# cosdata/cosdata

Measured on AMD Instinct MI355X. Metric: QPS at recall@10≥0.95, 1024-dim dense cosine, 1/2/4/8 MI355X, higher is better.
Workload: dtype u8

## Files before the change

### cosdata_amd/_lib.py

```python
from __future__ import annotations

import ctypes as C
import os
import subprocess

_PKG = os.path.dirname(os.path.abspath(__file__))
SO_PATH = os.path.join(_PKG, "libcosdata_hip.so")
CSRC = os.path.join(_PKG, "csrc")

OK, ERR_STORAGE_MISMATCH, ERR_CALCULATION, ERR_INVALID, ERR_UNIMPLEMENTED, ERR_HIP, ERR_NOT_READY, ERR_NO_DEVICE = range(8)
STATUS_NAMES = {
    0: "OK", 1: "StorageMismatch", 2: "CalculationError", 3: "Invalid", 4: "Unimplemented", 5: "HipError",
    6: "NotReady", 7: "NoDevice",
}
ABI_VERSION = 1


class CosdataError(RuntimeError):

    def __init__(self, status: int, message: str):
        super().__init__(f"[{STATUS_NAMES.get(status, status)}] {message}")
        self.status = status


class CosParams(C.Structure):
    _fields_ = [
        ("struct_size", C.c_uint32), ("abi_version", C.c_uint32), ("dim", C.c_uint32), ("metric", C.c_uint32),
        ("storage", C.c_uint32), ("resolution", C.c_uint32), ("range_lo", C.c_float), ("range_hi", C.c_float),
        ("num_layers", C.c_uint32), ("neighbors_count", C.c_uint32), ("level0_neighbors_count", C.c_uint32),
        ("ef_construction", C.c_uint32), ("ef_search", C.c_uint32), ("shortlist_size", C.c_uint32),
        ("visited_mode", C.c_uint32), ("device", C.c_int32), ("id_base", C.c_uint32), ("reserved", C.c_uint32),
        ("seed", C.c_uint64),
    ]


class CosSearchStats(C.Structure):
    _fields_ = [
        ("evals", C.c_uint64), ("expansions", C.c_uint64), ("adj_bytes", C.c_uint64), ("rerank_rows", C.c_uint64),
        ("walk_ms", C.c_float), ("finalize_ms", C.c_float), ("prep_ms", C.c_float), ("reserved", C.c_uint32),
    ]


class CosWalkSplit(C.Structure):
    _fields_ = [
        ("struct_size", C.c_uint32), ("queries", C.c_uint32), ("table_level_min", C.c_uint32), ("table_cols", C.c_uint32),
        ("cut_after_level", C.c_uint32), ("table_early_wgs", C.c_uint32),
        ("table_ms", C.c_float), ("upper_ms", C.c_float), ("sort_ms", C.c_float), ("lower_ms", C.c_float),
        ("table_int8_ops", C.c_double), ("table_evals", C.c_uint64),
        ("upper_evals", C.c_uint64), ("upper_expansions", C.c_uint64), ("upper_adj_bytes", C.c_uint64),
        ("lower_evals", C.c_uint64), ("lower_expansions", C.c_uint64), ("lower_adj_bytes", C.c_uint64),
    ]


class CosTimingSummary(C.Structure):
    _fields_ = [("launches", C.c_uint32), ("prep_ms_sum", C.c_float), ("walk_ms_sum", C.c_float), ("finalize_ms_sum", C.c_float),
                ("walk_ms_min", C.c_float), ("walk_ms_max", C.c_float)]


class CosCoalescingStats(C.Structure):
    _fields_ = [("launches", C.c_uint64), ("queries", C.c_uint64), ("requests", C.c_uint64), ("closed_full", C.c_uint64),
                ("closed_quiet", C.c_uint64), ("closed_deadline", C.c_uint64), ("solo_calls", C.c_uint64)]


class CosSparseStats(C.Structure):
    _fields_ = [("kernel_ms", C.c_float), ("blocks", C.c_uint32), ("postings_visited", C.c_uint64), ("posting_bytes", C.c_uint64)]


class CosFlatStats(C.Structure):
    _fields_ = [("gemm_ms", C.c_float), ("gemm_launches", C.c_uint32), ("int8_ops", C.c_double), ("code_bytes", C.c_double)]


SCAN_SKIP_DELETED = 1


class CosScanMask(C.Structure):
    _fields_ = [("struct_size", C.c_uint32), ("flags", C.c_uint32), ("n_masks", C.c_uint32), ("bits", C.c_void_p),
                ("query_mask", C.c_void_p)]


class CosBM25Stats(C.Structure):
    _fields_ = [("struct_size", C.c_uint32), ("documents_count", C.c_uint32), ("n_terms", C.c_uint32), ("largest_doc_id", C.c_uint32),
                ("dir_rows", C.c_uint32), ("dir_tiles", C.c_uint32), ("reserved", C.c_uint32),
                ("postings", C.c_uint64), ("tombstones", C.c_uint64), ("device_bytes", C.c_uint64)]


class CosSparseIndexStats(C.Structure):
    _fields_ = [("struct_size", C.c_uint32), ("n_vectors", C.c_uint32), ("n_dims", C.c_uint32), ("dir_rows", C.c_uint32),
                ("dir_tiles", C.c_uint32), ("packed", C.c_uint32), ("have_raw", C.c_uint32), ("reserved", C.c_uint32),
                ("postings", C.c_uint64), ("removed", C.c_uint64), ("raw_pairs", C.c_uint64), ("device_bytes", C.c_uint64)]


class CosHybridRequest(C.Structure):
    _fields_ = [("struct_size", C.c_uint32), ("B", C.c_uint32), ("arm", C.c_void_p), ("dense_queries", C.c_void_p),
                ("sparse_dims", C.c_void_p), ("sparse_vals", C.c_void_p), ("sparse_offsets", C.c_void_p),
                ("bm25_terms", C.c_void_p), ("bm25_offsets", C.c_void_p),
                ("sparse_early_terminate_threshold", C.c_float), ("sparse_reranking_factor", C.c_uint32),
                ("top_k", C.c_uint32), ("fusion_constant_k", C.c_float)]


def build(force: bool = False, verbose: bool = False) -> str:
    srcs = [os.path.join(CSRC, f) for f in os.listdir(CSRC) if f.endswith((".hip", ".h"))]
    srcs.append(os.path.join(_PKG, "..", "include", "cosdata_hip.h"))
    stale = force or not os.path.exists(SO_PATH) or any(os.path.getmtime(s) > os.path.getmtime(SO_PATH) for s in srcs)
    if force:
        subprocess.check_call(["make", "-C", CSRC, "-s", "clean"])
    if stale:
        cmd = ["make", "-C", CSRC, "-j", str(max(2, min(16, 2 * (os.cpu_count() or 1))))]
        if not verbose:
            cmd.append("-s")
        subprocess.check_call(cmd)
    return SO_PATH


_lib = None

ABI_SYMBOLS = [
    "cos_index_create", "cos_index_destroy", "cos_last_error_string", "cos_device_count",
    "cos_index_upload_vectors", "cos_index_set_root", "cos_index_upload_graph_level", "cos_index_level_count",
    "cos_index_download_graph_level", "cos_index_download_codes", "cos_index_download_root", "cos_index_build", "cos_index_append", "cos_index_delete", "cos_index_restore_link_state", "cos_index_release_link_state", "cos_index_enable_metadata", "cos_index_upload_meta_nodes", "cos_index_upload_meta_graph_level", "cos_index_build_meta", "cos_index_meta_level_count", "cos_index_download_meta_graph_level", "cos_search_filtered_batch",
    "cos_ann_search_filtered_batch", "cos_index_load_reference_dir", "cos_reference_dir_level_counts", "cos_reference_dir_read_level",
    "cos_search_batch", "cos_search_batch_device", "cos_ann_search_batch", "cos_index_set_coalescing", "cos_index_coalescing_stats", "cos_index_set_ef_search",
    "cos_index_set_visited_mode", "cos_index_set_latency_mode", "cos_index_set_latency_waves", "cos_index_set_walk_order", "cos_index_walk_order_cuts", "cos_index_set_walk_table", "cos_index_walk_table_info", "cos_index_last_walk_split", "cos_index_enable_timing", "cos_index_last_stats", "cos_index_timing_summary", "cos_quantize_batch",
    "cos_code_bytes", "cos_sample_values_range", "cos_distance_batch", "cos_bruteforce_topk", "cos_flat_search_batch",
    "cos_flat_search_masked_batch", "cos_bruteforce_topk_masked", "cos_index_deleted_count", "cos_index_download_deleted", "cos_bm25_create", "cos_bm25_destroy",
    "cos_bm25_insert", "cos_bm25_delete", "cos_bm25_stats", "cos_bm25_download",
    "cos_bm25_search_batch", "cos_bm25_search_batch_device", "cos_rrf_fuse_batch", "cos_hybrid_search_batch", "cos_text_process", "cos_text_count_tokens", "cos_bm25_term_frequency", "cos_xxhash32", "cos_stem_english", "cos_sparse_create", "cos_sparse_build_csr", "cos_sparse_create_from_vectors", "cos_sparse_destroy", "cos_sparse_search_batch", "cos_sparse_last_stats", "cos_sparse_layout",
    "cos_sparse_set_max_candidates", "cos_sparse_max_candidates", "cos_sparse_search_batch_device",
    "cos_hybrid_create", "cos_hybrid_destroy", "cos_hybrid_search_mixed",
    "cos_sparse_insert", "cos_sparse_delete", "cos_sparse_stats", "cos_sparse_download", "cos_merge_topk_device", "cos_merge_topk_packed_device", "cos_hbm_probe",
    "cos_shardset_unique_id", "cos_shardset_create", "cos_shardset_destroy", "cos_shardset_search_batch", "cos_shardset_exchange_device",
    "cos_tuning_set", "cos_tuning_clear", "cos_tuning_get",
]


def lib():
    global _lib
    if _lib is not None:
        return _lib
    if not os.path.exists(SO_PATH):
        raise CosdataError(ERR_NO_DEVICE, f"{SO_PATH} is missing: build it with `python -c 'import __graft_entry__ as g; g.build()'` "
                                          "(the HIP extension is mandatory; there is no CPU path)")
    try:
        import torch
    except ImportError:
        pass
    L = C.CDLL(SO_PATH)
    vp, i32, u32, f32 = C.c_void_p, C.c_int32, C.c_uint32, C.c_float
    sig = {
        "cos_index_create": [C.POINTER(CosParams), C.POINTER(vp)],
        "cos_index_destroy": [vp],
        "cos_device_count": [C.POINTER(i32)],
        "cos_index_upload_vectors": [vp, vp, u32, u32],
        "cos_index_set_root": [vp, vp],
        "cos_index_upload_graph_level": [vp, u32, u32, vp, vp],
        "cos_index_level_count": [vp, u32, C.POINTER(u32)],
        "cos_index_download_graph_level": [vp, u32, vp, vp],
        "cos_index_download_codes": [vp, vp, vp],
        "cos_index_download_root": [vp, vp],
        "cos_index_build": [vp, u32],
        "cos_index_append": [vp, vp, u32, u32, u32],
        "cos_index_release_link_state": [vp],
        "cos_index_restore_link_state": [vp],
        "cos_index_delete": [vp, vp, u32],
        "cos_index_load_reference_dir": [vp, C.c_char_p, u32, u32],
        "cos_index_enable_metadata": [vp, u32, u32],
        "cos_index_upload_meta_nodes": [vp, u32, vp, vp],
        "cos_index_upload_meta_graph_level": [vp, u32, u32, vp, vp],
        "cos_search_filtered_batch": [vp, vp, u32, vp, vp, u32, vp, vp, vp, vp],
        "cos_ann_search_filtered_batch": [vp, vp, u32, vp, vp, vp, vp, vp, vp],
        "cos_reference_dir_level_counts": [C.c_char_p, u32, u32, u32, vp],
        "cos_reference_dir_read_level": [C.c_char_p, u32, u32, u32, u32, vp, vp],
        "cos_search_batch": [vp, vp, u32, u32, vp, vp, vp, vp],
        "cos_search_batch_device": [vp, vp, u32, u32, vp, vp, vp, vp, vp],
        "cos_ann_search_batch": [vp, vp, u32, vp, vp, vp, vp],
        "cos_index_set_ef_search": [vp, u32],
        "cos_index_set_coalescing": [vp, u32, u32],
        "cos_index_coalescing_stats": [vp, C.POINTER(CosCoalescingStats)],
        "cos_index_set_visited_mode": [vp, u32],
        "cos_index_build_meta": [vp, u32, vp, vp, vp, u32],
        "cos_index_meta_level_count": [vp, u32, C.POINTER(u32)],
        "cos_index_download_meta_graph_level": [vp, u32, vp, vp],
        "cos_index_set_latency_mode": [vp, u32],
        "cos_index_set_latency_waves": [vp, u32],
        "cos_index_set_walk_order": [vp, u32],
        "cos_index_walk_order_cuts": [vp, C.POINTER(u32), u32, C.POINTER(u32)],
        "cos_index_enable_timing": [vp, i32],
        "cos_index_last_stats": [vp, vp, C.POINTER(CosSearchStats)],
        "cos_index_set_walk_table": [vp, u32, u32],
        "cos_index_walk_table_info": [vp, C.POINTER(u32), C.POINTER(u32)],
        "cos_index_last_walk_split": [vp, vp, C.POINTER(CosWalkSplit)],
        "cos_index_timing_summary": [vp, vp, C.POINTER(CosTimingSummary)],
        "cos_quantize_batch": [u32, u32, u32, f32, f32, vp, u32, vp, vp],
        "cos_sample_values_range": [vp, u32, u32, f32, C.POINTER(f32), C.POINTER(f32)],
        "cos_distance_batch": [u32, u32, u32, u32, vp, vp, u32, vp, vp, u32, vp, vp, u32, vp, vp],
        "cos_bruteforce_topk": [vp, vp, u32, u32, vp, vp],
        "cos_flat_search_batch": [vp, vp, u32, u32, vp, vp, vp, C.POINTER(CosFlatStats)],
        "cos_flat_search_masked_batch": [vp, vp, u32, u32, C.POINTER(CosScanMask), vp, vp, vp, C.POINTER(CosFlatStats)],
        "cos_bruteforce_topk_masked": [vp, vp, u32, u32, C.POINTER(CosScanMask), vp, vp, vp],
        "cos_index_deleted_count": [vp, C.POINTER(u32)],
        "cos_index_download_deleted": [vp, vp],
        "cos_bm25_create": [i32, vp, vp, u32, vp, vp, u32, C.POINTER(vp)],
        "cos_bm25_destroy": [vp],
        "cos_bm25_insert": [vp, vp, vp, u32, vp, vp],
        "cos_bm25_delete": [vp, vp, vp, u32, vp],
        "cos_bm25_stats": [vp, C.POINTER(CosBM25Stats)],
        "cos_bm25_download": [vp, C.POINTER(u32), C.POINTER(C.c_uint64), vp, vp, vp, vp, vp],
        "cos_bm25_search_batch": [vp, vp, vp, u32, u32, vp, vp, vp],
        "cos_bm25_search_batch_device": [vp, vp, vp, u32, u32, vp, vp, vp, vp],
        "cos_rrf_fuse_batch": [vp, vp, u32, vp, vp, u32, u32, f32, u32, vp, vp, vp],
        "cos_hybrid_search_batch": [vp, vp, vp, vp, vp, u32, u32, f32, vp, vp, vp],
        "cos_sparse_create": [i32, u32, f32, vp, u32, vp, vp, u32, vp, vp, vp, C.POINTER(vp)],
        "cos_sparse_build_csr": [u32, f32, u32, vp, vp, vp, vp, vp, vp, C.POINTER(u32)],
        "cos_sparse_create_from_vectors": [i32, u32, f32, u32, vp, vp, vp, i32, C.POINTER(vp)],
        "cos_sparse_destroy": [vp],
        "cos_sparse_search_batch": [vp, vp, vp, vp, u32, u32, f32, u32, vp, vp, vp],
        "cos_sparse_search_batch_device": [vp, vp, vp, vp, u32, u32, f32, u32, vp, vp, vp, vp],
        "cos_hybrid_create": [i32, C.POINTER(vp)],
        "cos_hybrid_destroy": [vp],
        "cos_hybrid_search_mixed": [vp, vp, vp, vp, C.POINTER(CosHybridRequest), vp, vp, vp],
        "cos_sparse_last_stats": [vp, vp],
        "cos_sparse_layout": [vp, C.POINTER(u32)],
        "cos_sparse_set_max_candidates": [vp, u32],
        "cos_sparse_max_candidates": [vp, C.POINTER(u32)],
        "cos_sparse_insert": [vp, u32, vp, vp, vp, C.POINTER(u32)],
        "cos_sparse_delete": [vp, vp, vp, u32, vp, vp, C.POINTER(C.c_uint64)],
        "cos_sparse_stats": [vp, C.POINTER(CosSparseIndexStats)],
        "cos_sparse_download": [vp, C.POINTER(u32), C.POINTER(C.c_uint64), vp, vp, vp],
        "cos_merge_topk_device": [vp, vp, vp, u32, u32, u32, vp, vp, vp, i32, vp],
        "cos_merge_topk_packed_device": [vp, u32, u32, u32, vp, vp, vp, i32, vp],
        "cos_hbm_probe": [i32, u32, C.c_uint64, u32, u32, C.POINTER(C.c_double)],
        "cos_shardset_unique_id": [vp],
        "cos_shardset_create": [vp, u32, u32, u32, vp, C.POINTER(vp)],
        "cos_shardset_destroy": [vp],
        "cos_shardset_search_batch": [vp, vp, u32, u32, vp, vp, vp],
        "cos_shardset_exchange_device": [vp, vp, u32, u32, vp, vp, vp, vp, vp],
        "cos_tuning_set": [C.c_char_p, C.c_int64],
        "cos_tuning_clear": [C.c_char_p],
        "cos_tuning_get": [C.c_char_p, C.POINTER(C.c_int64), C.POINTER(i32)],
    }
    for name, args in sig.items():
        fn = getattr(L, name)
        fn.restype = i32
        fn.argtypes = args
    L.cos_last_error_string.restype = C.c_char_p
    L.cos_last_error_string.argtypes = []
    L.cos_stem_english.restype = C.c_size_t
    L.cos_stem_english.argtypes = [vp, C.c_char_p, C.c_size_t, C.c_char_p, C.c_size_t]
    L.cos_text_process.restype = i32
    L.cos_text_process.argtypes = [C.c_char_p, C.c_size_t, u32, f32, f32, f32, vp, vp, vp, vp, u32, C.POINTER(u32)]
    L.cos_text_count_tokens.restype = u32
    L.cos_text_count_tokens.argtypes = [C.c_char_p, C.c_size_t, u32]
    L.cos_bm25_term_frequency.restype = f32
    L.cos_bm25_term_frequency.argtypes = [u32, u32, f32, f32, f32]
    L.cos_xxhash32.restype = u32
    L.cos_xxhash32.argtypes = [C.c_char_p, C.c_size_t, u32]
    L.cos_code_bytes.restype = C.c_size_t
    L.cos_code_bytes.argtypes = [u32, u32, u32]
    _lib = L
    return L


def check(rc: int):
    if rc != OK:
        raise CosdataError(rc, lib().cos_last_error_string().decode("utf-8", "replace"))


def tuning_set(name: str, value: int):
    check(lib().cos_tuning_set(name.encode(), int(value)))


def tuning_clear(name: str | None = None):
    check(lib().cos_tuning_clear(name.encode() if name is not None else None))


def tuning_get(name: str):
    v, isset = C.c_int64(), C.c_int32()
    check(lib().cos_tuning_get(name.encode(), C.byref(v), C.byref(isset)))
    return int(v.value) if isset.value else None


class tuning:

    def __init__(self, **knobs):
        self.knobs = knobs
        self.old = {}

    def __enter__(self):
        try:
            for k, v in self.knobs.items():
                old = tuning_get(k)
                tuning_set(k, v)
                self.old[k] = old
        except Exception:
            self.__exit__()
            raise
        return self

    def __exit__(self, *exc):
        for k, v in self.old.items():
            if v is None:
                tuning_clear(k)
            else:
                tuning_set(k, v)
        return False
```

### cosdata_amd/csrc/engine.hip

```cpp
#include <hip/hip_runtime.h>

#include <algorithm>
#include <cstdarg>
#include <cstdio>
#include <cstdlib>
#include <chrono>
#include <cmath>
#include <condition_variable>
#include <cstring>
#include <map>
#include <mutex>
#include <string>
#include <thread>
#include <vector>

#include "engine_internal.h"

using namespace cosdev;

static thread_local std::string g_err;
int32_t cos_fail(int32_t code, const char *fmt, ...) {
    char buf[512];
    va_list ap;
    va_start(ap, fmt);
// ... 506 lines not shown

extern "C" int32_t cos_index_download_root(const cos_index *ix, float *root_raw) {
    if (!ix || !root_raw) return cos_fail(COS_ERR_INVALID, "null argument");
    if (!ix->have_root) return cos_fail(COS_ERR_NOT_READY, "no root");
    memcpy(root_raw, ix->root_raw.data(), (size_t)ix->p.dim * 4);
    return COS_OK;
}

static int32_t ensure_level_table(cos_index *ix);
static u32 walk_table_min_B(const cos_index *ix);
extern "C" int32_t cos_index_set_ef_search(cos_index *ix, uint32_t ef) {
    if (!ix) return cos_fail(COS_ERR_INVALID, "null index");
    if (ef > cosdev::WALK_GENERAL_MAX_EF) return cos_fail(COS_ERR_UNIMPLEMENTED, "ef > %u not supported on the device", cosdev::WALK_GENERAL_MAX_EF);
    std::lock_guard<std::mutex> g(ix->mu);
    const bool live = graph_ready(ix);
    if (live)
        if (int32_t rc = cos_set_device(ix)) return rc;
    ix->p.ef_search = ef;
    if (live && walk_table_min_B(ix)) (void)ensure_level_table(ix);
    return COS_OK;
}
extern "C" int32_t cos_index_set_visited_mode(cos_index *ix, uint32_t mode) {
    if (!ix || mode > 1) return cos_fail(COS_ERR_INVALID, "bad visited mode");
    std::lock_guard<std::mutex> g(ix->mu);
    ix->p.visited_mode = mode;
    return COS_OK;
}
extern "C" int32_t cos_index_set_latency_mode(cos_index *ix, uint32_t max_queries) {
    if (!ix) return cos_fail(COS_ERR_INVALID, "null");
    std::lock_guard<std::mutex> g(ix->mu);
    ix->lat_max_B = max_queries;
    return COS_OK;
}

extern "C" int32_t cos_index_set_latency_waves(cos_index *ix, uint32_t max_queries) {
    if (!ix) return cos_fail(COS_ERR_INVALID, "null");
    std::lock_guard<std::mutex> g(ix->mu);
    ix->lat4_max_B = max_queries;
    return COS_OK;
}
extern "C" int32_t cos_index_set_walk_order(cos_index *ix, uint32_t min_queries) {
    if (!ix) return cos_fail(COS_ERR_INVALID, "null");
    std::lock_guard<std::mutex> g(ix->mu);
    ix->walk_order_min_B = min_queries;
    return COS_OK;
}
extern "C" int32_t cos_index_enable_timing(cos_index *ix, int32_t on) {
    if (!ix) return cos_fail(COS_ERR_INVALID, "null");
    std::lock_guard<std::mutex> g(ix->mu);
    if (on && !ix->timing) for (auto &kv : ix->ws) kv.second->ev_count = 0;
    ix->timing = on != 0;
    return COS_OK;
}

int32_t vis_tab_prepare(VisTab &vt, const cos_index *ix, u32 B, u32 ef, hipStream_t st, WalkArgs &wa) {
    const u32 M = std::max(ix->p.level0_neighbors_count, ix->p.neighbors_count);
    const u64 log_cap = (u64)ef * M + 2;
    u32 max_nodes = 0;
    for (const LevelHost &l : ix->lv) max_nodes = std::max(max_nodes, l.n);
    const u32 words = (max_nodes + 31) / 32 + 1;
    if (log_cap > 0xFFFFFFFFull) return cos_fail(COS_ERR_INVALID, "ef too large");
    const size_t need_bits = (size_t)B * words, need_log = (size_t)B * log_cap;
    if (need_bits > vt.bits.cap || need_log > vt.log.cap) {
        HIP_TRY(hipStreamSynchronize(st));
        if (need_bits > vt.bits.cap) vt.zeroed = false;
        HIP_TRY(vt.bits.grow(need_bits));
        HIP_TRY(vt.log.grow(need_log));
    }
    if (!vt.zeroed) {
        HIP_TRY(hipMemsetAsync(vt.bits, 0, vt.bits.cap * 4, st));
        vt.zeroed = true;
    }
    wa.vis_bits = vt.bits;
    wa.vis_log = vt.log;
    wa.vis_words_per_query = words;
    wa.vis_log_cap = (u32)log_cap;
    return COS_OK;
}

static int32_t ensure_order_rank(cos_index *ix) {
    if (ix->order_rank_valid) return COS_OK;
    for (u32 l = 0; l < cosdev::MAX_LEVELS; l++) {
        ix->d_order_rank[l].reset();
        ix->order_rank_n[l] = 0;
    }
    ix->order_levels.clear();
    const u32 Ltop = ix->p.num_layers;
    auto usable = [&](u32 l) { return l >= 1 && l <= Ltop && ix->lv[l].n > 1 && ix->lv[l].n <= (1u << 20) && ix->lv[l].d_adj_node; };
    std::vector<u32> want;
    if (const long long mask = cosdev::tune(cosdev::TUNE_WALK_SPLIT_LEVELS); mask != cosdev::TUNE_UNSET) {
        for (u32 l = Ltop; l >= 1; l--)
            if ((mask >> l) & 1) want.push_back(l);
    } else {
        for (u32 l = 1; l <= Ltop; l++)
            if (usable(l) && (size_t)ix->lv[l].n * ix->row_stride <= ((size_t)64 << 20)) { want.push_back(l); break; }
    }
    u32 prev = Ltop + 1;
    for (u32 l : want) {
        if (!usable(l) || l >= prev) continue;
        ix->order_levels.push_back(l);
        prev = l;
    }
    if (!ix->order_levels.empty()) HIP_TRY(hipDeviceSynchronize());
    for (u32 kl : ix->order_levels) {
        const LevelHost &H = ix->lv[kl];
        const u32 n = H.n, M = H.M;
        std::vector<u32> adj((size_t)n * M), rank(n, 0u), stack;
        HIP_TRY(hipMemcpy(adj.data(), H.d_adj_node, adj.size() * 4, hipMemcpyDeviceToHost));
        std::vector<uint8_t> seen(n, 0);
        u32 next = 0;
        auto dfs_from = [&](u32 start) {
            stack.push_back(start);
            while (!stack.empty()) {
                const u32 v = stack.back();
                stack.pop_back();
                if (seen[v]) continue;
                seen[v] = 1;
                rank[v] = next++;
                const u32 *row = &adj[(size_t)v * M];
                for (u32 j = M; j-- > 0;) {
                    const u32 u = row[j];
                    if (u != cosdev::ROW_EMPTY && u < n && !seen[u]) stack.push_back(u);
                }
            }
        };
        dfs_from(n - 1);
        for (u32 v = 0; v < n; v++) if (!seen[v]) dfs_from(v);
        HIP_TRY(ix->d_order_rank[kl].alloc(n));
        HIP_TRY(hipMemcpy(ix->d_order_rank[kl], rank.data(), (size_t)n * 4, hipMemcpyHostToDevice));
        ix->order_rank_n[kl] = n;
    }
    ix->order_rank_valid = true;
    return COS_OK;
}

static void clear_current_table(cos_index *ix) {
    ix->d_tcodes = nullptr;
    ix->d_tmags = nullptr;
    ix->d_tcsums = nullptr;
    ix->table_cols = 0;
    ix->table_level_min = 0;
    ix->table_stride = 0;
}
static u32 walk_table_max_cols(const cos_index *ix) {
    const long long env = cosdev::tune_or(cosdev::TUNE_WALK_TABLE_COLS, -1);
    return env >= 0 ? (u32)std::min<long long>(env, 1ll << 20) : ix->walk_table_max_cols;
}
static u32 walk_table_min_B(const cos_index *ix) {
    const long long env = cosdev::tune_or(cosdev::TUNE_WALK_TABLE_MIN_B, -1);
    return env >= 0 ? (u32)std::min<long long>(env, 0xFFFFFFFFll) : ix->walk_table_min_B;
}
static constexpr long long WALK_TABLE_EARLY_WGS_DEFAULT = 0;
static constexpr long long WALK_UP_TABLE_DEFAULT = 1;
cosdev::WalkPlanIn cos_walk_plan_in(const cos_index *ix, u32 B, u32 ef) {
    cosdev::WalkPlanIn in{};
    in.eng = ix->eng;
    in.storage = ix->p.storage;
    in.nchunks = ix->nchunks;
    in.G = ix->G;
    in.num_layers = ix->p.num_layers;
    for (u32 l = 0; l <= ix->p.num_layers; l++) in.M[l] = ix->lv[l].M;
    in.shortlist = ix->p.shortlist_size;
    in.visited_mode = ix->p.visited_mode;
    in.mdim = ix->meta.mdim;
    in.B = B;
    in.ef = ef;
    in.chain = true;
    const long long lat = cosdev::tune_or(cosdev::TUNE_WALK_LAT, -1), lat4 = cosdev::tune_or(cosdev::TUNE_WALK_LAT4, -1);
    in.lat_max_B = lat >= 0 ? (u32)std::min(lat, 0xFFFFFFFFll) : ix->lat_max_B;
    in.lat4_max_B = lat4 >= 0 ? (u32)std::min(lat4, 0xFFFFFFFFll) : ix->lat4_max_B;
    in.small_table_tk = cosdev::tune_or(cosdev::TUNE_WALK_SMALL_TABLE_TK, 1) != 0;
    in.adj_mag_mode = (u32)cosdev::tune_or(cosdev::TUNE_WALK_ADJ_MAG, 1);
    in.table_min_B = walk_table_min_B(ix);
    in.order_min_B = ix->walk_order_min_B;
    in.chain_min_B = ix->chain_min_B;
    in.side_min_B = ix->walk_side_min_B;
    in.table_after_sort = cosdev::tune_or(cosdev::TUNE_WALK_TABLE_AFTER_SORT, 1);
    in.table_supported = cosdev::level_table_eng_supported(ix->eng, ix->row_stride);
    in.adj_mag_valid = ix->adj_mag_valid;
    in.up_table_mode = (u32)std::min<long long>(std::max<long long>(cosdev::tune_or(cosdev::TUNE_WALK_UP_TABLE, WALK_UP_TABLE_DEFAULT), 0), 2);
    in.table_early_wgs = (u32)std::min<long long>(std::max<long long>(cosdev::tune_or(cosdev::TUNE_WALK_TABLE_EARLY_WGS, WALK_TABLE_EARLY_WGS_DEFAULT), 0), 0xFFFFFFFFll);
    in.table_queue = cosdev::level_table_gemm_queue(ix->eng, ix->row_stride);
    in.n_cus = ix->n_cus;
    return in;
}
static int32_t ensure_level_table(cos_index *ix) {
    const u32 max_cols = walk_table_max_cols(ix);
    const bool automatic = max_cols == COS_WALK_TABLE_AUTO;
    const u32 efs = ix->p.ef_search, Mup = ix->p.neighbors_count;
    const u64 c_rule = (u64)cosdev::tune_or(cosdev::TUNE_WALK_TABLE_RULE_C, 2u * efs <= 3u * Mup ? 10 : (efs <= 2u * Mup ? 8 : 6));
    const u64 per_level = automatic ? std::min<u64>(c_rule * ix->p.ef_search * ix->p.neighbors_count, 1u << 20) : (u64)(1u << 20);
    const u64 total_cap = automatic ? (u64)(1u << 20) : (u64)max_cols;
    const u64 key = automatic ? (0x8000000000000000ull | per_level) : (u64)max_cols;
    if (ix->level_table_valid && ix->table_built_for_key == key) return COS_OK;
    if (!ix->level_table_valid) {
        HIP_TRY(hipDeviceSynchronize());
        ix->table_sets.clear();
    }
    ix->level_table_valid = true;
    ix->table_built_for_key = key;
    clear_current_table(ix);
    for (const auto &t : ix->table_sets)
        if (t.key == key) {
            ix->table_level_min = t.level_min;
            ix->table_cols = t.cols;
            ix->table_stride = t.stride;
            memcpy(ix->table_col0, t.col0, sizeof(t.col0));
            ix->d_tcodes = t.tcodes;
            ix->d_tmags = t.tmags;
            ix->d_tcsums = t.tcsums;
            return COS_OK;
        }
    if (!cosdev::level_table_eng_supported(ix->eng, ix->row_stride) || max_cols == 0) return COS_OK;
    const u32 Ltop = ix->p.num_layers;
    u32 cols = 0, lmin = 0;
    for (u32 l = Ltop; l >= 1; l--) {
        if (!ix->lv[l].d_node_vec || ix->lv[l].n == 0 || ix->lv[l].n > per_level || (u64)cols + ix->lv[l].n > total_cap) break;
        cols += ix->lv[l].n;
        lmin = l;
    }
    if (lmin == 0) return COS_OK;
    HIP_TRY(hipDeviceSynchronize());
    cos_index::TableSet t;
    auto build = [&]() -> hipError_t {
        hipError_t e = t.tcodes.alloc((size_t)cols * ix->row_stride);
        if (e == hipSuccess) e = t.tmags.alloc(cols);
        if (e == hipSuccess) e = t.tcsums.alloc(cols);
        u32 c0 = 0;
        for (u32 l = Ltop; l >= lmin && e == hipSuccess; l--) {
            ix->table_col0[l] = c0;
            e = cosdev::launch_level_table_gather(ix->d_codes, ix->d_mags, ix->row_stride, ix->lv[l].d_node_vec, ix->lv[l].n, c0, t.tcodes, t.tmags, nullptr);
            c0 += ix->lv[l].n;
        }
        if (e == hipSuccess) e = cosdev::launch_code_sums(t.tcodes, ix->row_stride, cols, t.tcsums, nullptr);
        if (e == hipSuccess) e = hipDeviceSynchronize();
        return e;
    };
    if (const hipError_t e = build(); e != hipSuccess) {
        (void)hipDeviceSynchronize();
        if (e == hipErrorOutOfMemory) {
            (void)hipGetLastError();
            return COS_OK;
        }
        ix->level_table_valid = false;
        HIP_TRY(e);
    }
    ix->d_tcodes = t.tcodes;
    ix->d_tmags = t.tmags;
    ix->d_tcsums = t.tcsums;
    ix->table_cols = cols;
    ix->table_level_min = lmin;
    ix->table_stride = ((u64)cols + 31) / 32 * 32;
    t.key = key;
    t.level_min = lmin;
    t.cols = cols;
    t.stride = ix->table_stride;
    memcpy(t.col0, ix->table_col0, sizeof(t.col0));
    ix->table_sets.push_back(std::move(t));
    return COS_OK;
}

extern "C" int32_t cos_index_set_walk_table(cos_index *ix, uint32_t max_cols, uint32_t min_queries) {
    if (!ix) return cos_fail(COS_ERR_INVALID, "null argument");
    if (max_cols > (1u << 20) && max_cols != COS_WALK_TABLE_AUTO) return cos_fail(COS_ERR_INVALID, "max_cols must be <= 2^20 (or COS_WALK_TABLE_AUTO)");
    std::lock_guard<std::mutex> g(ix->mu);
    ix->walk_table_max_cols = max_cols;
    ix->walk_table_min_B = min_queries;
    return COS_OK;
}

extern "C" int32_t cos_index_walk_table_info(cos_index *ix, uint32_t *out_level_min, uint32_t *out_cols) {
    if (!ix || !out_level_min || !out_cols) return cos_fail(COS_ERR_INVALID, "null argument");
    *out_level_min = *out_cols = 0;
    if (!graph_ready(ix)) return cos_fail(COS_ERR_NOT_READY, "index needs vectors, root and every graph level");
    int32_t rc = cos_set_device(ix);
    if (rc) return rc;
    std::lock_guard<std::mutex> g(ix->mu);
    if (walk_table_min_B(ix) == 0) return COS_OK;
    if ((rc = ensure_level_table(ix))) return rc;
    *out_level_min = ix->table_level_min;
    *out_cols = ix->table_cols;
    return COS_OK;
}

static int32_t ensure_adj_mags(cos_index *ix) {
    if (ix->adj_mag_valid) return COS_OK;
    if (!graph_ready(ix) || ix->meta.mdim != 0u) return COS_OK;
    if (cosdev::walk_rows_over_64_slots(cos_walk_plan_in(ix, 0, 0))) return COS_OK;
    HIP_TRY(hipDeviceSynchronize());
    for (u32 l = 0; l <= ix->p.num_layers; l++) {
        ix->lv[l].d_adj_mag.reset();
    }
    for (u32 l = 0; l <= ix->p.num_layers; l++) {
        LevelHost &H = ix->lv[l];
        const u32 slots = std::min(H.M, ix->p.shortlist_size);
        const hipError_t e = H.d_adj_mag.alloc((size_t)H.n * slots);
        if (e == hipErrorOutOfMemory) {
            (void)hipGetLastError();
            for (u32 k = 0; k < l; k++) ix->lv[k].d_adj_mag.reset();
            return COS_OK;
        }
        HIP_TRY(e);
        HIP_TRY(cosdev::launch_fill_adj_mag(H.d_adj_vec, ix->d_mags, H.d_adj_mag, H.n, H.M, slots, ix->own_stream));
    }
    HIP_TRY(hipStreamSynchronize(ix->own_stream));
    ix->adj_mag_valid = true;
    return COS_OK;
}

static int32_t ensure_adj_up(cos_index *ix) {
    const u32 want = (ix->adj_mag_valid && ix->level_table_valid && ix->table_level_min >= 2u && ix->eng == ENG_U8 && ix->G == 64u &&
                      cosdev::tune_or(cosdev::TUNE_WALK_UP_TABLE, WALK_UP_TABLE_DEFAULT) != 0)
                         ? ix->table_level_min - 1u
                         : 0u;
    if (want != 0u && (ix->adj_up_level == want || ix->adj_up_oom_level == want)) return COS_OK;
    bool any = false;
    for (u32 l = 0; l <= ix->p.num_layers; l++) any = any || ix->lv[l].d_adj_up;
    if (any) {
        HIP_TRY(hipDeviceSynchronize());
        for (u32 l = 0; l <= ix->p.num_layers; l++) ix->lv[l].d_adj_up.reset();
    }
    ix->adj_up_level = 0;
    if (want == 0u) return COS_OK;
    ix->adj_up_oom_level = 0;
    HIP_TRY(hipDeviceSynchronize());
    LevelHost &H = ix->lv[want];
    const LevelHost &U = ix->lv[want + 1];
    const u32 slots = std::min(H.M, ix->p.shortlist_size);
    if (!H.d_adj_node || !U.d_child || H.n == 0 || U.n == 0) return COS_OK;
    DevArr<u32> up;
    hipError_t e = H.d_adj_up.alloc((size_t)H.n * slots);
    if (e == hipSuccess) e = up.alloc(H.n);
    if (e == hipErrorOutOfMemory) {
        (void)hipGetLastError();
        H.d_adj_up.reset();
        ix->adj_up_oom_level = want;
        return COS_OK;
    }
    HIP_TRY(e);
    HIP_TRY(cosdev::launch_fill_adj_up(H.d_adj_vec, H.d_adj_node, ix->d_mags, U.d_child, U.n, up, H.d_adj_up, H.n, H.M, slots, ix->own_stream));
    HIP_TRY(hipStreamSynchronize(ix->own_stream));
    ix->adj_up_level = want;
    return COS_OK;
}

int32_t cos_prepare_walk_plans(cos_index *ix) {
    std::lock_guard<std::mutex> g(ix->mu);
    if (int32_t rc = ensure_adj_mags(ix)) return rc;
    if (ix->walk_order_min_B)
        if (int32_t rc = ensure_order_rank(ix)) return rc;
    if (walk_table_min_B(ix)) {
        if (int32_t rc = ensure_level_table(ix)) return rc;
        if (int32_t rc = ensure_adj_up(ix)) return rc;
    }
    return COS_OK;
}

extern "C" int32_t cos_index_walk_order_cuts(cos_index *ix, uint32_t *out_levels, uint32_t cap, uint32_t *out_n) {
    if (!ix || !out_n || (cap && !out_levels)) return cos_fail(COS_ERR_INVALID, "null argument");
    *out_n = 0;
    if (!graph_ready(ix)) return cos_fail(COS_ERR_NOT_READY, "index needs vectors, root and every graph level");
    int32_t rc = cos_set_device(ix);
    if (rc) return rc;
    std::lock_guard<std::mutex> g(ix->mu);
    if ((rc = ensure_order_rank(ix))) return rc;
    for (u32 l : ix->order_levels) {
        if (*out_n < cap) out_levels[*out_n] = l;
        (*out_n)++;
    }
    return COS_OK;
}

struct SearchLaunch {
    cosdev::WalkPlan plan;
    u32 ef = 0, visited_mode = 0;
    bool timed = false;
    u64 tab_stride = 0;
    u32 tab_col0[cosdev::MAX_LEVELS] = {};
    const uint8_t *tcodes = nullptr;
    const float *tmags = nullptr;
    const u32 *tcsums = nullptr;
    u32 n_keys = 0, key_level[cosdev::MAX_LEVELS], key_n[cosdev::MAX_LEVELS];
    const u32 *order_rank[cosdev::MAX_LEVELS];
};

static int32_t get_workspace(cos_index *ix, void *key, hipStream_t st, u32 B, u32 top_k, bool host_api, Workspace **out, SearchLaunch *L,
                             bool chain = true) {
    std::lock_guard<std::mutex> g(ix->mu);
    std::unique_ptr<Workspace> &slot = ix->ws[key];
    if (!slot) slot.reset(new Workspace());
    Workspace *w = slot.get();
    const u32 L1 = ix->p.num_layers + 1;
    if (B > w->capB) {
        u32 cap = std::max(B, 64u);
        HIP_TRY(hipStreamSynchronize(st));
        w->capB = 0;
        w->cap_topk = 0;
        HIP_TRY(w->q_codes.alloc((size_t)cap * ix->row_stride));
        HIP_TRY(w->q_mags.alloc(cap));
        HIP_TRY(w->q_raw_mags.alloc(cap));
        HIP_TRY(w->walk_ids.alloc((size_t)cap * L1 * KEEP_SEARCH));
        HIP_TRY(w->walk_sims.alloc((size_t)cap * L1 * KEEP_SEARCH));
        HIP_TRY(w->walk_counts.alloc((size_t)cap * L1));
        HIP_TRY(w->walk_status.alloc(cap));
        HIP_TRY(w->stats.alloc((size_t)cap * 4));
        HIP_TRY(w->stats2.alloc((size_t)cap * 4));
        HIP_TRY(w->qsums.alloc(cap));
        HIP_TRY(w->tab_queue.alloc(16));
        if (ix->eng == ENG_Q2) HIP_TRY(w->qdig.alloc((size_t)cap * (ix->row_stride / 16) * 64));
        HIP_TRY(w->fin_flags.alloc((size_t)cap + 1));
        HIP_TRY(w->rerank_rows.alloc(cap));
        HIP_TRY(w->d_queries.alloc((size_t)cap * ix->p.dim));
        HIP_TRY(w->d_out_counts.alloc(cap));
        HIP_TRY(w->d_out_status.alloc(cap));
        w->capB = cap;
    }
    L->ef = ix->p.ef_search;
    L->visited_mode = ix->p.visited_mode;
    L->timed = ix->timing;
    cosdev::WalkPlanIn in = cos_walk_plan_in(ix, B, L->ef);
    in.chain = chain;
    const cosdev::WalkPlan want = cosdev::walk_plan(in);
    cosdev::WalkHave have{};
    if (want.refill_adj_mag) {
        if (int32_t rc = ensure_adj_mags(ix)) return rc;
        in.adj_mag_valid = ix->adj_mag_valid;
    }
    if (want.prepare_order) {
        if (w->order.cap < w->capB) {
            HIP_TRY(hipStreamSynchronize(st));
            HIP_TRY(cosdev::walk_order_reserve(w->order, w->capB));
        }
        if (int32_t rc = ensure_order_rank(ix)) return rc;
        have.order_buffers = w->order.cap >= B;
        have.n_order_keys = (u32)ix->order_levels.size();
        have.order_level0 = have.n_order_keys ? ix->order_levels[0] : 0u;
    }
    if (want.prepare_table) {
        if (int32_t rc = ensure_level_table(ix)) return rc;
        if (int32_t rc = ensure_adj_up(ix)) return rc;
        have.adj_up_level = ix->adj_up_level;
        const size_t need = (size_t)w->capB * ix->table_stride;
        if (need > w->tab.cap) {
            const size_t budget = (size_t)cosdev::tune_or(cosdev::TUNE_WALK_TABLE_MAX_BYTES, (long long)48 << 30);
            HIP_TRY(hipStreamSynchronize(st));
            ix->table_bytes_total -= w->tab.cap * 4;
            w->tab.reset();
            if (ix->table_bytes_total + need * 4 <= budget) {
                if (const hipError_t e = w->tab.alloc(need); e == hipSuccess)
                    ix->table_bytes_total += need * 4;
                else if (e == hipErrorOutOfMemory)
                    (void)hipGetLastError();
                else
                    HIP_TRY(e);
            }
        }
        have.table_level_min = ix->level_table_valid ? ix->table_level_min : 0u;
        have.table_cols = ix->table_cols;
        have.table_buffer = w->tab && (size_t)B * ix->table_stride <= w->tab.cap;
    }
    L->plan = cosdev::walk_plan(in, &have);
    if (L->plan.use_table) {
        L->tab_stride = ix->table_stride;
        memcpy(L->tab_col0, ix->table_col0, sizeof(L->tab_col0));
        L->tcodes = ix->d_tcodes;
        L->tmags = ix->d_tmags;
        L->tcsums = ix->d_tcsums;
    }
    if (L->plan.ordered)
        for (u32 l : ix->order_levels) {
            L->key_level[L->n_keys] = l;
            L->key_n[L->n_keys] = ix->order_rank_n[l];
            L->order_rank[L->n_keys++] = ix->d_order_rank[l];
        }
    if (host_api && (size_t)top_k * w->capB > (size_t)w->cap_topk * w->capB) {
        w->cap_topk = 0;
        HIP_TRY(w->d_out_ids.alloc((size_t)w->capB * top_k));
        HIP_TRY(w->d_out_scores.alloc((size_t)w->capB * top_k));
        w->cap_topk = top_k;
    }
    if (w->ev.empty()) {
        w->ev.assign((size_t)Workspace::EV_RING * Workspace::EV_PER, nullptr);
        for (auto &e : w->ev) HIP_TRY(hipEventCreate(&e));
    }
    if (!w->walk_done) HIP_TRY(hipEventCreateWithFlags(&w->walk_done, hipEventDisableTiming));
    if (!w->walk_fin) HIP_TRY(hipEventCreateWithFlags(&w->walk_fin, hipEventDisableTiming));
    if (!w->last_range) HIP_TRY(hipEventCreateWithFlags(&w->last_range, hipEventDisableTiming));
    if (!w->upper_done) HIP_TRY(hipEventCreateWithFlags(&w->upper_done, hipEventDisableTiming));
    *out = w;
    return COS_OK;
}

static int32_t run_search(cos_index *ix, Workspace *w, const SearchLaunch &L, const float *d_queries, u32 B, u32 top_k, u32 *d_out_ids,
                          float *d_out_scores, u32 *d_out_counts, int32_t *d_out_status, bool do_finalize, hipStream_t st,
                          hipStream_t st_fin = nullptr, hipEvent_t walk_ev = nullptr) {
    const cosdev::WalkPlan &plan = L.plan;
    const bool timed = L.timed, ordered = plan.ordered, chained = plan.chained;
    const u32 ef = L.ef, n_keys = L.n_keys;
    IndexDev dev = cos_make_index_dev(ix);
    dev.visited_mode = L.visited_mode;
    for (u32 l = 0; l <= dev.num_layers; l++)
        if (!((plan.use_adj_mag >> l) & 1u)) dev.lv[l].adj_mag = nullptr;
    for (u32 l = 0; l <= dev.num_layers; l++)
        if (plan.up_table_level != l || l == 0u || dev.lv[l].adj_mag == nullptr) dev.lv[l].adj_up = nullptr;
    WalkArgs wa;
    memset(&wa, 0, sizeof(wa));
    if (dev.visited_mode == COS_VISITED_EXACT) {
        int32_t rc = vis_tab_prepare(w->vis, ix, B, ef, st, wa);
        if (rc) return rc;
    }
    hipEvent_t *ev = &w->ev[(size_t)(w->ev_count % Workspace::EV_RING) * Workspace::EV_PER];
    if (timed) HIP_TRY(hipEventRecord(ev[0], st));
    HIP_TRY(launch_quantize_rows(ix->eng, d_queries, ix->p.dim, B, ix->p.dim, ix->p.range_lo, ix->p.range_hi, w->q_codes, ix->row_stride,
                                 w->q_mags, w->q_raw_mags, st, plan.use_table && ix->eng == ENG_U8 ? w->qsums.p : nullptr));
    HIP_TRY(hipMemsetAsync(w->stats2, 0, (size_t)B * 32, st));
    if (plan.use_table) {
        auto table_part = [&](hipEvent_t cos_index::*handle_ev, hipEvent_t own_ev, hipEvent_t *marks, u32 wgs, bool first) -> int32_t {
            if (plan.table_waits_for_sort) {
                std::lock_guard<std::mutex> g(ix->chain_mu);
                if (ix->*handle_ev && ix->*handle_ev != own_ev) HIP_TRY(hipStreamWaitEvent(st, ix->*handle_ev, 0));
            }
            if (timed) HIP_TRY(hipEventRecord(marks[0], st));
            HIP_TRY(cosdev::launch_level_table(ix->eng, w->q_codes, w->q_mags, w->qsums, w->qdig, B, L.tcodes, L.tmags, L.tcsums, ix->row_stride, plan.table_cols,
                                               w->tab, L.tab_stride, ix->n_cus, st, w->tab_queue, wgs, first, plan.table_waits_for_sort));
            if (timed) HIP_TRY(hipEventRecord(marks[1], st));
            return COS_OK;
        };
        if (cosdev::level_table_gemm_queue(ix->eng, ix->row_stride)) HIP_TRY(hipMemsetAsync(w->tab_queue, 0, sizeof(u32), st));
        if (plan.table_early_wgs) {
            if (int32_t rc = table_part(&cos_index::chain_upper_ev, w->upper_done, ev + 4, plan.table_early_wgs, true)) return rc;
            if (int32_t rc = table_part(&cos_index::chain_ev, w->walk_done, ev + 8, 0u, false)) return rc;
        } else if (int32_t rc = table_part(&cos_index::chain_last_range_ev, w->last_range, ev + 4, 0u, true))
            return rc;
    }
    if (timed) HIP_TRY(hipEventRecord(ev[1], st));
    wa.qcodes = w->q_codes;
    wa.qmags = w->q_mags;
    wa.B = B;
    wa.ef = ef;
    wa.keep = KEEP_SEARCH;
    wa.out_ids = w->walk_ids;
    wa.out_sims = w->walk_sims;
    wa.out_counts = w->walk_counts;
    wa.out_status = w->walk_status;
    wa.out_stats = w->stats;
    wa.out_stats2 = w->stats2;
    if (plan.use_table) {
        wa.tab = w->tab;
        wa.tab_mags = L.tmags;
        wa.tab_stride = L.tab_stride;
        wa.tab_level_min = plan.table_level_min;
        memcpy(wa.tab_col0, L.tab_col0, sizeof(L.tab_col0));
    }
    hipStream_t sw = st;
    if (plan.side_stream) {
        if (!w->walk_stream) {
            int lo = 0, hi = 0;
            HIP_TRY(hipDeviceGetStreamPriorityRange(&lo, &hi));
            HIP_TRY(hipStreamCreateWithPriority(&w->walk_stream, hipStreamNonBlocking, lo));
            HIP_TRY(hipEventCreateWithFlags(&w->prep_done, hipEventDisableTiming));
        }
        sw = w->walk_stream;
        HIP_TRY(hipEventRecord(w->prep_done, st));
        HIP_TRY(hipStreamWaitEvent(sw, w->prep_done, 0));
    }
    auto walk = [&](hipStream_t s) -> int32_t {
        if (!ordered) {
            if (chained) HIP_TRY(hipEventRecord(w->upper_done, s));
            if (chained) HIP_TRY(hipEventRecord(w->last_range, s));
            HIP_TRY(launch_walk(ix->eng, dev, wa, plan.kernel, s));
            return COS_OK;
        }
        wa.phase = 1;
        wa.entry0 = w->order.entry0;
        wa.order_key = w->order.order_key;
        wa.order_iota = w->order.iota;
        u32 first = dev.num_layers;
        for (u32 i = 0; i <= n_keys; i++) {
            const bool last = i == n_keys;
            wa.level_first = first;
            wa.level_last = last ? 0u : L.key_level[i];
            wa.key_n = last ? 0u : L.key_n[i];
            wa.order_rank = last ? nullptr : L.order_rank[i];
            if (last && chained) HIP_TRY(hipEventRecord(w->last_range, s));
            HIP_TRY(launch_walk(ix->eng, dev, wa, plan.kernel, s));
            if (last) break;
            if (chained && i == 0) HIP_TRY(hipEventRecord(w->upper_done, s));
            if (timed && i == 0) HIP_TRY(hipEventRecord(ev[6], s));
            HIP_TRY(cosdev::launch_walk_order(w->order, B, L.key_n[i], ix->num_xcd, s));
            if (timed && i == 0) HIP_TRY(hipEventRecord(ev[7], s));
            wa.q_order = w->order.q_order;
            first = L.key_level[i] - 1;
        }
        return COS_OK;
    };
    if (chained) {
        std::lock_guard<std::mutex> g(ix->chain_mu);
        if (ix->chain_ev && ix->chain_ev != w->walk_done) HIP_TRY(hipStreamWaitEvent(sw, ix->chain_ev, 0));
        if (timed) HIP_TRY(hipEventRecord(ev[1], sw));
        if (int32_t rc = walk(sw)) return rc;
        HIP_TRY(hipEventRecord(w->walk_done, sw));
        ix->chain_ev = w->walk_done;
        ix->chain_last_range_ev = w->last_range;
        ix->chain_upper_ev = w->upper_done;
    } else {
        if (timed && sw != st) HIP_TRY(hipEventRecord(ev[1], sw));
        if (int32_t rc = walk(sw)) return rc;
    }
    if (timed) HIP_TRY(hipEventRecord(ev[2], sw));
    hipStream_t sf = st_fin ? st_fin : st;
    if (sf != sw) {
        hipEvent_t we = walk_ev ? walk_ev : w->walk_fin;
        HIP_TRY(hipEventRecord(we, sw));
        HIP_TRY(hipStreamWaitEvent(sf, we, 0));
    }
    if (do_finalize) {
        HIP_TRY(launch_finalize(dev, d_queries, ix->p.dim, w->q_raw_mags, w->walk_ids, w->walk_sims, w->walk_counts, w->walk_status, B, top_k,
                                d_out_ids, d_out_scores, d_out_counts, d_out_status, w->rerank_rows, sf, ordered ? w->order.q_order : nullptr, w->fin_flags));
    }
    if (timed) { HIP_TRY(hipEventRecord(ev[3], sf)); w->ev_count++; }
    w->lastB = B;
    w->timed = timed;
    w->last_plan = plan;
    { std::lock_guard<std::mutex> g(ix->mu); ix->last_ws = w; }
    return COS_OK;
}

static int32_t check_search_args(cos_index *ix, const void *q, u32 B, u32 top_k) {
    if (!ix || !q) return cos_fail(COS_ERR_INVALID, "null argument");
    if (!graph_ready(ix)) return cos_fail(COS_ERR_NOT_READY, "index needs vectors, root and every graph level before search");
    if (top_k == 0 || top_k > 1024) return cos_fail(COS_ERR_INVALID, "top_k must be in [1, 1024]");
    if (B == 0) return cos_fail(COS_ERR_INVALID, "empty batch");
    return cos_set_device(ix);
}

extern "C" int32_t cos_search_batch_device(cos_index *ix, const float *d_queries, uint32_t B, uint32_t top_k, uint32_t *d_out_ids,
                                           float *d_out_scores, uint32_t *d_out_counts, int32_t *d_out_status, void *stream) {
    int32_t rc = check_search_args(ix, d_queries, B, top_k);
    if (rc) return rc;
    if (!d_out_ids || !d_out_scores || !d_out_counts || !d_out_status) return cos_fail(COS_ERR_INVALID, "null output");
    Workspace *w;
    SearchLaunch L;
    rc = get_workspace(ix, stream, (hipStream_t)stream, B, top_k, false, &w, &L);
    if (rc) return rc;
    return run_search(ix, w, L, d_queries, B, top_k, d_out_ids, d_out_scores, d_out_counts, d_out_status, true, (hipStream_t)stream);
}

struct PipeLease {
    cos_index *ix;
    HostPipe *hp = nullptr;
    explicit PipeLease(cos_index *ix_) : ix(ix_) {}
    PipeLease(const PipeLease &) = delete;
    PipeLease &operator=(const PipeLease &) = delete;
    int32_t acquire() {
        std::unique_lock<std::mutex> lk(ix->pipe_mu);
        for (;;) {
            if (!ix->pipes_free.empty()) { hp = ix->pipes_free.back(); ix->pipes_free.pop_back(); break; }
            if (ix->pipes_all.size() < COS_MAX_HOST_PIPES) {
                std::unique_ptr<HostPipe> n(new HostPipe());
                hipError_t e = hipStreamCreateWithFlags(&n->s[0], hipStreamNonBlocking);
                if (e != hipSuccess) return cos_fail(COS_ERR_HIP, "hipStreamCreateWithFlags: %s", hipGetErrorString(e));
                hp = n.get();
                ix->pipes_all.push_back(std::move(n));
                break;
            }
            ix->pipe_cv.wait(lk);
        }
        ix->host_calls_active.fetch_add(1);
        return COS_OK;
    }
    ~PipeLease() {
        if (!hp) return;
        ix->host_calls_active.fetch_sub(1);
        { std::lock_guard<std::mutex> g(ix->pipe_mu); ix->pipes_free.push_back(hp); }
        ix->pipe_cv.notify_one();
    }
};

static int32_t report_status(const int32_t *status, u32 B) {
    for (u32 b = 0; b < B; b++)
        if (status[b] != COS_OK) return cos_fail(status[b], "query %u failed with status %d (zero-norm vector -> DistanceError::CalculationError)", b, status[b]);
    return COS_OK;
}

static int32_t search_host_simple(cos_index *ix, HostPipe *hp, const float *queries, uint32_t B, uint32_t top_k, uint32_t *out_ids, float *out_scores,
                                  uint32_t *out_counts, int32_t *out_status) {
    hipStream_t st = hp->s[0];
    Workspace *w;
    SearchLaunch L;
    int32_t rc = get_workspace(ix, (void *)st, st, B, top_k, true, &w, &L);
    if (rc) return rc;
    HIP_TRY(hipMemcpyAsync(w->d_queries, queries, (size_t)B * ix->p.dim * 4, hipMemcpyHostToDevice, st));
    rc = run_search(ix, w, L, w->d_queries, B, top_k, w->d_out_ids, w->d_out_scores, w->d_out_counts, w->d_out_status, true, st);
    if (rc) { (void)hipDeviceSynchronize(); return rc; }
    std::vector<int32_t> status(B);
    hipError_t e = hipMemcpyAsync(out_ids, w->d_out_ids, (size_t)B * top_k * 4, hipMemcpyDeviceToHost, st);
    if (e == hipSuccess) e = hipMemcpyAsync(out_scores, w->d_out_scores, (size_t)B * top_k * 4, hipMemcpyDeviceToHost, st);
    if (e == hipSuccess) e = hipMemcpyAsync(out_counts, w->d_out_counts, (size_t)B * 4, hipMemcpyDeviceToHost, st);
    if (e == hipSuccess) e = hipMemcpyAsync(status.data(), w->d_out_status, (size_t)B * 4, hipMemcpyDeviceToHost, st);
    const hipError_t es = hipStreamSynchronize(st);
    HIP_TRY(e);
    HIP_TRY(es);
    if (out_status) memcpy(out_status, status.data(), (size_t)B * 4);
    return report_status(status.data(), B);
}

static int32_t search_host_pipelined(cos_index *ix, HostPipe *hp, const float *queries, uint32_t B, uint32_t top_k, uint32_t *out_ids,
                                     float *out_scores, uint32_t *out_counts, int32_t *out_status) {
    const size_t dim = ix->p.dim;
    const u32 chunk = (((B + HostPipe::MAX_CHUNKS - 1) / HostPipe::MAX_CHUNKS) + 255u) & ~255u;
    const u32 nch = (B + chunk - 1) / chunk;
    if (!hp->s[1]) HIP_TRY(hipStreamCreateWithFlags(&hp->s[1], hipStreamNonBlocking));
    if (!hp->sc) HIP_TRY(hipStreamCreateWithFlags(&hp->sc, hipStreamNonBlocking));
    if (!hp->sf) HIP_TRY(hipStreamCreateWithFlags(&hp->sf, hipStreamNonBlocking));
    for (u32 i = 0; i < HostPipe::MAX_CHUNKS; i++) {
        if (!hp->ev_in[i]) HIP_TRY(hipEventCreateWithFlags(&hp->ev_in[i], hipEventDisableTiming));
        if (!hp->ev_walk[i]) HIP_TRY(hipEventCreateWithFlags(&hp->ev_walk[i], hipEventDisableTiming));
    }
    HIP_TRY(hp->d_q.grow((size_t)B * dim));
    HIP_TRY(hp->d_ids.grow((size_t)B * top_k));
    HIP_TRY(hp->d_scores.grow((size_t)B * top_k));
    HIP_TRY(hp->d_counts.grow((size_t)B));
    HIP_TRY(hp->d_status.grow((size_t)B));
    struct Drain {
        HostPipe *hp;
        bool ok = false;
        ~Drain() {
            hipStream_t sts[] = {hp->sc, hp->s[0], hp->s[1], hp->sf};
            for (hipStream_t st : sts) if (st) (void)hipStreamSynchronize(st);
            if (!ok) (void)hipDeviceSynchronize();
        }
    } drain{hp};
    for (u32 i = 0; i < nch; i++) {
        const u32 c0 = i * chunk, cb = std::min(chunk, B - c0);
        hipStream_t st = hp->s[i & 1];
        Workspace *w;
        SearchLaunch L;
        int32_t rc = get_workspace(ix, (void *)&hp->wkey[i], st, cb, top_k, false, &w, &L, false);
        if (rc) return rc;
        float *dq = hp->d_q + (size_t)c0 * dim;
        const float *src = queries + (size_t)c0 * dim;
        HIP_TRY(hipMemcpyAsync(dq, src, (size_t)cb * dim * 4, hipMemcpyHostToDevice, hp->sc));
        HIP_TRY(hipEventRecord(hp->ev_in[i], hp->sc));
        HIP_TRY(hipStreamWaitEvent(st, hp->ev_in[i], 0));
        rc = run_search(ix, w, L, dq, cb, top_k, hp->d_ids + (size_t)c0 * top_k, hp->d_scores + (size_t)c0 * top_k, hp->d_counts + c0, hp->d_status + c0,
                        true, st, hp->sf, hp->ev_walk[i]);
        if (rc) return rc;
    }
    std::vector<int32_t> status(B);
    hipError_t e = hipMemcpyAsync(out_ids, hp->d_ids, (size_t)B * top_k * 4, hipMemcpyDeviceToHost, hp->sf);
    if (e == hipSuccess) e = hipMemcpyAsync(out_scores, hp->d_scores, (size_t)B * top_k * 4, hipMemcpyDeviceToHost, hp->sf);
    if (e == hipSuccess) e = hipMemcpyAsync(out_counts, hp->d_counts, (size_t)B * 4, hipMemcpyDeviceToHost, hp->sf);
    if (e == hipSuccess) e = hipMemcpyAsync(status.data(), hp->d_status, (size_t)B * 4, hipMemcpyDeviceToHost, hp->sf);
    const hipError_t es = hipStreamSynchronize(hp->sf);
    HIP_TRY(e);
    HIP_TRY(es);
    drain.ok = true;
    if (out_status) memcpy(out_status, status.data(), (size_t)B * 4);
    return report_status(status.data(), B);
}

static u32 host_pipeline_min_B() {
    return (u32)cosdev::tune_or(cosdev::TUNE_HOST_PIPELINE_MIN_B, 8192);
}

static int32_t search_host_once(cos_index *ix, const float *queries, uint32_t B, uint32_t top_k, uint32_t *out_ids, float *out_scores,
                                uint32_t *out_counts, int32_t *out_status) {
    PipeLease lease(ix);
    int32_t rc = lease.acquire();
    if (rc) return rc;
    const u32 min_B = host_pipeline_min_B();
    if (min_B && B >= min_B && ix->host_calls_active.load() == 1)
        return search_host_pipelined(ix, lease.hp, queries, B, top_k, out_ids, out_scores, out_counts, out_status);
    return search_host_simple(ix, lease.hp, queries, B, top_k, out_ids, out_scores, out_counts, out_status);
}

// ... 173 lines not shown
        {
            std::lock_guard<std::mutex> lk(sl->mu);
            sl->rc = r;
            sl->err = e;
            sl->done = true;
        }
        sl->cv_done.notify_all();
    } else {
        std::unique_lock<std::mutex> lk(sl->mu);
        while (!sl->done) sl->cv_done.wait(lk);
    }
    const int32_t slot_rc = sl->rc;
    std::string slot_err = slot_rc != COS_OK ? sl->err : std::string();
    int32_t my_rc = COS_OK;
    u32 bad_q = 0;
    if (slot_rc == COS_OK) {
        const u32 *p_ids = sl->pin_out.as<const u32>();
        const float *p_sc = (const float *)(p_ids + (size_t)sl->cap * top_k);
        const u32 *p_cnt = (const u32 *)(p_sc + (size_t)sl->cap * top_k);
        const int32_t *p_st = (const int32_t *)(p_cnt + sl->cap);
        memcpy(out_ids, p_ids + (size_t)off * top_k, (size_t)B * top_k * 4);
        memcpy(out_scores, p_sc + (size_t)off * top_k, (size_t)B * top_k * 4);
        memcpy(out_counts, p_cnt + off, (size_t)B * 4);
        if (out_status) memcpy(out_status, p_st + off, (size_t)B * 4);
        for (u32 b = 0; b < B; b++)
            if (p_st[off + b] != COS_OK) { my_rc = p_st[off + b]; bad_q = b; break; }
    }
    if (sl->left.fetch_sub(1, std::memory_order_acq_rel) == 1) {
        std::lock_guard<std::mutex> lk(ix->co_mu);
        sl->n_req = 0;
        sl->closed = false;
    }
    if (slot_rc != COS_OK) return cos_fail(slot_rc, "%s", slot_err.c_str());
    if (my_rc != COS_OK) return cos_fail(my_rc, "query %u failed with status %d (zero-norm vector -> DistanceError::CalculationError)", bad_q, my_rc);
    return COS_OK;
}

extern "C" int32_t cos_ann_search_batch(cos_index *ix, const float *queries, uint32_t B, uint32_t *out_ids, float *out_sims,
                                        uint32_t *out_counts, int32_t *out_status) {
    int32_t rc = check_search_args(ix, queries, B, 1);
    if (rc) return rc;
    if (!out_ids || !out_sims || !out_counts) return cos_fail(COS_ERR_INVALID, "null output");
    PipeLease lease(ix);
    rc = lease.acquire();
    if (rc) return rc;
    hipStream_t st = lease.hp->s[0];
    Workspace *w;
    SearchLaunch L;
    rc = get_workspace(ix, (void *)st, st, B, 1, true, &w, &L);
    if (rc) return rc;
    const u32 L1 = ix->p.num_layers + 1;
    HIP_TRY(hipMemcpyAsync(w->d_queries, queries, (size_t)B * ix->p.dim * 4, hipMemcpyHostToDevice, st));
    rc = run_search(ix, w, L, w->d_queries, B, 1, nullptr, nullptr, nullptr, nullptr, false, st);
    if (rc) return rc;
    std::vector<int32_t> status(B);
    HIP_TRY(hipMemcpyAsync(out_ids, w->walk_ids, (size_t)B * L1 * KEEP_SEARCH * 4, hipMemcpyDeviceToHost, st));
    HIP_TRY(hipMemcpyAsync(out_sims, w->walk_sims, (size_t)B * L1 * KEEP_SEARCH * 4, hipMemcpyDeviceToHost, st));
    HIP_TRY(hipMemcpyAsync(out_counts, w->walk_counts, (size_t)B * L1 * 4, hipMemcpyDeviceToHost, st));
    HIP_TRY(hipMemcpyAsync(status.data(), w->walk_status, (size_t)B * 4, hipMemcpyDeviceToHost, st));
    HIP_TRY(hipStreamSynchronize(st));
    if (out_status) memcpy(out_status, status.data(), (size_t)B * 4);
    for (u32 b = 0; b < B; b++)
        if (status[b] != COS_OK) return cos_fail(status[b], "query %u failed with status %d", b, status[b]);
    return COS_OK;
}

static Workspace *find_workspace(cos_index *ix, void *stream, bool null_is_last) {
    std::lock_guard<std::mutex> g(ix->mu);
    if (!stream && null_is_last) return ix->last_ws;
    auto it = ix->ws.find(stream);
    return it != ix->ws.end() ? it->second.get() : nullptr;
}
static int32_t sum_launch_stats(const u64 *d_stats, u32 B, u64 sum[4]) {
    std::vector<u64> st((size_t)B * 4);
    HIP_TRY(hipMemcpy(st.data(), d_stats, st.size() * 8, hipMemcpyDeviceToHost));
    sum[0] = sum[1] = sum[2] = sum[3] = 0;
    for (u32 b = 0; b < B; b++)
        for (int k = 0; k < 4; k++) sum[k] += st[(size_t)b * 4 + k];
    return COS_OK;
}

extern "C" int32_t cos_index_last_stats(cos_index *ix, void *stream, cos_search_stats *out) {
    if (!ix || !out) return cos_fail(COS_ERR_INVALID, "null argument");
    memset(out, 0, sizeof(*out));
    int32_t rc = cos_set_device(ix);
    if (rc) return rc;
    Workspace *w = find_workspace(ix, stream, true);
    if (!w || w->lastB == 0) return cos_fail(COS_ERR_NOT_READY, "no batch has run on this stream");
    if (w->timed && w->ev_count) {
        hipEvent_t *ev = &w->ev[(size_t)((w->ev_count - 1) % Workspace::EV_RING) * Workspace::EV_PER];
        HIP_TRY(hipEventSynchronize(ev[3]));
        HIP_TRY(hipEventElapsedTime(&out->prep_ms, ev[0], ev[1]));
        HIP_TRY(hipEventElapsedTime(&out->walk_ms, ev[1], ev[2]));
        HIP_TRY(hipEventElapsedTime(&out->finalize_ms, ev[2], ev[3]));
    } else {
        HIP_TRY(hipDeviceSynchronize());
    }
    u64 st[4];
    if ((rc = sum_launch_stats(w->stats, w->lastB, st))) return rc;
    out->evals = st[0];
    out->expansions = st[1];
    out->adj_bytes = st[2];
    out->reserved = (uint32_t)st[3];
    std::vector<u64> rr(w->lastB);
    HIP_TRY(hipMemcpy(rr.data(), w->rerank_rows, rr.size() * 8, hipMemcpyDeviceToHost));
    for (u32 b = 0; b < w->lastB; b++) out->rerank_rows += rr[b];
    return COS_OK;
}

extern "C" int32_t cos_index_last_walk_split(cos_index *ix, void *stream, cos_walk_split *out) {
    if (!ix || !out) return cos_fail(COS_ERR_INVALID, "null argument");
    if (out->struct_size != sizeof(cos_walk_split)) return cos_fail(COS_ERR_INVALID, "cos_walk_split.struct_size mismatch");
    memset(out, 0, sizeof(*out));
    out->struct_size = sizeof(cos_walk_split);
    int32_t rc = cos_set_device(ix);
    if (rc) return rc;
    Workspace *w = find_workspace(ix, stream, true);
    if (!w || w->lastB == 0) return cos_fail(COS_ERR_NOT_READY, "no batch has run on this stream");
    const cosdev::WalkPlan &plan = w->last_plan;
    out->queries = w->lastB;
    out->table_level_min = plan.table_level_min;
    out->table_cols = plan.table_cols;
    out->cut_after_level = plan.cut_after_level;
    out->table_early_wgs = plan.use_table ? plan.table_early_wgs : 0u;
    if (w->timed && w->ev_count) {
        hipEvent_t *ev = &w->ev[(size_t)((w->ev_count - 1) % Workspace::EV_RING) * Workspace::EV_PER];
        HIP_TRY(hipEventSynchronize(ev[3]));
        if (plan.use_table) HIP_TRY(hipEventElapsedTime(&out->table_ms, ev[4], ev[5]));
        if (plan.use_table && plan.table_early_wgs) {
            float late_ms = 0.f;
            HIP_TRY(hipEventElapsedTime(&late_ms, ev[8], ev[9]));
            out->table_ms += late_ms;
        }
        if (plan.ordered) {
            HIP_TRY(hipEventElapsedTime(&out->upper_ms, ev[1], ev[6]));
            HIP_TRY(hipEventElapsedTime(&out->sort_ms, ev[6], ev[7]));
            HIP_TRY(hipEventElapsedTime(&out->lower_ms, ev[7], ev[2]));
        } else
            HIP_TRY(hipEventElapsedTime(&out->lower_ms, ev[1], ev[2]));
    } else {
        HIP_TRY(hipDeviceSynchronize());
    }
    const u32 kdims = (u32)((ix->row_stride + 63) / 64 * 64);
    out->table_int8_ops = 2.0 * (double)w->lastB * (double)out->table_cols * (double)kdims;
    u64 st[4], s2[4];
    if ((rc = sum_launch_stats(w->stats, w->lastB, st)) || (rc = sum_launch_stats(w->stats2, w->lastB, s2))) return rc;
    out->lower_evals = s2[0];
    out->lower_expansions = s2[1];
    out->lower_adj_bytes = s2[2];
    out->table_evals = s2[3];
    out->upper_evals = st[0] - s2[0];
    out->upper_expansions = st[1] - s2[1];
    out->upper_adj_bytes = st[2] - s2[2];
    return COS_OK;
}

extern "C" int32_t cos_index_timing_summary(cos_index *ix, void *stream, cos_timing_summary *out) {
    if (!ix || !out) return cos_fail(COS_ERR_INVALID, "null argument");
    memset(out, 0, sizeof(*out));
    int32_t rc = cos_set_device(ix);
    if (rc) return rc;
    Workspace *w = find_workspace(ix, stream, false);
    if (!w || w->ev_count == 0) return cos_fail(COS_ERR_NOT_READY, "no timed batch has run on this stream");
    const u32 n = std::min(w->ev_count, Workspace::EV_RING);
    out->launches = n;
    out->walk_ms_min = 1e30f;
    for (u32 i = 0; i < n; i++) {
        hipEvent_t *ev = &w->ev[(size_t)((w->ev_count - 1 - i) % Workspace::EV_RING) * Workspace::EV_PER];
        float a = 0, b = 0, c = 0;
        HIP_TRY(hipEventSynchronize(ev[3]));
        HIP_TRY(hipEventElapsedTime(&a, ev[0], ev[1]));
        HIP_TRY(hipEventElapsedTime(&b, ev[1], ev[2]));
        HIP_TRY(hipEventElapsedTime(&c, ev[2], ev[3]));
        out->prep_ms_sum += a;
        out->walk_ms_sum += b;
        out->finalize_ms_sum += c;
        out->walk_ms_min = std::min(out->walk_ms_min, b);
        out->walk_ms_max = std::max(out->walk_ms_max, b);
    }
    return COS_OK;
}

static constexpr u32 PSEUDO_LO = 0xFFFFFEFEu, PSEUDO_HI = 0xFFFFFFFDu;

extern "C" int32_t cos_index_enable_metadata(cos_index *ix, uint32_t mdim, uint32_t max_replicas_per_node) {
    if (!ix || mdim == 0 || mdim > 64 || max_replicas_per_node == 0) return cos_fail(COS_ERR_INVALID, "metadata dimensions must be in [1, 64] and max_replicas_per_node >= 1");
    if (!ix->have_vectors) return cos_fail(COS_ERR_NOT_READY, "upload vectors before enabling the metadata component");
    if (ix->p.ef_construction > cosdev::WALK_FAST_MAX_EF || std::min(ix->p.neighbors_count, ix->p.shortlist_size) > 64u ||
        std::min(ix->p.level0_neighbors_count, ix->p.shortlist_size) > 64u ||
        (ix->nchunks != 0u && (ix->nchunks + ix->G - 1u) / ix->G > (ix->eng == ENG_U8 ? 2u : 1u)))
        return cos_fail(COS_ERR_UNIMPLEMENTED, "metadata collections: ef_construction <= %u, at most 64 scanned neighbour slots per node, u8 rows of at most 2048 / SubByte rows of at most 64 x 16 bytes", cosdev::WALK_FAST_MAX_EF);
    if ((u64)ix->n * max_replicas_per_node >= PSEUDO_LO) return cos_fail(COS_ERR_INVALID, "replica ids would run into the reserved id range");
    if (ix->p.id_base % max_replicas_per_node != 0)
        return cos_fail(COS_ERR_INVALID, "id_base %u of a metadata collection's shard must be a multiple of max_replicas_per_node %u (first embedding x replicas)", ix->p.id_base, max_replicas_per_node);
    if ((u64)ix->p.id_base + (u64)ix->n * max_replicas_per_node >= PSEUDO_LO) return cos_fail(COS_ERR_INVALID, "replica ids would run into the reserved id range");
    for (auto &l : ix->lv)
        if (l.n) return cos_fail(COS_ERR_INVALID, "enable the metadata component before uploading / building the base graph: it changes the id of every vector (row x max_replicas)");
    int32_t rc = cos_set_device(ix);
    if (rc) return rc;
    ix->id_stride = max_replicas_per_node;
    ix->meta.mdim = mdim;
    ix->meta.lv.resize(ix->p.num_layers + 1);
    for (u32 l = 0; l <= ix->p.num_layers; l++) ix->meta.lv[l].M = l == 0 ? ix->p.level0_neighbors_count : ix->p.neighbors_count;
    DevBuf z;
    HIP_TRY(z.alloc(((size_t)ix->p.dim + 1) * 4));
    HIP_TRY(hipMemsetAsync(z.p, 0, ((size_t)ix->p.dim + 1) * 4, ix->own_stream));
    HIP_TRY(launch_quantize_rows(ix->eng, z.as<float>(), ix->p.dim, 1, ix->p.dim, ix->p.range_lo, ix->p.range_hi,
                                 ix->d_codes + ((size_t)ix->n + 1) * ix->row_stride, ix->row_stride, ix->d_mags + ix->n + 1, z.as<float>() + ix->p.dim, ix->own_stream));
    HIP_TRY(hipStreamSynchronize(ix->own_stream));
    return COS_OK;
}

extern "C" int32_t cos_index_upload_meta_nodes(cos_index *ix, uint32_t n_nodes, const uint32_t *node_ids, const int32_t *mbits) {
    if (!ix || !node_ids || !mbits || n_nodes == 0) return cos_fail(COS_ERR_INVALID, "null/empty node table");
    if (!ix->meta.mdim || !ix->have_vectors) return cos_fail(COS_ERR_NOT_READY, "cos_index_enable_metadata first");
    int32_t rc = cos_set_device(ix);
    if (rc) return rc;
    const u32 md = ix->meta.mdim;
    for (u32 i = 0; i < n_nodes; i++) {
        if (i && node_ids[i] <= node_ids[i - 1]) return cos_fail(COS_ERR_INVALID, "node ids must be strictly ascending");
        const bool pseudo = node_ids[i] >= PSEUDO_LO && node_ids[i] <= PSEUDO_HI;
        if (!pseudo && node_ids[i] / ix->id_stride >= ix->n) return cos_fail(COS_ERR_INVALID, "replica id %u has no resident vector", node_ids[i]);
    }
    std::vector<float> mags(n_nodes);
    for (u32 i = 0; i < n_nodes; i++) {
        float acc = -0.0f;
        for (u32 j = 0; j < md; j++) { const float x = (float)mbits[(size_t)i * md + j]; acc = acc + x * x; }
        mags[i] = sqrtf(acc);
    }
    ix->meta.d_mbits.reset();
    ix->meta.d_mmags.reset();
    for (auto &l : ix->meta.lv) l.release();
    HIP_TRY(ix->meta.d_mbits.alloc((size_t)n_nodes * md));
    HIP_TRY(ix->meta.d_mmags.alloc(n_nodes));
    HIP_TRY(hipMemcpy(ix->meta.d_mbits, mbits, (size_t)n_nodes * md * 4, hipMemcpyHostToDevice));
    HIP_TRY(hipMemcpy(ix->meta.d_mmags, mags.data(), (size_t)n_nodes * 4, hipMemcpyHostToDevice));
    ix->meta.node_ids.assign(node_ids, node_ids + n_nodes);
    return COS_OK;
}

extern "C" int32_t cos_index_upload_meta_graph_level(cos_index *ix, uint32_t level, uint32_t n_nodes, const uint32_t *node_ids, const uint32_t *nbr_ids) {
    if (!ix || !node_ids || !nbr_ids || n_nodes == 0) return cos_fail(COS_ERR_INVALID, "null/empty level");
    if (!ix->meta.mdim || !ix->have_vectors || ix->meta.node_ids.empty()) return cos_fail(COS_ERR_NOT_READY, "cos_index_enable_metadata + cos_index_upload_meta_nodes first");
    if (level > ix->p.num_layers) return cos_fail(COS_ERR_INVALID, "bad level");
    int32_t rc = cos_set_device(ix);
    if (rc) return rc;
    LevelHost &L = ix->meta.lv[level];
    const u32 M = L.M, n = ix->n;
    const std::vector<u32> &tab = ix->meta.node_ids;
    if (node_ids[0] != PSEUDO_LO && !std::binary_search(node_ids, node_ids + n_nodes, PSEUDO_LO)) return cos_fail(COS_ERR_INVALID, "level %u: the pseudo root (u32::MAX - 257) must be a node of every level", level);
    std::vector<u32> adj_vec((size_t)n_nodes * M), adj_node((size_t)n_nodes * M), node_vec(n_nodes), node_meta(n_nodes);
    u32 root_idx = 0;
    for (u32 i = 0; i < n_nodes; i++) {
        if (i && node_ids[i] <= node_ids[i - 1]) return cos_fail(COS_ERR_INVALID, "level %u: node_ids must be strictly ascending", level);
        auto it = std::lower_bound(tab.begin(), tab.end(), node_ids[i]);
        if (it == tab.end() || *it != node_ids[i]) return cos_fail(COS_ERR_INVALID, "level %u: node %u is not in the node table", level, node_ids[i]);
        node_meta[i] = (u32)(it - tab.begin());
        const bool pseudo = node_ids[i] >= PSEUDO_LO && node_ids[i] <= PSEUDO_HI;
        if (!pseudo && node_ids[i] / ix->id_stride >= n) return cos_fail(COS_ERR_INVALID, "level %u: replica id %u has no resident vector", level, node_ids[i]);
        node_vec[i] = pseudo ? n + 1 : node_ids[i] / ix->id_stride;
        if (node_ids[i] == PSEUDO_LO) root_idx = i;
    }
    for (u32 i = 0; i < n_nodes; i++)
        for (u32 j = 0; j < M; j++) {
            const u32 id = nbr_ids[(size_t)i * M + j];
            if (id == COS_SLOT_EMPTY) { adj_vec[(size_t)i * M + j] = adj_node[(size_t)i * M + j] = ROW_EMPTY; continue; }
            const uint32_t *it = std::lower_bound(node_ids, node_ids + n_nodes, id);
            if (it == node_ids + n_nodes || *it != id) return cos_fail(COS_ERR_INVALID, "level %u: neighbour id %u of node %u is not a node of this level", level, id, node_ids[i]);
            adj_node[(size_t)i * M + j] = (u32)(it - node_ids);
            adj_vec[(size_t)i * M + j] = node_vec[it - node_ids];
        }
    L.release();
    auto up = [&](DevArr<u32> &dst, const std::vector<u32> &src) -> hipError_t {
        hipError_t e = dst.alloc(src.size());
        return e == hipSuccess ? hipMemcpy(dst, src.data(), src.size() * 4, hipMemcpyHostToDevice) : e;
    };
    std::vector<u32> ids(node_ids, node_ids + n_nodes);
    HIP_TRY(up(L.d_adj_vec, adj_vec));
    HIP_TRY(up(L.d_adj_node, adj_node));
    HIP_TRY(up(L.d_node_vec, node_vec));
    HIP_TRY(up(L.d_node_id, ids));
    HIP_TRY(up(L.d_node_meta, node_meta));
    L.node_ids = std::move(ids);
    L.n = n_nodes;
    L.root_idx = root_idx;
    for (u32 lv = level; lv <= std::min(level + 1, ix->p.num_layers); lv++) {
        if (lv == 0) continue;
        LevelHost &U = ix->meta.lv[lv], &D = ix->meta.lv[lv - 1];
        if (U.n == 0 || D.n == 0) continue;
        std::vector<u32> child(U.n);
        for (u32 i = 0; i < U.n; i++) {
            auto it = std::lower_bound(D.node_ids.begin(), D.node_ids.end(), U.node_ids[i]);
            if (it == D.node_ids.end() || *it != U.node_ids[i]) return cos_fail(COS_ERR_INVALID, "node %u of level %u is missing on level %u", U.node_ids[i], lv, lv - 1);
            child[i] = (u32)(it - D.node_ids.begin());
        }
        HIP_TRY(up(U.d_child, child));
    }
    return COS_OK;
}

static bool meta_ready(const cos_index *ix) {
    if (!ix->meta.mdim || ix->meta.lv.size() != ix->p.num_layers + 1) return false;
    for (u32 l = 0; l <= ix->p.num_layers; l++)
        if (ix->meta.lv[l].n == 0 || (l > 0 && !ix->meta.lv[l].d_child)) return false;
    return ix->have_vectors;
}
// ... 149 lines not shown
```

### cosdata_amd/csrc/engine_internal.h

```cpp
#pragma once
#include <hip/hip_runtime.h>

#include <atomic>
#include <condition_variable>
#include <map>
#include <memory>
#include <mutex>
#include <string>
#include <thread>
#include <vector>

#include "../../include/cosdata_hip.h"
#include "engine_types.h"
#include "tuning.h"
#include "link_types.h"
#include "dev_mem.h"
#include "walk_plan.h"

namespace cosdev {
hipError_t launch_fill_i32(int32_t *p, u64 n, int32_t v, hipStream_t st);
hipError_t launch_edge_pairs(const u32 *adj_vec, const u32 *node_vec, u32 node0, u32 cn, u32 M, u32 *px, u32 *py, hipStream_t st);
hipError_t launch_edge_keys(const u32 *adj_vec, const float *sims, const int32_t *st_in, u32 node0, u32 cn, u32 M, u32 metric, int32_t *key, int32_t *fail, hipStream_t st);
hipError_t launch_low_cache(const u32 *adj_vec, const int32_t *key, u32 n, u32 M, int32_t kmin, int32_t kmax, uint8_t *low_idx, int32_t *low_key, hipStream_t st);
hipError_t launch_unlink(const LinkArgs &a, const u32 *dn, u32 *status, hipStream_t st);
hipError_t launch_index_pair_distances(int eng, const uint8_t *codes, const float *mags, u64 row_stride, u32 nchunks, u32 dim, u32 metric, const u32 *d_pair_x,
                                       const u32 *d_pair_y, u32 n_pairs, float *d_out, int32_t *d_status, hipStream_t st);
hipError_t launch_grow_rows(const u32 *src, u32 *dst, u32 old_n, u32 new_n, u32 M, u32 remap_from, u32 remap_to, u32 fill, hipStream_t st);
hipError_t launch_grow_bytes(const uint8_t *src, uint8_t *dst, u32 old_n, u32 new_n, hipStream_t st);
hipError_t launch_fill_adj_mag(const u32 *adj_vec, const float *mags, float *adj_mag, u32 n, u32 M, u32 slots, hipStream_t st);
hipError_t launch_fill_adj_up(const u32 *adj_vec, const u32 *adj_node, const float *mags, const u32 *child_up, u32 n_up, u32 *up, AdjUp *adj_up, u32 n, u32 M, u32 slots,
                              hipStream_t st);
hipError_t launch_link_round(const LinkArgs &a, u32 maxM, const u32 *pend, const u32 *pcount, u32 *next, u32 *next_count, u32 *evq, u32 *evq_count,
                             u32 count_ub, u32 round, hipStream_t st);
hipError_t launch_quantize_rows(int eng, const float *x, u64 x_stride, u32 n, u32 dim, float lo, float hi, uint8_t *codes,
                                u64 row_stride, float *mags, float *raw_mags, hipStream_t st, u32 *code_sums = nullptr);
hipError_t launch_walk(int eng, const IndexDev &ix, const WalkArgs &wa, WalkKernel kernel, hipStream_t st);
static_assert(WALK_PLAN_MAX_LEVELS == MAX_LEVELS && WALK_PLAN_ENG_U8 == ENG_U8 && WALK_PLAN_ENG_Q2 == ENG_Q2 && WALK_PLAN_FAST_MAX_EF == WALK_FAST_MAX_EF &&
              COS_STORAGE_U8 == 0u && COS_VISITED_REF == 0u, "walk_plan.h restates these");
hipError_t launch_walk_meta(int eng, const IndexDev &ix, const WalkArgs &wa, hipStream_t st);
hipError_t launch_walk_meta_index(int eng, const IndexDev &ix, const WalkArgs &wa, hipStream_t st);
hipError_t launch_finalize(const IndexDev &ix, const float *queries, u64 q_stride, const float *q_raw_mags, const u32 *walk_ids,
                           const float *walk_sims, const u32 *walk_counts, const int32_t *walk_status, u32 B, u32 top_k,
                           u32 *out_ids, float *out_scores, u32 *out_counts, int32_t *out_status, u64 *out_rerank_rows,
                           hipStream_t st, const u32 *q_order = nullptr, u32 *slow_list = nullptr);
struct WalkOrder {
    u32 cap = 0;
    DevArr<u32> entry0;
    DevArr<u32> order_key;
    DevArr<u32> keys_sorted;
    DevArr<u32> iota, vals_sorted, q_order;
    DevBuf tmp;
};
hipError_t walk_order_reserve(WalkOrder &o, u32 B);
hipError_t launch_walk_order(WalkOrder &o, u32 B, u32 key_max, u32 num_xcd, hipStream_t st);
hipError_t launch_level_table_gather(const uint8_t *codes, const float *mags, u64 row_stride, const u32 *node_vec, u32 n, u32 col0,
                                     uint8_t *tcodes, float *tmags, hipStream_t st);
hipError_t launch_code_sums(const uint8_t *codes, u64 row_stride, u32 n, u32 *sums, hipStream_t st);
hipError_t launch_level_table(int eng, const uint8_t *qcodes, const float *qmags, const u32 *qsums, uint8_t *qdig, u32 B, const uint8_t *tcodes, const float *tmags,
                              const u32 *tcsums, u64 row_stride, u32 ncols, float *tab, u64 tab_stride, u32 n_cus, hipStream_t st, u32 *queue, u32 wgs, bool first, bool shared);
bool level_table_gemm_queue(int eng, u64 row_stride);
bool level_table_eng_supported(int eng, u64 row_stride);
int32_t quantize_ref_layout(uint32_t storage, uint32_t res, uint32_t dim, const float *x, uint32_t n, void *codes, float *mags);
int32_t distance_ref_layout(uint32_t metric, uint32_t storage, uint32_t res, uint32_t dim, const void *x_codes, const float *x_mags, uint32_t nx,
                            const void *y_codes, const float *y_mags, uint32_t ny, const uint32_t *pair_x, const uint32_t *pair_y, uint32_t n_pairs,
                            float *out, int32_t *status);
}

using cosdev::u32;
using cosdev::u64;

int32_t cos_fail(int32_t code, const char *fmt, ...);
#define HIP_TRY(expr)                                                                                  \
    do {                                                                                               \
        hipError_t _e = (expr);                                                                        \
        if (_e != hipSuccess) return cos_fail(COS_ERR_HIP, "%s: %s (%s:%d)", #expr, hipGetErrorString(_e), __FILE__, __LINE__); \
    } while (0)

namespace cosdev {
std::mutex &sparse_mutex(cos_sparse *s);
int32_t sparse_device(const cos_sparse *s);
void sparse_limits(const cos_sparse *s, u32 *max_candidates, bool *have_raw, u32 *batch_bound);
int32_t sparse_search_locked(cos_sparse *s, const uint32_t *q_dims, const float *q_vals, const uint32_t *q_offsets, u32 B, u32 top_k,
                             float early_terminate_threshold, u32 reranking_factor, u32 *d_out_ids, float *d_out_scores, u32 *d_out_counts, hipStream_t st);
}

struct LevelHost {
    std::vector<u32> node_ids;
    std::vector<u32> nbr_ids;
    DevArr<u32> d_adj_vec, d_adj_node, d_node_vec, d_child;
    DevArr<u32> d_node_id, d_node_meta;
    DevArr<float> d_adj_mag;
    DevArr<cosdev::AdjUp> d_adj_up;
    u32 n = 0, M = 0;
    u32 root_idx = 0;
    bool host_valid = false;
    void release() {
        d_adj_vec.reset(); d_adj_node.reset(); d_node_vec.reset(); d_child.reset();
        d_node_id.reset(); d_node_meta.reset(); d_adj_mag.reset(); d_adj_up.reset();
        n = 0;
        node_ids.clear();
        nbr_ids.clear();
        host_valid = false;
    }
};

struct LinkState {
    DevBuf key[cosdev::MAX_LEVELS], low_idx[cosdev::MAX_LEVELS], low_key[cosdev::MAX_LEVELS], owner[cosdev::MAX_LEVELS];
    uint64_t rng = 0;
    u32 n_built = 0;
    bool valid = false;
    void release() {
        for (int l = 0; l < cosdev::MAX_LEVELS; l++) { key[l].reset(); low_idx[l].reset(); low_key[l].reset(); owner[l].reset(); }
        valid = false;
    }
};

struct VisTab {
    DevArr<u32> bits, log;
    bool zeroed = false;
};
int32_t vis_tab_prepare(VisTab &vt, const cos_index *ix, u32 B, u32 ef, hipStream_t st, cosdev::WalkArgs &wa);

struct Workspace {
    u32 capB = 0, cap_topk = 0;
    DevArr<uint8_t> q_codes;
    DevArr<float> q_mags, q_raw_mags;
    DevArr<u32> walk_ids, walk_counts;
    DevArr<float> walk_sims;
    DevArr<int32_t> walk_status;
    DevArr<u64> stats;
    DevArr<u64> stats2;
    DevArr<float> tab;
    DevArr<u32> qsums;
    DevArr<u32> tab_queue;
    DevArr<uint8_t> qdig;
    DevArr<u32> fin_flags;
    DevArr<u64> rerank_rows;
    VisTab vis;
    cosdev::WalkOrder order;
    DevArr<float> d_queries;
    DevArr<u32> d_out_ids, d_out_counts;
    DevArr<float> d_out_scores;
    DevArr<int32_t> d_out_status;
    DevArr<u32> f_buf;
    static constexpr u32 EV_RING = 128;
    static constexpr u32 EV_PER = 10;
    std::vector<hipEvent_t> ev;
    u32 ev_count = 0;
    hipEvent_t walk_done = nullptr;
    hipEvent_t last_range = nullptr;
    hipEvent_t upper_done = nullptr;
    hipStream_t walk_stream = nullptr;
    hipEvent_t prep_done = nullptr, walk_fin = nullptr;
    u32 lastB = 0;
    bool timed = false;
    cosdev::WalkPlan last_plan{};
    Workspace() = default;
    Workspace(const Workspace &) = delete;
    ~Workspace() {
        for (hipEvent_t e : {walk_done, walk_fin, last_range, upper_done, prep_done}) if (e) (void)hipEventDestroy(e);
        for (hipEvent_t e : ev) if (e) (void)hipEventDestroy(e);
        if (walk_stream) (void)hipStreamDestroy(walk_stream);
    }
};

struct MetaGraph {
    u32 mdim = 0;
    std::vector<u32> node_ids;
    DevArr<int32_t> d_mbits;
    DevArr<float> d_mmags;
    std::vector<LevelHost> lv;
};

struct HostPipe {
    static constexpr u32 MAX_CHUNKS = 4;
    hipStream_t s[2] = {nullptr, nullptr}, sc = nullptr, sf = nullptr;
    hipEvent_t ev_in[MAX_CHUNKS] = {}, ev_walk[MAX_CHUNKS] = {};
    char wkey[MAX_CHUNKS] = {};
    DevArr<float> d_q;
    DevArr<u32> d_ids, d_counts;
    DevArr<float> d_scores;
    DevArr<int32_t> d_status;
    HostPipe() = default;
    HostPipe(const HostPipe &) = delete;
    ~HostPipe() {
        for (hipEvent_t e : ev_in) if (e) (void)hipEventDestroy(e);
        for (hipEvent_t e : ev_walk) if (e) (void)hipEventDestroy(e);
        for (hipStream_t st : {s[0], s[1], sc, sf}) if (st) (void)hipStreamDestroy(st);
    }
};
static constexpr u32 COS_MAX_HOST_PIPES = 32;

struct cos_index {
    cos_params p;
    int eng = -1;
    u32 n = 0;
    bool have_vectors = false, have_root = false;
    const float *d_raw = nullptr;
    DevArr<float> raw_own;
    DevArr<float> d_raw_mags;
    DevArr<uint8_t> d_codes;
    DevArr<float> d_mags;
    DevArr<u32> d_deleted;
    u64 row_stride = 0;
    u32 nchunks = 0, G = 1;
    std::vector<float> root_raw;
    std::vector<LevelHost> lv;
    u32 id_stride = 1;
    MetaGraph meta;
    hipStream_t own_stream = nullptr;
    std::mutex mu;
    std::map<void *, std::unique_ptr<Workspace>> ws;
    std::mutex pipe_mu;
    std::condition_variable pipe_cv;
    std::vector<std::unique_ptr<HostPipe>> pipes_all;
    std::vector<HostPipe *> pipes_free;
    std::atomic<int> host_calls_active{0};
    Workspace *last_ws = nullptr;
    std::mutex co_mu;
    std::condition_variable co_cv;
    std::vector<struct CoSlot *> co_slots;
    struct CoSlot *co_open = nullptr;
    u32 co_max_queries = 0, co_window_us = 0;
    u32 co_inflight = 0;
    cos_coalescing_stats co_stats{};
    bool timing = false;
    std::mutex chain_mu;
    hipEvent_t chain_ev = nullptr;
    hipEvent_t chain_last_range_ev = nullptr;
    hipEvent_t chain_upper_ev = nullptr;
    u32 chain_min_B = 16384;
    u32 walk_order_min_B = COS_WALK_ORDER_DEFAULT_MIN_B;
    u32 n_cus = 256;
    u32 num_xcd = 8;
    DevArr<u32> d_order_rank[cosdev::MAX_LEVELS];
    u32 order_rank_n[cosdev::MAX_LEVELS] = {};
    std::vector<u32> order_levels;
    bool order_rank_valid = false;
    u32 walk_table_max_cols = COS_WALK_TABLE_AUTO, walk_table_min_B = COS_WALK_TABLE_DEFAULT_MIN_B;
    size_t table_bytes_total = 0;
    bool adj_mag_valid = false;
    u32 adj_up_level = 0, adj_up_oom_level = 0;
    void invalidate_adj_side() { adj_mag_valid = false; adj_up_level = 0; adj_up_oom_level = 0; }
    LinkState link;
    bool level_table_valid = false;
    u32 table_level_min = 0, table_cols = 0;
    u64 table_built_for_key = 0;
    u64 table_stride = 0;
    u32 table_col0[cosdev::MAX_LEVELS] = {};
    const uint8_t *d_tcodes = nullptr;
    const float *d_tmags = nullptr;
    const u32 *d_tcsums = nullptr;
    struct TableSet { u64 key; u32 level_min, cols; u64 stride; u32 col0[cosdev::MAX_LEVELS]; DevArr<uint8_t> tcodes; DevArr<float> tmags; DevArr<u32> tcsums; };
    std::vector<TableSet> table_sets;
    u32 walk_side_min_B = 4096;
    u32 lat_max_B = COS_LATENCY_MODE_DEFAULT_MAX_B;
    u32 lat4_max_B = COS_LATENCY_WAVES_DEFAULT_MAX_B;
    struct FlatWs *flat_ws = nullptr;
};


struct FlatWs;
void cos_flat_ws_release(cos_index *ix);
hipError_t cos_deleted_reset(cos_index *ix, u32 n, hipStream_t st);
hipError_t cos_deleted_grow(cos_index *ix, u32 n0, u32 n1, hipStream_t st);
hipError_t cos_deleted_mark(cos_index *ix, const u32 *ids, u32 m, hipStream_t st);
void cos_coalesce_release(cos_index *ix);
cosdev::IndexDev cos_make_index_dev(const cos_index *ix);
cosdev::IndexDev cos_make_meta_dev(const cos_index *ix);
int32_t cos_set_device(const cos_index *ix);
cosdev::WalkPlanIn cos_walk_plan_in(const cos_index *ix, u32 B, u32 ef);
int32_t cos_prepare_walk_plans(cos_index *ix);
void cos_meta_free_levels(cos_index *ix);
```

### cosdata_amd/csrc/engine_types.h

```cpp
#pragma once
#include <stdint.h>
#include "device_common.h"

namespace cosdev {

struct LevelDev {
    const u32 *adj_vec;
    const u32 *adj_node;
    const u32 *node_vec;
    const u32 *child;
    u32 n;
    u32 M;
    u32 root_idx;
    const float *adj_mag;
    u32 mag_stride;
    const AdjUp *adj_up;
    const u32 *node_id;
    const u32 *node_meta;
};

struct IndexDev {
    const uint8_t *codes;
    const float *mags;
    const float *raw;
    const float *raw_mags;
    u64 row_stride;
    u64 raw_stride;
    u32 n;
    u32 dim;
    u32 metric;
    u32 storage;
    u32 num_layers;
    u32 shortlist;
    u32 visited_mode;
    u32 nchunks;
    u32 G;
    u32 id_base;
    u32 id_stride;
    const int32_t *mbits;
    const float *mmags;
    u32 mdim;
    LevelDev lv[MAX_LEVELS];
};

struct WalkArgs {
    const uint8_t *qcodes;
    const float *qmags;
    const u32 *q_rows;
    const u32 *self_ids;
    u32 *vis_bits;
    u32 *vis_log;
    u32 vis_words_per_query;
    u32 vis_log_cap;
    u32 B;
    u32 ef;
    u32 keep;
    u32 *out_ids;
    float *out_sims;
    u32 *out_nodes;
    u32 *out_counts;
    int32_t *out_status;
    const int32_t *f_dims;
    const float *f_mags;
    const u32 *f_off;
    u64 *out_stats;
    u64 *out_stats2;
    const float *tab;
    const float *tab_mags;
    u64 tab_stride;
    u32 tab_level_min;
    u32 tab_col0[MAX_LEVELS];
    u32 no_self_seed;
    u32 smem_mmax;
    u32 smem_win_bytes;
    u32 merge_min;
    u32 phase;
    u32 level_first, level_last;
    u32 key_n;
    const u32 *order_rank;
    const u32 *q_order;
    u32 *entry0;
    u32 *order_key;
    u32 *order_iota;
};

constexpr u32 WALK_FAST_MAX_EF = 1024u;
constexpr u32 WALK_GENERAL_MAX_EF = 16384u;

}
```

### cosdata_amd/csrc/tuning.h

```cpp
#pragma once
#include <cstdint>

namespace cosdev {

enum TuneKey : int {
    TUNE_WALK_CHAIN_MIN_B,
    TUNE_WALK_ORDER_MIN_B,
    TUNE_WALK_SIDE_MIN_B,
    TUNE_WALK_SPLIT_LEVELS,
    TUNE_WALK_TABLE_COLS,
    TUNE_WALK_TABLE_MIN_B,
    TUNE_WALK_TABLE_MAX_BYTES,
    TUNE_WALK_TABLE_GEMM,
    TUNE_HOST_PIPELINE_MIN_B,
    TUNE_FLAT_UNFUSED,
    TUNE_FLAT_TILE_KERNEL,
    TUNE_FLAT_PF,
    TUNE_FLAT_FP4,
    TUNE_BM25_BLOCKS,
    TUNE_SPARSE_LAYOUT,
    TUNE_WALK_PB,
    TUNE_WALK_PB_UPPER,
    TUNE_WALK_LAT,
    TUNE_WALK_LAT4,
    TUNE_WALK_SMALL_TABLE_TK,
    TUNE_WALK_LAT_WARM,
    TUNE_WALK_LAT_LA,
    TUNE_WALK_LAT4_E,
    TUNE_FINALIZE_FAST,
    TUNE_SHARDSET_FORCE_RCCL,
    TUNE_BUILD_PROFILE,
    TUNE_WALK_MERGE_MIN,
    TUNE_WALK_ADJ_MAG,
    TUNE_WALK_TABLE_RULE_C,
    TUNE_WALK_TABLE_AFTER_SORT,
    TUNE_WALK_UPPER_LDS_PAD,
    TUNE_WALK_R2,
    TUNE_FINALIZE_WIDE_MAX_B,
    TUNE_FLAT_FP4_W8,
    TUNE_WALK_TABLE_EARLY_WGS,
    TUNE_WALK_UP_TABLE,
    TUNE_COUNT
};

constexpr long long TUNE_UNSET = INT64_MIN;

long long tune(TuneKey k);
inline long long tune_or(TuneKey k, long long dflt) {
    const long long v = tune(k);
    return v == TUNE_UNSET ? dflt : v;
}

}
```

### cosdata_amd/csrc/tuning.hip

```cpp
#include <atomic>
#include <cstdlib>
#include <cstring>
#include <mutex>

#include "engine_internal.h"
#include "tuning.h"

namespace cosdev {
namespace {

const char *const NAMES[TUNE_COUNT] = {
    "walk_chain_min_b", "walk_order_min_b", "walk_side_min_b", "walk_split_levels", "walk_table_cols", "walk_table_min_b",
    "walk_table_max_bytes", "walk_table_gemm", "host_pipeline_min_b", "flat_unfused", "flat_tile_kernel", "flat_pf", "flat_fp4",
    "bm25_blocks", "sparse_layout", "walk_pb", "walk_pb_upper", "walk_lat", "walk_lat4", "walk_small_table_tk", "walk_lat_warm",
    "walk_lat_la", "walk_lat4_e", "finalize_fast", "shardset_force_rccl", "build_profile",
    "walk_merge_min", "walk_adj_mag", "walk_table_rule_c", "walk_table_after_sort", "walk_upper_lds_pad", "walk_r2", "finalize_wide_max_b", "flat_fp4_w8",
    "walk_table_early_wgs", "walk_up_table",
};
std::atomic<long long> g_values[TUNE_COUNT];
std::once_flag g_once;

int find_key(const char *name, size_t len) {
    for (int k = 0; k < TUNE_COUNT; k++)
        if (strlen(NAMES[k]) == len && strncmp(NAMES[k], name, len) == 0) return k;
    return -1;
}

void init_once() {
    std::call_once(g_once, [] {
        for (auto &v : g_values) v.store(TUNE_UNSET, std::memory_order_relaxed);
        const char *e = getenv("COS_TUNING");
        while (e && *e) {
            const char *end = strchr(e, ',');
            const size_t item = end ? (size_t)(end - e) : strlen(e);
            const char *eq = (const char *)memchr(e, '=', item);
            if (eq) {
                const int k = find_key(e, (size_t)(eq - e));
                char *stop = nullptr;
                const long long v = strtoll(eq + 1, &stop, 10);
                if (k >= 0 && stop != eq + 1) g_values[k].store(v, std::memory_order_relaxed);
            }
            e = end ? end + 1 : nullptr;
        }
    });
}

}

long long tune(TuneKey k) {
    init_once();
    return g_values[k].load(std::memory_order_relaxed);
}

}

using namespace cosdev;

extern "C" int32_t cos_tuning_set(const char *name, int64_t value) {
    if (!name) return cos_fail(COS_ERR_INVALID, "null knob name");
    const int k = find_key(name, strlen(name));
    if (k < 0) return cos_fail(COS_ERR_INVALID, "unknown tuning knob '%s'", name);
    if (value == TUNE_UNSET) return cos_fail(COS_ERR_INVALID, "INT64_MIN is the 'unset' marker: use cos_tuning_clear");
    init_once();
    g_values[k].store(value, std::memory_order_relaxed);
    return COS_OK;
}

extern "C" int32_t cos_tuning_clear(const char *name) {
    init_once();
    if (!name) {
        for (auto &v : g_values) v.store(TUNE_UNSET, std::memory_order_relaxed);
        return COS_OK;
    }
    const int k = find_key(name, strlen(name));
    if (k < 0) return cos_fail(COS_ERR_INVALID, "unknown tuning knob '%s'", name);
    g_values[k].store(TUNE_UNSET, std::memory_order_relaxed);
    return COS_OK;
}

extern "C" int32_t cos_tuning_get(const char *name, int64_t *out_value, int32_t *out_is_set) {
    if (!name || !out_value || !out_is_set) return cos_fail(COS_ERR_INVALID, "null argument");
    const int k = find_key(name, strlen(name));
    if (k < 0) return cos_fail(COS_ERR_INVALID, "unknown tuning knob '%s'", name);
    const long long v = tune((TuneKey)k);
    *out_is_set = v != TUNE_UNSET;
    *out_value = v == TUNE_UNSET ? 0 : v;
    return COS_OK;
}
```

### cosdata_amd/csrc/walk_kernel.inc

```
constexpr int PB = 4;
constexpr int LA = 4;

struct WalkSmem {
    u32 *vis;
    u64 *res;
    u32 *wl_vec;
    u32 *wl_node;
    u32 *win_vec;
    u32 *win_node;
    float *win_mag;
    float *qf;
};

template <int ENG, int CH, int R, bool G64, bool EXACT, int PB64 = 4>
__global__ __launch_bounds__(64) __attribute__((amdgpu_waves_per_eu(CH >= 3 ? (R <= 4 ? (CH == 3 ? 4 : 3) : (CH == 3 ? 3 : 2)) : (R == 1 ? ((ENG == ENG_U8 && CH == 1 && G64 && !EXACT) ? 7 : 6) : (R <= 4 ? 5 : 4)), 8))) void walk_kernel(const IndexDev ix, const WalkArgs wa) {
    extern __shared__ __attribute__((aligned(16))) unsigned char smem_raw[];
    const int lane = threadIdx.x;
    if (blockIdx.x >= wa.B) return;
    const u32 qi = wa.q_order ? wa.q_order[blockIdx.x] : blockIdx.x;
    const bool resume = wa.phase != 0u && wa.level_first < ix.num_layers;
    if (resume && wa.out_status[qi] != COS_OK) return;

    const u32 Mmax = wa.smem_mmax;
    WalkSmem sm;
    {
        unsigned char *p = smem_raw;
        sm.vis = (u32 *)p;      p += (size_t)Mmax * 8;
        sm.res = (u64 *)p;      p += (size_t)wa.ef * 8;
        sm.wl_vec = (u32 *)p;   p += 64 * 4;
        sm.wl_node = (u32 *)p;  p += 64 * 4;
        sm.win_vec = (u32 *)p;
        sm.win_node = (u32 *)(p + LA * 64 * 4);
        sm.win_mag = (float *)(p + 2 * LA * 64 * 4);
        p += wa.smem_win_bytes;
        p = (unsigned char *)(((size_t)p + 15) & ~(size_t)15);
        sm.qf = (float *)p;
    }

    const u32 qrow = wa.q_rows ? wa.q_rows[qi] : qi;
    const u32 self_id = wa.self_ids ? wa.self_ids[qi] * ix.id_stride : COS_QUERY_ID;
    const uint8_t *qcode = wa.qcodes + (u64)qrow * ix.row_stride;
    const float qmag = wa.qmags[qrow];
    const u32 N = ix.n;
    const u32 L = ix.num_layers;
    const u32 metric = ix.metric;
    constexpr bool exact = EXACT;
    u32 *vis = exact ? wa.vis_bits + (u64)qi * wa.vis_words_per_query : sm.vis;
    u32 *vlog = exact ? wa.vis_log + (u64)qi * wa.vis_log_cap : nullptr;

    constexpr bool FLOAT_ENG = ENG == ENG_F32 || ENG == ENG_F16;
    constexpr bool TABLE_OK = ENG == ENG_U8 || ENG == ENG_Q2;
    const int G = (ENG == ENG_F32) ? 8 : (ENG == ENG_F16 ? 1 : (int)ix.G);
    const int lig = lane & (G - 1);
    const int grp = lane / G;
    const int RP = 64 / G;
    uint4 qreg[CH];
    if constexpr (!FLOAT_ENG) {
#pragma unroll
        for (int c = 0; c < CH; c++) {
            u32 chunk = (u32)lig + (u32)c * (u32)G;
            qreg[c] = chunk < ix.nchunks ? *(const uint4 *)(qcode + (u64)chunk * 16) : make_uint4(0, 0, 0, 0);
        }
    } else if constexpr (ENG == ENG_F16) {
        const __half *qh = (const __half *)qcode;
        for (u32 i = lane; i < ix.dim; i += 64) sm.qf[i] = __half2float(qh[i]);
        __builtin_amdgcn_s_waitcnt(0);
#pragma unroll
        for (int c = 0; c < CH; c++) qreg[c] = make_uint4(0, 0, 0, 0);
    } else {
        const float *qg = (const float *)qcode;
        for (u32 i = lane; i < (u32)(ix.row_stride / 4); i += 64) sm.qf[i] = qg[i];
        __builtin_amdgcn_s_waitcnt(0);
#pragma unroll
        for (int c = 0; c < CH; c++) qreg[c] = make_uint4(0, 0, 0, 0);
    }

    u32 loff64[CH];
#pragma unroll
    for (int c = 0; c < CH; c++) {
        const u32 chunk = (u32)lane + (u32)c * 64u;
        loff64[c] = (chunk < ix.nchunks ? chunk : 0u) * 16u;
    }

    u64 n_evals = 0, n_exp = 0, adj_bytes = 0, n_rounds = 0, n_tab = 0;
    const u32 merge_min = uniform_u32(wa.merge_min);
    int32_t status = COS_OK;
    u32 entry = uniform_u32(resume ? wa.entry0[qi] : ix.lv[L].root_idx);
    const int level_first = wa.phase ? (int)wa.level_first : (int)L, level_last = wa.phase ? (int)wa.level_last : 0;
    u32 order_key = wa.key_n;

    auto single_distance = [&](u32 row, float &sim_out) -> bool {
        float dotf;
        if constexpr (!FLOAT_ENG) {
            dotf = (float)int_row_dot_group0<ENG, CH>(qreg, ix.codes + (u64)row * ix.row_stride, ix.nchunks, lig, grp, G);
        } else if constexpr (ENG == ENG_F16) {
            float d = f16_lane_dot(ix.codes + (u64)row * ix.row_stride, sm.qf, ix.dim);
            dotf = __uint_as_float(readlane_u32(__float_as_uint(d), 0));
        } else {
            float d = f32_oct_dot((const float *)(ix.codes + (u64)row * ix.row_stride), sm.qf, ix.dim, lane & 7);
            dotf = __uint_as_float(readlane_u32(__float_as_uint(d), 0));
        }
        bool bad;
        sim_out = cosine_or_dot(metric, dotf, qmag, uniform_f32(ix.mags[row]), bad);
        return !bad;
    };

    for (int level = level_first; level >= level_last; level--) {
        const LevelDev lv = ix.lv[level];
        const u32 M = lv.M;
        const u32 slots = M < ix.shortlist ? M : ix.shortlist;
        const u32 bitmask = 64u * M - 1u;
        const u32 out_slot = L - (u32)level;
        u32 nlog = 0;
        const bool tab_level = TABLE_OK && wa.tab != nullptr && (u32)level >= wa.tab_level_min;
        const float *tabq = wa.tab + (u64)qi * wa.tab_stride + wa.tab_col0[level];
        const float *tabm = wa.tab_mags + wa.tab_col0[level];

        if (!exact) {
            vis_clear<64>(sm.vis, M, lane);
            if (lane == 0 && wa.no_self_seed == 0u) vis_set_bit(sm.vis, self_id & bitmask);
        }

        Pool<R> pool;
        pool.clear();
        u32 npool = 0, npop = 0;
        u32 res_lo = 0, res_hi = 0;

        {
            const u32 erow = uniform_u32(lv.node_vec ? lv.node_vec[entry] : entry);
            float s0;
            if (tab_level) {
                bool bad;
                s0 = cosine_or_dot(metric, uniform_f32(tabq[entry]), qmag, uniform_f32(tabm[entry]), bad);
                if (bad) { status = COS_ERR_CALCULATION; break; }
            } else if (!single_distance(erow, s0)) { status = COS_ERR_CALCULATION; break; }
            if (lane == 0) {
                if (!exact) vis_set_bit(sm.vis, vis_bit_of(erow, N, ix.id_stride, bitmask));
                else {
                    atomicOr(&vis[entry >> 5], 1u << (entry & 31));
                    vlog[0] = entry >> 5;
                }
            }
            pool.insert_at(pack_key(metric_key(metric, s0), entry), 0, lane);
            npool = 1;
            if (exact) nlog = 1;
        }

        u32 failed = 0;
        u32 lev_evals = 1;
        const u32 log2M = (u32)__ffs((int)M) - 1u;
        const u64 slotmask = slots >= 64u ? ~0ull : ((1ull << slots) - 1ull);
        auto level_rounds = [&](auto tabc, auto cosc, auto amagc, auto upc) __attribute__((always_inline)) {
        constexpr bool TAB = decltype(tabc)::value;
        constexpr bool COSINE = decltype(cosc)::value;
        constexpr bool AMAG = decltype(amagc)::value && G64 && !FLOAT_ENG;
        constexpr bool UPT = decltype(upc)::value && AMAG && !TAB && ENG == ENG_U8;
        const u32 metric_t = COSINE ? 0u : metric;
        constexpr int LAW = UPT ? LA - 1 : LA;
        u32 *const w_vec = sm.win_vec, *const w_node = UPT ? sm.win_vec + LAW * 64 : sm.win_node, *const w_up = sm.win_vec + 3 * LAW * 64;
        float *const w_mag = UPT ? (float *)(sm.win_vec + 2 * LAW * 64) : sm.win_mag;
        const float *tabu = UPT ? wa.tab + (u64)qi * wa.tab_stride + wa.tab_col0[UPT ? level + 1 : 0] : nullptr;
        while (npool > 0 && npop < wa.ef) {
            n_rounds++;
            u32 kwin = npool < (u32)LAW ? npool : (u32)LAW;
            if (kwin > wa.ef - npop) kwin = wa.ef - npop;
            u32 wv_[LA], wn_[LA];
            {
                const u32 slot_l = (u32)lane < slots ? (u32)lane : slots - 1u;
                auto fetch_stage = [&](auto bothc) {
                    constexpr bool BOTH = decltype(bothc)::value;
                    float wm_[LA];
                    u32 wu_[LA];
                    static_for<0, LAW>([&](auto ic) {
                        constexpr int i = decltype(ic)::value;
                        const u32 nd = pool.template peek_node<i>();
                        const u64 off = ((u64)nd << log2M) + slot_l;
                        wv_[i] = lv.adj_vec[off];
                        if constexpr (BOTH) wn_[i] = lv.adj_node[off];
                        if constexpr (!TAB && AMAG && !UPT) wm_[i] = lv.adj_mag[(u64)nd * lv.mag_stride + slot_l];
                        if constexpr (UPT) {
                            const uint2 mu = ((const uint2 *)lv.adj_up)[(u64)nd * lv.mag_stride + slot_l];
                            wm_[i] = __uint_as_float(mu.x);
                            wu_[i] = mu.y;
                        }
                    });
                    if constexpr (!TAB) {
                        static_for<0, LAW>([&](auto ic) {
                            constexpr int i = decltype(ic)::value;
                            w_vec[i * 64 + lane] = wv_[i];
                            w_node[i * 64 + lane] = BOTH ? wn_[i] : wv_[i];
                            if constexpr (AMAG) w_mag[i * 64 + lane] = wm_[i];
                            if constexpr (UPT) w_up[i * 64 + lane] = wu_[i];
                        });
                    }
                };
                if (TAB || level != 0) fetch_stage(std::true_type{});
                else fetch_stage(std::false_type{});
            }
            u32 stop = 0;
            auto consume = [&](u32 wi, u32 nb_vec, u32 nb_node, float nb_mag, u32 nb_up) __attribute__((always_inline)) {
                if constexpr (R == 1) {
                    const u64 hd = pool.head();
                    res_lo = writelane_dyn(res_lo, (u32)hd, (int)npop);
                    res_hi = writelane_dyn(res_hi, (u32)(hd >> 32), (int)npop);
                } else if (lane == 0) sm.res[npop] = pool.e[0];
                pool.pop_head(lane);
                npool--;
                npop++;
                const int limit = (int)wa.ef - (int)npop;
                const int ahead = (int)kwin - 1 - (int)wi;
                u32 window_ok = 1;

                const u64 vmask = ballot64(nb_vec != ROW_EMPTY) & slotmask;
                u64 wmask;
                if (!exact) {
                    u32 bit = vis_bit_of(nb_vec, N, 1u, bitmask);
                    if (ix.id_stride != 1u) {
                        asm volatile("");
                        bit = vis_bit_of(nb_vec, N, ix.id_stride, bitmask);
                    }
                    const u32 word = bit >> 5, msk = 1u << (bit & 31);
                    u32 seen = sm.vis[word];
                    asm volatile("" : "+v"(seen));
                    const u64 cmask = vmask & ballot64((seen & msk) == 0u);
                    wmask = cmask;
                    if (cmask) {
                    u32 old = 0;
                    if (__builtin_amdgcn_inverse_ballot_w64(cmask)) old = atomicOr(&sm.vis[word], msk);
                    wmask = vis_alias_winners(cmask, bit, cmask & ballot64((old & msk) != 0u));
                    }
                } else {
                    u32 w = 0;
                    if (__builtin_amdgcn_inverse_ballot_w64(vmask)) w = __hip_atomic_load(&vis[nb_node >> 5], __ATOMIC_RELAXED, __HIP_MEMORY_SCOPE_AGENT);
                    wmask = vmask & ballot64(((w >> (nb_node & 31)) & 1u) == 0u);
                    if (__builtin_amdgcn_inverse_ballot_w64(wmask)) {
                        atomicOr(&vis[nb_node >> 5], 1u << (nb_node & 31));
                        vlog[nlog + (u32)__popcll(wmask & ((1ull << lane) - 1ull))] = nb_node >> 5;
                    }
                    nlog += (u32)__popcll(wmask);
                }
                if (wmask) {
                const bool win = __builtin_amdgcn_inverse_ballot_w64(wmask);
                const int W = __popcll(wmask);
                lev_evals += (u32)W;
                auto insert_serial = [&](u64 pm, u32 keyv, u32 nodev) {
                    while (pm) {
                        const int p = __ffsll((long long)pm) - 1;
                        pm = clear_bit_u64(pm, p);
                        const u64 kk = pack_key(readlane_u32(keyv, p), readlane_u32(nodev, p));
                        const int pos = pool.rank_of(kk);
                        if (pos < limit) {
                            pool.insert_at(kk, pos, lane);
                            npool = npool + 1u < (u32)(64 * R) ? npool + 1u : (u32)(64 * R);
                            window_ok = pos < ahead ? 0u : window_ok;
                        }
                    }
                };
                auto commit = [&](u64 leadmask, u32 keyv, u32 nodev) {
                    const u64 bar = limit > 0 ? pool.peek_dyn((u32)(limit - 1)) : ~0ull;
                    insert_serial(leadmask & ballot64(pack_key(keyv, nodev) > bar), keyv, nodev);
                };
                auto commit_merge = [&](u64 leadmask, u32 keyv, u32 nodev) {
                    const u64 bar = limit > 0 ? pool.peek_dyn((u32)(limit - 1)) : ~0ull;
                    const u64 mykey = pack_key(keyv, nodev);
                    const u64 pm = leadmask & ballot64(mykey > bar);
                    const u32 Wp = (u32)__popcll(pm);
                    if (Wp < merge_min) { insert_serial(pm, keyv, nodev); return; }
                    u32 below[R];
#pragma unroll
                    for (int r = 0; r < R; r++) below[r] = 0u;
                    u32 posv = 0u;
                    u32 abovev = 0u;
                    u32 minrank = ~0u;
                    u64 m = pm;
                    while (m) {
                        const int p = __ffsll((long long)m) - 1;
                        m = clear_bit_u64(m, p);
                        const u64 kk = pack_key(readlane_u32(keyv, p), readlane_u32(nodev, p));
                        u32 rank = 0;
#pragma unroll
                        for (int r = 0; r < R; r++) {
                            const bool gt = pool.e[r] > kk;
                            rank += (u32)__popcll(ballot64(gt));
                            below[r] += gt ? 1u : 0u;
                        }
                        minrank = rank < minrank ? rank : minrank;
                        abovev += kk > mykey ? 1u : 0u;
                        posv = writelane_dyn(posv, rank, p);
                    }
                    window_ok = (int)minrank < ahead ? 0u : window_ok;
                    u64 *mg = (u64 *)sm.win_vec;
#pragma unroll
                    for (int r = 0; r < R; r++) {
                        u32 np = (u32)lane * R + r + (Wp - below[r]);
                        np = np < (u32)(64 * R) ? np : (u32)(64 * R);
                        mg[np] = pool.e[r];
                    }
                    if (__builtin_amdgcn_inverse_ballot_w64(pm)) {
                        u32 np = posv + abovev;
                        np = np < (u32)(64 * R) ? np : (u32)(64 * R);
                        mg[np] = mykey;
                    }
                    __builtin_amdgcn_fence(__ATOMIC_RELEASE, "wavefront");
                    __builtin_amdgcn_wave_barrier();
                    __builtin_amdgcn_fence(__ATOMIC_ACQUIRE, "wavefront");
#pragma unroll
                    for (int r = 0; r < R; r++) pool.e[r] = mg[(u32)lane * R + r];
                    npool = npool + Wp < (u32)(64 * R) ? npool + Wp : (u32)(64 * R);
                };
                if constexpr (TAB) {
                    float simv = 0.0f, magv = 1.0f;
                    if (win) { simv = tabq[nb_node]; magv = tabm[nb_node]; }
                    bool badl;
                    simv = cosine_or_dot<ENG == ENG_U8>(metric_t, simv, qmag, magv, badl);
                    if (wmask & ballot64(badl)) failed = 1;
                    else if constexpr (R <= 4) {
                        if (merge_min != 0u) commit_merge(wmask, metric_key(metric_t, simv), nb_node);
                        else commit(wmask, metric_key(metric_t, simv), nb_node);
                    } else commit(wmask, metric_key(metric_t, simv), nb_node);
                } else if constexpr (G64 && !FLOAT_ENG) {
                    float magw = 1.0f;
                    if constexpr (AMAG) magw = nb_mag;
                    else if (win) magw = ix.mags[nb_vec];
                    u64 m = wmask;
                    if constexpr (UPT) {
                        const u64 tmask = wmask & ballot64(nb_up != ADJ_UP_NONE);
                        if (tmask) {
                            float dotv = 0.0f;
                            if (__builtin_amdgcn_inverse_ballot_w64(tmask)) dotv = tabu[nb_up];
                            bool badl;
                            const float sim = cosine_or_dot<ENG == ENG_U8>(metric, dotv, qmag, magw, badl);
                            if (tmask & ballot64(badl)) failed = 1;
                            else commit(tmask, metric_key(metric, sim), nb_node);
                            n_tab += (u64)__popcll(tmask);
                            m = wmask & ~tmask;
                        }
                    }
                    while (m && !failed) {
                        u32 lsel = 0;
                        u32 tot = 0;
                        u64 leadmask = 0;
                        auto eval_block = [&](auto npc) {
                            constexpr int NP = decltype(npc)::value;
                            constexpr int LS = 64 / NP;
                            uint4 buf[NP][CH];
                            int cnt = 0;
                            static_for<0, NP>([&](auto pc) {
                                constexpr int p = decltype(pc)::value;
                                if (m) {
                                    const int l = __ffsll((long long)m) - 1;
                                    m = clear_bit_u64(m, l);
                                    const uint8_t *rp = row_ptr_scalar(ix.codes, readlane_u32(nb_vec, l), (u32)ix.row_stride);
                                    lsel = writelane_u32<p * LS>(lsel, (u32)l << 2);
#pragma unroll
                                    for (int c = 0; c < CH; c++) {
                                        u32 lo = loff64[c];
                                        asm("" : "+v"(lo));
                                        buf[p][c] = *(const uint4 *)(rp + lo);
                                    }
                                    cnt++;
                                }
                            });
                            u32 acc[NP];
                            static_for<0, NP>([&](auto pc) {
                                constexpr int p = decltype(pc)::value;
                                acc[p] = 0;
                                if (p < cnt) {
                                    asm volatile("");
#pragma unroll
                                    for (int c = 0; c < CH; c++) acc[p] = chunk_dot<ENG>(qreg[c], buf[p][c], acc[p]);
                                }
                            });
                            tot = wave_reduce_rows<NP>(acc);
                            constexpr u64 firsts = NP == 8 ? 0x0101010101010101ull : 0x0001000100010001ull;
                            leadmask = cnt == NP ? firsts : firsts & ((1ull << (cnt * LS)) - 1ull);
                        };
                        if constexpr (PB64 == 8) {
                            if (__popcll(m) > 4) eval_block(std::integral_constant<int, 8>{});
                            else eval_block(std::integral_constant<int, 4>{});
                        } else {
                            eval_block(std::integral_constant<int, 4>{});
                        }
                        const float magv = __uint_as_float((u32)__builtin_amdgcn_ds_bpermute((int)lsel, (int)__float_as_uint(magw)));
                        const u32 nodev = (u32)__builtin_amdgcn_ds_bpermute((int)lsel, (int)nb_node);
                        const float dotv = (float)tot;
                        bool badl;
                        const float sim = cosine_or_dot<ENG == ENG_U8>(metric, dotv, qmag, magv, badl);
                        if (leadmask & ballot64(badl)) { failed = 1; break; }
                        commit(leadmask, metric_key(metric, sim), nodev);
                    }
                } else {
                if (win) {
                    const int rank = __popcll(wmask & ((1ull << lane) - 1ull));
                    sm.wl_vec[rank] = nb_vec;
                    sm.wl_node[rank] = nb_node;
                }

                for (int base = 0; base < W; base += RP * PB) {
                    u32 prow[PB];
                    float pmag[PB];
                    uint4 buf[PB][CH];
                    float fdot[PB];
#pragma unroll
                    for (int p = 0; p < PB; p++) {
                        if (base + p * RP >= W) break;
                        const int my = base + p * RP + grp;
                        const bool v = my < W;
                        prow[p] = v ? sm.wl_vec[my] : 0u;
                        pmag[p] = 1.0f;
                        if (v) pmag[p] = ix.mags[prow[p]];
                        if constexpr (!FLOAT_ENG) {
#pragma unroll
                            for (int c = 0; c < CH; c++) {
                                u32 chunk = (u32)lig + (u32)c * (u32)G;
                                buf[p][c] = make_uint4(0, 0, 0, 0);
                                if (v && chunk < ix.nchunks) buf[p][c] = *(const uint4 *)(ix.codes + (u64)prow[p] * ix.row_stride + (u64)chunk * 16);
                            }
                        }
                    }
                    if constexpr (FLOAT_ENG) {
#pragma unroll
                        for (int p = 0; p < PB; p++) {
                            if (base + p * RP >= W) break;
                            if constexpr (ENG == ENG_F32)
                                fdot[p] = f32_oct_dot((const float *)(ix.codes + (u64)prow[p] * ix.row_stride), sm.qf, ix.dim, lane & 7);
                            else
                                fdot[p] = f16_lane_dot(ix.codes + (u64)prow[p] * ix.row_stride, sm.qf, ix.dim);
                        }
                    }
#pragma unroll
                    for (int p = 0; p < PB; p++) {
                        if (base + p * RP >= W) break;
                        float dotf;
                        if constexpr (!FLOAT_ENG) {
                            u32 acc = 0;
#pragma unroll
                            for (int c = 0; c < CH; c++) acc = chunk_dot<ENG>(qreg[c], buf[p][c], acc);
                            acc = group_reduce_add_u32(acc, G);
                            dotf = (float)acc;
                        } else {
                            dotf = fdot[p];
                        }
                        const int mine = base + p * RP + grp;
                        const bool leadg = lig == 0 && mine < W;
                        bool badl;
                        const float sim = cosine_or_dot(metric, dotf, qmag, pmag[p], badl);
                        if (ballot64(mine < W && badl)) { failed = 1; break; }
                        const u32 mynode = leadg ? sm.wl_node[mine] : 0u;
                        commit(ballot64(leadg), metric_key(metric, sim), mynode);
                    }
                    if (failed) break;
                }
                }
                stop = failed | (window_ok ^ 1u);
                }
            };
            if constexpr (TAB) {
                static_for<0, LA>([&](auto ic) __attribute__((always_inline)) {
                    constexpr int i = decltype(ic)::value;
                    if ((u32)i < kwin && !stop) consume((u32)i, wv_[i], wn_[i], 1.0f, ADJ_UP_NONE);
                });
            } else {
                for (u32 wi = 0; wi < kwin && !stop; wi++)
                    consume(wi, w_vec[wi * 64 + lane], w_node[wi * 64 + lane], AMAG ? w_mag[wi * 64 + lane] : 1.0f, UPT ? w_up[wi * 64 + lane] : ADJ_UP_NONE);
            }
            if (failed) break;
        }
        };
        if (tab_level) {
            if (metric == 0u) level_rounds(std::true_type{}, std::true_type{}, std::false_type{}, std::false_type{});
            else level_rounds(std::true_type{}, std::false_type{}, std::false_type{}, std::false_type{});
        } else {
            bool done = false;
            if constexpr (G64 && !FLOAT_ENG) {
                if (lv.adj_mag != nullptr) {
                    bool up = false;
                    if constexpr (ENG == ENG_U8) {
                        if (lv.adj_up != nullptr && wa.tab != nullptr && (u32)level + 1u == wa.tab_level_min) {
                            level_rounds(std::false_type{}, std::false_type{}, std::true_type{}, std::true_type{});
                            up = true;
                        }
                    }
                    if (!up) level_rounds(std::false_type{}, std::false_type{}, std::true_type{}, std::false_type{});
                    done = true;
                }
            }
            if (!done) level_rounds(std::false_type{}, std::false_type{}, std::false_type{}, std::false_type{});
        }
        n_exp += npop;
        adj_bytes += (u64)npop * slots * 4;
        n_evals += lev_evals;
        if (tab_level) n_tab += lev_evals;
        if (exact) {
            __atomic_signal_fence(__ATOMIC_SEQ_CST);
            __builtin_amdgcn_s_waitcnt(0);
            for (u32 i = lane; i < nlog; i += 64) {
                const u32 w = __hip_atomic_load(&vlog[i], __ATOMIC_RELAXED, __HIP_MEMORY_SCOPE_AGENT);
                __hip_atomic_store(&vis[w], 0u, __ATOMIC_RELAXED, __HIP_MEMORY_SCOPE_AGENT);
            }
            __atomic_signal_fence(__ATOMIC_SEQ_CST);
            __builtin_amdgcn_s_waitcnt(0);
        }
        if (failed) { status = COS_ERR_CALCULATION; break; }

        u64 rk[R];
#pragma unroll
        for (int r = 0; r < R; r++) {
            const u32 e = (u32)lane * R + r;
            if constexpr (R == 1) rk[r] = e < npop ? pack_key(res_hi, res_lo) : 0ull;
            else rk[r] = e < npop ? sm.res[e] : 0ull;
        }
        bitonic_sort_desc<R>(rk, lane);
        u32 cnt = npop < wa.keep ? npop : wa.keep;
        if (npop == 0) {
            const u32 erow = uniform_u32(lv.node_vec ? lv.node_vec[entry] : entry);
            float s0;
            if (!single_distance(erow, s0)) { status = COS_ERR_CALCULATION; break; }
            rk[0] = lane == 0 ? pack_key(metric_key(metric, s0), entry) : 0ull;
            cnt = 1;
        }
        const u64 obase = level_list_base(ix, wa, qi, out_slot);
#pragma unroll
        for (int r = 0; r < R; r++) {
            const u32 e = (u32)lane * R + r;
            if (e < cnt) {
                const u32 nd = (u32)rk[r];
                const u32 vrow = lv.node_vec ? lv.node_vec[nd] : nd;
                wa.out_ids[obase + e] = vrow == N ? COS_ROOT_ID : vrow * ix.id_stride;
                wa.out_sims[obase + e] = metric_key_inv(metric, (u32)(rk[r] >> 32));
                if (wa.out_nodes) wa.out_nodes[obase + e] = nd;
            }
        }
        if (lane == 0) wa.out_counts[(u64)qi * (L + 1) + out_slot] = cnt;
        if (level > 0) {
            const u32 best = (u32)readlane_u64(rk[0], 0);
            entry = uniform_u32(lv.child[best]);
            if (wa.phase != 0u && level == level_last) order_key = uniform_u32(wa.order_rank[best]);
        }
    }

    if (lane == 0) {
        wa.out_status[qi] = status;
        if (wa.phase != 0u && level_last > 0) {
            wa.entry0[qi] = entry;
            wa.order_key[qi] = status == COS_OK ? order_key : wa.key_n;
            wa.order_iota[qi] = qi;
        }
        if (wa.out_stats) {
            const bool add = resume;
            wa.out_stats[(u64)qi * 4 + 0] = n_evals + (add ? wa.out_stats[(u64)qi * 4 + 0] : 0ull);
            wa.out_stats[(u64)qi * 4 + 1] = n_exp + (add ? wa.out_stats[(u64)qi * 4 + 1] : 0ull);
            wa.out_stats[(u64)qi * 4 + 2] = adj_bytes + (add ? wa.out_stats[(u64)qi * 4 + 2] : 0ull);
            wa.out_stats[(u64)qi * 4 + 3] = n_rounds + (add ? wa.out_stats[(u64)qi * 4 + 3] : 0ull);
        }
        if (wa.out_stats2) {
            if (resume || wa.phase == 0u) {
                wa.out_stats2[(u64)qi * 4 + 0] = n_evals;
                wa.out_stats2[(u64)qi * 4 + 1] = n_exp;
                wa.out_stats2[(u64)qi * 4 + 2] = adj_bytes;
            }
            wa.out_stats2[(u64)qi * 4 + 3] = n_tab + (resume ? wa.out_stats2[(u64)qi * 4 + 3] : 0ull);
        }
    }
}
```

### cosdata_amd/csrc/walk_plan.h

```cpp
#pragma once
#include <algorithm>
#include <cstdint>

namespace cosdev {

constexpr int WALK_PLAN_MAX_LEVELS = 16;
constexpr int WALK_PLAN_ENG_U8 = 0, WALK_PLAN_ENG_Q2 = 1;
constexpr uint32_t WALK_PLAN_FAST_MAX_EF = 1024u;

constexpr uint32_t ADJ_MAG_REFILL_MIN_B = 1024u, ADJ_MAG_USE_MIN_B = 4096u;

enum class WalkKernel : uint8_t {
    General,
    Throughput,
    Lat1,
    Lat4
};

struct WalkPlanIn {
    int eng;
    uint32_t storage;
    uint32_t nchunks, G;
    uint32_t num_layers, M[WALK_PLAN_MAX_LEVELS], shortlist, visited_mode, mdim;
    uint32_t B, ef;
    bool chain;
    bool no_self_seed;
    uint32_t lat_max_B, lat4_max_B;
    bool small_table_tk;
    uint32_t adj_mag_mode;
    uint32_t table_min_B;
    uint32_t order_min_B, chain_min_B, side_min_B;
    long long table_after_sort;
    bool table_supported;
    bool adj_mag_valid;
    uint32_t table_early_wgs;
    bool table_queue;
    uint32_t n_cus;
    uint32_t up_table_mode;
};

struct WalkHave {
    uint32_t table_level_min, table_cols;
    bool table_buffer;
    uint32_t n_order_keys, order_level0;
    bool order_buffers;
    uint32_t adj_up_level;
};

struct WalkPlan {
    WalkKernel kernel;
    bool ordered;
    bool use_table;
    bool table_waits_for_sort;
    uint32_t table_early_wgs;
    uint32_t use_adj_mag;
    bool refill_adj_mag;
    bool chained;
    bool side_stream;
    bool prepare_order, prepare_table;
    uint32_t table_level_min, table_cols, cut_after_level;
    uint32_t up_table_level;
};

inline uint32_t table_gemm_stripe_tiles(uint32_t B, uint32_t cols, uint32_t n_cus, bool shared) {
    const uint32_t n_tiles = (cols + 63u) / 64u, row_groups = (B + 255u) / 256u, cus = n_cus ? n_cus : 256u;
    if (!shared) {
        const uint32_t groups = std::max(1u, cus / std::max(1u, std::min(row_groups, cus)));
        return std::max(1u, (n_tiles + groups - 1u) / groups);
    }
    const uint64_t units = (uint64_t)n_tiles * row_groups;
    return (uint32_t)std::min<uint64_t>(64u, std::max<uint64_t>(2u, units / (24ull * cus)));
}
inline uint32_t table_gemm_items(uint32_t B, uint32_t cols, uint32_t n_cus, bool shared) {
    const uint32_t n_tiles = (cols + 63u) / 64u, st = table_gemm_stripe_tiles(B, cols, n_cus, shared);
    return (uint32_t)std::min<uint64_t>(0xFFFFFFFFull, (uint64_t)((n_tiles + st - 1u) / st) * ((B + 255u) / 256u));
}

inline bool walk_rows_over_64_slots(const WalkPlanIn &in) {
    for (uint32_t l = 0; l <= in.num_layers; l++)
        if (std::min(in.M[l], in.shortlist) > 64u) return true;
    return false;
}

inline bool walk_general_needed(const WalkPlanIn &in) {
    if (in.ef > WALK_PLAN_FAST_MAX_EF) return true;
    if (in.nchunks != 0u && in.G != 0u && (in.nchunks + in.G - 1u) / in.G > (in.storage == 0u  ? 4u : 1u)) return true;
    return walk_rows_over_64_slots(in);
}

inline bool walk_latency_domain(const WalkPlanIn &in, uint32_t max_B) {
    if (max_B == 0 || in.B > max_B) return false;
    if (in.visited_mode != 0) return false;
    if (in.eng != WALK_PLAN_ENG_U8 && in.eng != WALK_PLAN_ENG_Q2) return false;
    if (in.nchunks == 0 || in.nchunks > 64u) return false;
    if (in.ef == 0 || in.ef > 256) return false;
    return true;
}

inline WalkKernel walk_fast_kernel(const WalkPlanIn &in, bool table_available) {
    if (in.no_self_seed) return WalkKernel::Throughput;
    const bool lat4 = walk_latency_domain(in, in.lat4_max_B) && std::max(in.M[0], in.M[in.num_layers]) <= 64u;
    if (table_available && in.small_table_tk && in.eng == WALK_PLAN_ENG_U8)
        return in.ef > 128u && lat4 ? WalkKernel::Lat4 : WalkKernel::Throughput;
    if (lat4) return WalkKernel::Lat4;
    if (walk_latency_domain(in, in.lat_max_B)) return WalkKernel::Lat1;
    return WalkKernel::Throughput;
}

inline WalkPlan walk_plan(const WalkPlanIn &in, const WalkHave *have = nullptr) {
    WalkPlan p{};
    const bool general = walk_general_needed(in);
    p.ordered = !general && in.order_min_B && in.B >= in.order_min_B && in.ef <= 256u && (!have || (have->n_order_keys > 0 && have->order_buffers));
    bool table = !general && in.table_min_B && (have ? have->table_level_min != 0 && have->table_buffer : in.table_supported);
    const bool table_size = in.B >= in.table_min_B || in.B <= in.lat4_max_B;
    if (general) p.kernel = WalkKernel::General;
    else if (p.ordered) {
        p.kernel = WalkKernel::Throughput;
        table = table && table_size;
    } else {
        const WalkKernel with_table = walk_fast_kernel(in, true);
        table = table && ((with_table == WalkKernel::Lat4 && in.eng == WALK_PLAN_ENG_U8) || (with_table == WalkKernel::Throughput && table_size));
        p.kernel = table ? with_table : walk_fast_kernel(in, false);
    }
    p.use_table = table;
    p.chained = in.chain && in.B >= in.chain_min_B;
    if (have && table) {
        p.table_level_min = have->table_level_min;
        p.table_cols = have->table_cols;
        p.table_waits_for_sort = p.chained && (in.table_after_sort == 2 || (in.table_after_sort == 1 && (uint64_t)have->table_cols * in.B >= (1ull << 30)));
        if (p.table_waits_for_sort && in.table_queue)
            p.table_early_wgs = std::min(in.table_early_wgs, table_gemm_items(in.B, have->table_cols, in.n_cus, true));
    }
    if (have && p.ordered) p.cut_after_level = have->order_level0;
    if (in.adj_mag_valid && in.adj_mag_mode != 0)
        for (uint32_t l = 0; l <= in.num_layers; l++)
            if (in.adj_mag_mode == 2 || (in.ef <= 2u * in.M[l] && in.B >= ADJ_MAG_USE_MIN_B)) p.use_adj_mag |= 1u << l;
    p.refill_adj_mag = !in.adj_mag_valid && in.B >= ADJ_MAG_REFILL_MIN_B;
    if (have && p.use_table && p.kernel == WalkKernel::Throughput && in.up_table_mode != 0 && in.eng == WALK_PLAN_ENG_U8 && in.G == 64u &&
        in.mdim == 0u && have->table_level_min >= 2u && have->adj_up_level == have->table_level_min - 1u) {
        const uint32_t l = have->table_level_min - 1u;
        if (in.up_table_mode == 2 && in.adj_mag_valid && in.adj_mag_mode != 0) p.use_adj_mag |= 1u << l;
        if ((p.use_adj_mag >> l) & 1u) p.up_table_level = l;
    }
    p.side_stream = in.side_min_B && in.B >= in.side_min_B;
    p.prepare_order = p.ordered;
    p.prepare_table = p.use_table;
    return p;
}

}
```

### cosdata_amd/index.py

```python
from __future__ import annotations

import ctypes as C
import enum
from dataclasses import dataclass
from typing import List, Optional, Sequence, Tuple

import numpy as np

from . import _lib
from ._lib import CosdataError, CosFlatStats, CosParams, CosSearchStats, CosTimingSummary, CosWalkSplit, check

ROOT_ID, QUERY_ID, SLOT_EMPTY = 0xFFFFFFFF, 0xFFFFFFFE, 0xFFFFFFFD
VISITED_REF, VISITED_EXACT = 0, 1


class DistanceMetric(enum.IntEnum):
    Cosine = 0
    Euclidean = 1
    Hamming = 2
    DotProduct = 3


class StorageKind(enum.IntEnum):
    UnsignedByte = 0
# ... 104 lines not shown
        self.mdim = 0
        return self

    def upload_vectors_device(self, dev_ptr: int, n: int, keepalive=None):
        check(_lib.lib().cos_index_upload_vectors(self._h, C.c_void_p(dev_ptr), n, 1))
        self.n = n
        self.mdim = 0
        self._keepalive = keepalive
        return self

    def _queries(self, queries) -> np.ndarray:
        q = _c(np.atleast_2d(queries), np.float32)
        if q.ndim != 2 or q.shape[1] != self.dim:
            raise CosdataError(_lib.ERR_INVALID, f"queries must be [B][{self.dim}] f32, got shape {tuple(q.shape)}")
        return q

    def set_root(self, root_raw):
        r = _c(root_raw, np.float32)
        if r.size != self.dim:
            raise CosdataError(_lib.ERR_INVALID, f"root vector must hold {self.dim} values, got {r.size}")
        check(_lib.lib().cos_index_set_root(self._h, _p(r)))
        return self

    def level_M(self, level: int) -> int:
        return self.hnsw_params.level_0_neighbors_count if level == 0 else self.hnsw_params.neighbors_count

    def upload_graph_level(self, level: int, node_ids, nbr_ids):
        ids, nbr = _c(node_ids, np.uint32), _c(nbr_ids, np.uint32)
        assert nbr.shape == (ids.size, self.level_M(level))
        check(_lib.lib().cos_index_upload_graph_level(self._h, level, ids.size, _p(ids), _p(nbr)))
        return self

    def upload_graph(self, levels: Sequence[Tuple[np.ndarray, np.ndarray]], root_raw):
        self.set_root(root_raw)
        for l, (ids, nbr) in enumerate(levels):
            self.upload_graph_level(l, ids, nbr)
        return self

    def level_count(self, level: int) -> int:
        n = C.c_uint32()
        check(_lib.lib().cos_index_level_count(self._h, level, C.byref(n)))
        return n.value

    def download_graph(self):
        out = []
        for l in range(self.hnsw_params.num_layers + 1):
            n = self.level_count(l)
            ids = np.zeros(n, np.uint32)
            nbr = np.zeros((n, self.level_M(l)), np.uint32)
            check(_lib.lib().cos_index_download_graph_level(self._h, l, _p(ids), _p(nbr)))
            out.append((ids, nbr))
        return out

    def download_root(self):
        r = np.zeros(self.dim, np.float32)
        check(_lib.lib().cos_index_download_root(self._h, _p(r)))
        return r

    def download_codes(self):
        cb = _lib.lib().cos_code_bytes(int(self.storage_type.kind), self.storage_type.resolution, self.dim)
        codes = np.zeros((self.n + 1, cb), np.uint8)
        mags = np.zeros(self.n + 1, np.float32)
        check(_lib.lib().cos_index_download_codes(self._h, _p(codes), _p(mags)))
        return codes, mags

    def load_reference_dir(self, dense_hnsw_dir: str, root_ptr_offset: int, verify_codes: bool = False):
        check(_lib.lib().cos_index_load_reference_dir(self._h, dense_hnsw_dir.encode(), root_ptr_offset, 1 if verify_codes else 0))
        return self

    def build(self, batch_size: int = 0):
        check(_lib.lib().cos_index_build(self._h, batch_size))
        return self

    def append(self, raw_new, batch_size: int = 0):
        x = _c(np.atleast_2d(raw_new), np.float32)
        if x.ndim != 2 or x.shape[1] != self.dim or x.shape[0] == 0:
            raise CosdataError(_lib.ERR_INVALID, f"new vectors must be [m][{self.dim}] f32, got shape {tuple(x.shape)}")
        check(_lib.lib().cos_index_append(self._h, _p(x), x.shape[0], 0, batch_size))
        self.n += x.shape[0]
        return self

    def append_device(self, dev_ptr_all: int, m: int, batch_size: int = 0, keepalive=None):
        check(_lib.lib().cos_index_append(self._h, C.c_void_p(dev_ptr_all), m, 1, batch_size))
        self.n += m
        self._keepalive = keepalive
        return self

    def delete(self, ids):
        a = _c(np.atleast_1d(ids), np.uint32)
        check(_lib.lib().cos_index_delete(self._h, _p(a), a.size))
        return self

    def restore_link_state(self):
        check(_lib.lib().cos_index_restore_link_state(self._h))
        return self

    def release_link_state(self):
        check(_lib.lib().cos_index_release_link_state(self._h))
        return self

    def set_ef_search(self, ef: int):
        check(_lib.lib().cos_index_set_ef_search(self._h, ef))
        self.hnsw_params.ef_search = ef

    def set_coalescing(self, max_queries: int, window_us: int = 200):
        check(_lib.lib().cos_index_set_coalescing(self._h, max_queries, window_us))

    def coalescing_stats(self) -> dict:
        st = _lib.CosCoalescingStats()
        check(_lib.lib().cos_index_coalescing_stats(self._h, C.byref(st)))
        return {f: int(getattr(st, f)) for f, _ in st._fields_}

    def set_visited_mode(self, mode: int):
        check(_lib.lib().cos_index_set_visited_mode(self._h, mode))

    LATENCY_MODE_DEFAULT_MAX_B = 2048

    def set_latency_mode(self, max_queries: int):
        check(_lib.lib().cos_index_set_latency_mode(self._h, max_queries))

    LATENCY_WAVES_DEFAULT_MAX_B = 512

    def set_latency_waves(self, max_queries: int):
        check(_lib.lib().cos_index_set_latency_waves(self._h, max_queries))

    WALK_ORDER_DEFAULT_MIN_B = 8192

    def set_walk_order(self, min_queries: int):
        check(_lib.lib().cos_index_set_walk_order(self._h, min_queries))

    def walk_order_cuts(self):
        lv = (C.c_uint32 * 16)()
        n = C.c_uint32()
        check(_lib.lib().cos_index_walk_order_cuts(self._h, lv, 16, C.byref(n)))
        return [int(lv[i]) for i in range(min(n.value, 16))]

    WALK_TABLE_DEFAULT_MIN_B = 1
    WALK_TABLE_DEFAULT_MAX_COLS = 8192
    WALK_TABLE_AUTO = 0xFFFFFFFF

    def set_walk_table(self, max_cols: int = WALK_TABLE_AUTO, min_queries: int = WALK_TABLE_DEFAULT_MIN_B):
        check(_lib.lib().cos_index_set_walk_table(self._h, max_cols, min_queries))

    def walk_table_info(self):
        lv, cols = C.c_uint32(), C.c_uint32()
        check(_lib.lib().cos_index_walk_table_info(self._h, C.byref(lv), C.byref(cols)))
        return int(lv.value), int(cols.value)

    def last_walk_split(self, stream: int = 0) -> CosWalkSplit:
        st = CosWalkSplit()
        st.struct_size = C.sizeof(CosWalkSplit)
        check(_lib.lib().cos_index_last_walk_split(self._h, C.c_void_p(stream), C.byref(st)))
        return st

    def batch_search(self, queries, top_k: int, return_status: bool = False):
        q = self._queries(queries)
        B = q.shape[0]
        ids = np.full((B, top_k), 0xFFFFFFFF, np.uint32)
        scores = np.zeros((B, top_k), np.float32)
        counts = np.zeros(B, np.uint32)
        status = np.zeros(B, np.int32)
        rc = _lib.lib().cos_search_batch(self._h, _p(q), B, top_k, _p(ids), _p(scores), _p(counts), _p(status))
        if return_status:
            return ids, scores, counts, rc, status
        check(rc)
        return ids, scores, counts

    def search_internal(self, query, top_k: int):
        ids, scores, counts = self.batch_search(np.asarray(query, np.float32)[None, :], top_k)
        return [(int(ids[0, i]), float(scores[0, i])) for i in range(int(counts[0]))]

    def batch_search_device(self, q_ptr: int, B: int, top_k: int, out_ids_ptr: int, out_scores_ptr: int, out_counts_ptr: int,
                            out_status_ptr: int, stream: int = 0):
        check(_lib.lib().cos_search_batch_device(self._h, C.c_void_p(q_ptr), B, top_k, C.c_void_p(out_ids_ptr),
                                                 C.c_void_p(out_scores_ptr), C.c_void_p(out_counts_ptr),
                                                 C.c_void_p(out_status_ptr), C.c_void_p(stream)))

    def ann_search_batch(self, queries):
        q = self._queries(queries)
        B, L1 = q.shape[0], self.hnsw_params.num_layers + 1
        ids = np.zeros((B, L1, 100), np.uint32)
        sims = np.zeros((B, L1, 100), np.float32)
        counts = np.zeros((B, L1), np.uint32)
        status = np.zeros(B, np.int32)
        check(_lib.lib().cos_ann_search_batch(self._h, _p(q), B, _p(ids), _p(sims), _p(counts), _p(status)))
        return ids, sims, counts

    def enable_metadata(self, mdim: int, max_replicas_per_node: int):
        check(_lib.lib().cos_index_enable_metadata(self._h, mdim, max_replicas_per_node))
        self.mdim = mdim
        return self

    def upload_meta_graph(self, node_ids, mbits, levels):
        ids, mb = _c(node_ids, np.uint32), _c(mbits, np.int32)
        assert mb.shape == (ids.size, self.mdim)
        check(_lib.lib().cos_index_upload_meta_nodes(self._h, ids.size, _p(ids), _p(mb)))
        for l, (lid, nbr) in enumerate(levels):
            lid, nbr = _c(lid, np.uint32), _c(nbr, np.uint32)
            assert nbr.shape == (lid.size, self.level_M(l))
            check(_lib.lib().cos_index_upload_meta_graph_level(self._h, l, lid.size, _p(lid), _p(nbr)))
        return self

    def build_meta(self, node_ids, mbits, max_levels, batch_size: int = 0):
        ids, mb, ml = _c(node_ids, np.uint32), _c(mbits, np.int32), _c(max_levels, np.uint8)
        assert mb.shape == (ids.size, self.mdim) and ml.size == ids.size
        check(_lib.lib().cos_index_build_meta(self._h, ids.size, _p(ids), _p(mb), _p(ml), batch_size))
        return self

    def download_meta_graph(self):
        out = []
        for l in range(self.hnsw_params.num_layers + 1):
            n = C.c_uint32()
            check(_lib.lib().cos_index_meta_level_count(self._h, l, C.byref(n)))
            ids = np.zeros(n.value, np.uint32)
            nbr = np.zeros((n.value, self.level_M(l)), np.uint32)
            check(_lib.lib().cos_index_download_meta_graph_level(self._h, l, _p(ids), _p(nbr)))
            out.append((ids, nbr))
        return out

    def _filters(self, filter_offsets, filter_dims):
        off, fd = _c(filter_offsets, np.uint32), _c(np.atleast_2d(filter_dims), np.int8)
        if fd.shape[1] != self.mdim or off[-1] != fd.shape[0]:
            raise CosdataError(_lib.ERR_INVALID, f"filters must be [F][{self.mdim}] i8 with offsets ending at F")
        return off, fd

    def search_filtered(self, queries, filter_offsets, filter_dims, top_k: int, return_status: bool = False):
        q = self._queries(queries)
        off, fd = self._filters(filter_offsets, filter_dims)
        B = q.shape[0]
        ids = np.full((B, top_k), 0xFFFFFFFF, np.uint32)
        scores = np.zeros((B, top_k), np.float32)
        counts = np.zeros(B, np.uint32)
        status = np.zeros(B, np.int32)
        rc = _lib.lib().cos_search_filtered_batch(self._h, _p(q), B, _p(off), _p(fd), top_k, _p(ids), _p(scores), _p(counts), _p(status))
        if return_status:
            return ids, scores, counts, rc, status
        check(rc)
        return ids, scores, counts

    def ann_search_filtered(self, queries, filter_offsets, filter_dims):
        q = self._queries(queries)
        off, fd = self._filters(filter_offsets, filter_dims)
        B, L1 = q.shape[0], self.hnsw_params.num_layers + 1
        ids = np.zeros((B, L1, 100), np.uint32)
        sims = np.zeros((B, L1, 100), np.float32)
        counts = np.zeros((B, L1), np.uint32)
        status = np.zeros(B, np.int32)
        check(_lib.lib().cos_ann_search_filtered_batch(self._h, _p(q), B, _p(off), _p(fd), _p(ids), _p(sims), _p(counts), _p(status)))
        return ids, sims, counts

    def enable_timing(self, on: bool = True):
        check(_lib.lib().cos_index_enable_timing(self._h, 1 if on else 0))

    def last_stats(self, stream: int = 0) -> CosSearchStats:
        st = CosSearchStats()
        check(_lib.lib().cos_index_last_stats(self._h, C.c_void_p(stream), C.byref(st)))
        return st

    def timing_summary(self, stream: int) -> CosTimingSummary:
        st = CosTimingSummary()
        check(_lib.lib().cos_index_timing_summary(self._h, C.c_void_p(stream), C.byref(st)))
        return st

    def flat_search(self, queries, top_k: int, with_stats: bool = False):
        q = self._queries(queries)
        B = q.shape[0]
        ids = np.full((B, top_k), 0xFFFFFFFF, np.uint32)
        scores = np.zeros((B, top_k), np.float32)
        counts = np.zeros(B, np.uint32)
        st = CosFlatStats()
        check(_lib.lib().cos_flat_search_batch(self._h, _p(q), B, top_k, _p(ids), _p(scores), _p(counts), C.byref(st)))
        return (ids, scores, counts, st) if with_stats else (ids, scores, counts)

    def bruteforce_topk(self, queries, k: int):
        q = self._queries(queries)
        ids = np.zeros((q.shape[0], k), np.uint32)
        scores = np.zeros((q.shape[0], k), np.float32)
        check(_lib.lib().cos_bruteforce_topk(self._h, _p(q), q.shape[0], k, _p(ids), _p(scores)))
        return ids, scores

    def _scan_mask(self, masks, query_mask, skip_deleted: bool, B: int):
        if masks is None and query_mask is None and not skip_deleted:
            return None, ()
        words = (self.n + 31) // 32
        bits, qm, G = None, None, 0
        if masks is not None and np.asarray(masks).dtype == np.uint32:
            bits = _c(np.atleast_2d(masks), np.uint32)
            if bits.ndim != 2 or bits.shape[1] != words:
                raise CosdataError(_lib.ERR_INVALID, f"packed masks must be uint32 [G][{words}], got shape {tuple(bits.shape)}")
            G = bits.shape[0]
        elif masks is not None:
            m = np.atleast_2d(np.asarray(masks, dtype=bool))
            if m.ndim != 2 or m.shape[1] != self.n:
                raise CosdataError(_lib.ERR_INVALID, f"masks must be bool [{self.n}] or [G][{self.n}], got shape {tuple(np.shape(masks))}")
            G = m.shape[0]
            bits = pack_row_masks(m)
        if query_mask is not None:
            qm = _c(np.atleast_1d(query_mask), np.uint32)
            if qm.shape != (B,):
                raise CosdataError(_lib.ERR_INVALID, f"query_mask must hold {B} mask indices, got shape {tuple(qm.shape)}")
        sm = _lib.CosScanMask(C.sizeof(_lib.CosScanMask), _lib.SCAN_SKIP_DELETED if skip_deleted else 0, G,
                              bits.ctypes.data if bits is not None else None, qm.ctypes.data if qm is not None else None)
        return sm, (bits, qm)

    def flat_search_masked(self, queries, top_k: int, masks=None, query_mask=None, skip_deleted: bool = False, with_stats: bool = False):
        q = self._queries(queries)
# ... 41 lines not shown
```

### include/cosdata_hip.h

```cpp
#ifndef COSDATA_HIP_H
#define COSDATA_HIP_H

#include <stddef.h>
#include <stdint.h>

#ifdef __cplusplus
extern "C" {
#endif

#define COS_ABI_VERSION 1u

typedef enum { COS_METRIC_COSINE = 0, COS_METRIC_EUCLIDEAN = 1, COS_METRIC_HAMMING = 2, COS_METRIC_DOT = 3 } cos_metric;
typedef enum { COS_STORAGE_U8 = 0, COS_STORAGE_SUBBYTE = 1, COS_STORAGE_F16 = 2, COS_STORAGE_F32 = 3 } cos_storage;

typedef enum {
    COS_OK = 0,
    COS_ERR_STORAGE_MISMATCH = 1,
    COS_ERR_CALCULATION = 2,
    COS_ERR_INVALID = 3,
    COS_ERR_UNIMPLEMENTED = 4,
    COS_ERR_HIP = 5,
    COS_ERR_NOT_READY = 6,
    COS_ERR_NO_DEVICE = 7
} cos_status;

#define COS_ROOT_ID 0xFFFFFFFFu
#define COS_QUERY_ID 0xFFFFFFFEu
#define COS_SLOT_EMPTY 0xFFFFFFFDu

#define COS_VISITED_REF 0u
#define COS_VISITED_EXACT 1u

#define COS_UPLOAD_DEFAULT 0u
#define COS_UPLOAD_BORROW_DEVICE 1u

typedef struct {
    uint32_t struct_size;
    uint32_t abi_version;
    uint32_t dim;
    uint32_t metric;
    uint32_t storage;
    uint32_t resolution;
    float range_lo, range_hi;
    uint32_t num_layers;
    uint32_t neighbors_count;
    uint32_t level0_neighbors_count;
    uint32_t ef_construction;
    uint32_t ef_search;
    uint32_t shortlist_size;
    uint32_t visited_mode;
    int32_t device;
    uint32_t id_base;
    uint32_t reserved;
    uint64_t seed;
} cos_params;

typedef struct cos_index cos_index;

typedef struct {
    uint64_t evals;
    uint64_t expansions;
    uint64_t adj_bytes;
    uint64_t rerank_rows;
    float walk_ms;
    float finalize_ms;
    float prep_ms;
    uint32_t reserved;
} cos_search_stats;

int32_t cos_index_create(const cos_params *params, cos_index **out);
int32_t cos_index_destroy(cos_index *ix);
const char *cos_last_error_string(void);
int32_t cos_device_count(int32_t *out);
int32_t cos_hbm_probe(int32_t device, uint32_t kind, uint64_t buffer_bytes, uint32_t row_bytes, uint32_t iters,
                      double *out_gbps);

int32_t cos_index_upload_vectors(cos_index *ix, const float *raw, uint32_t n, uint32_t flags);
int32_t cos_index_set_root(cos_index *ix, const float *root_raw);
int32_t cos_index_upload_graph_level(cos_index *ix, uint32_t level, uint32_t n_nodes, const uint32_t *node_ids,
                                     const uint32_t *nbr_ids);
int32_t cos_index_level_count(const cos_index *ix, uint32_t level, uint32_t *n_nodes);
int32_t cos_index_download_graph_level(const cos_index *ix, uint32_t level, uint32_t *node_ids, uint32_t *nbr_ids);
int32_t cos_index_download_codes(const cos_index *ix, void *codes, float *mags);
int32_t cos_index_download_root(const cos_index *ix, float *root_raw);

#define COS_LOAD_DEFAULT 0u
#define COS_LOAD_VERIFY_CODES 1u
int32_t cos_index_load_reference_dir(cos_index *ix, const char *dense_hnsw_dir, uint32_t root_ptr_offset, uint32_t flags);
int32_t cos_reference_dir_level_counts(const char *dense_hnsw_dir, uint32_t num_layers, uint32_t neighbors_count,
                                       uint32_t level0_neighbors_count, uint32_t *level_counts );
int32_t cos_reference_dir_read_level(const char *dense_hnsw_dir, uint32_t num_layers, uint32_t neighbors_count,
                                     uint32_t level0_neighbors_count, uint32_t level, uint32_t *node_ids, uint32_t *nbr_ids);

int32_t cos_index_build(cos_index *ix, uint32_t batch_size);
int32_t cos_index_append(cos_index *ix, const float *raw, uint32_t m, uint32_t flags, uint32_t batch_size );
int32_t cos_index_delete(cos_index *ix, const uint32_t *ids, uint32_t m);
int32_t cos_index_restore_link_state(cos_index *ix);
int32_t cos_index_release_link_state(cos_index *ix);

int32_t cos_search_batch(cos_index *ix, const float *queries, uint32_t B, uint32_t top_k, uint32_t *out_ids,
                         float *out_scores, uint32_t *out_counts, int32_t *out_status);
int32_t cos_search_batch_device(cos_index *ix, const float *d_queries, uint32_t B, uint32_t top_k, uint32_t *d_out_ids,
                                float *d_out_scores, uint32_t *d_out_counts, int32_t *d_out_status, void *stream);
int32_t cos_ann_search_batch(cos_index *ix, const float *queries, uint32_t B, uint32_t *out_ids, float *out_sims,
                             uint32_t *out_counts, int32_t *out_status);
int32_t cos_index_set_coalescing(cos_index *ix, uint32_t max_queries, uint32_t window_us);
typedef struct cos_coalescing_stats {
    uint64_t launches;
    uint64_t queries;
    uint64_t requests;
    uint64_t closed_full;
    uint64_t closed_quiet;
    uint64_t closed_deadline;
    uint64_t solo_calls;
} cos_coalescing_stats;
int32_t cos_index_coalescing_stats(cos_index *ix, cos_coalescing_stats *out);
int32_t cos_index_set_ef_search(cos_index *ix, uint32_t ef_search);
int32_t cos_index_set_visited_mode(cos_index *ix, uint32_t mode);
#define COS_LATENCY_MODE_DEFAULT_MAX_B 2048u
int32_t cos_index_set_latency_mode(cos_index *ix, uint32_t max_queries);
#define COS_LATENCY_WAVES_DEFAULT_MAX_B 512u
int32_t cos_index_set_latency_waves(cos_index *ix, uint32_t max_queries);
#define COS_WALK_ORDER_DEFAULT_MIN_B 8192u
int32_t cos_index_set_walk_order(cos_index *ix, uint32_t min_queries);
int32_t cos_index_walk_order_cuts(cos_index *ix, uint32_t *out_levels, uint32_t cap, uint32_t *out_n);
#define COS_WALK_TABLE_DEFAULT_MIN_B 1u
#define COS_WALK_TABLE_DEFAULT_MAX_COLS 8192u
#define COS_WALK_TABLE_AUTO 0xFFFFFFFFu
int32_t cos_index_set_walk_table(cos_index *ix, uint32_t max_cols, uint32_t min_queries);
int32_t cos_index_walk_table_info(cos_index *ix, uint32_t *out_level_min, uint32_t *out_cols);
typedef struct {
    uint32_t struct_size;
    uint32_t queries;
    uint32_t table_level_min;
    uint32_t table_cols;
    uint32_t cut_after_level;
    uint32_t table_early_wgs;
    float table_ms;
    float upper_ms, sort_ms, lower_ms;
    double table_int8_ops;
    uint64_t table_evals;
    uint64_t upper_evals, upper_expansions, upper_adj_bytes;
    uint64_t lower_evals, lower_expansions, lower_adj_bytes;
} cos_walk_split;
int32_t cos_index_last_walk_split(cos_index *ix, void *stream, cos_walk_split *out);
int32_t cos_index_enable_timing(cos_index *ix, int32_t on);
int32_t cos_index_last_stats(cos_index *ix, void *stream, cos_search_stats *out);
typedef struct {
    uint32_t launches;
    float prep_ms_sum, walk_ms_sum, finalize_ms_sum;
    float walk_ms_min, walk_ms_max;
} cos_timing_summary;
int32_t cos_index_timing_summary(cos_index *ix, void *stream, cos_timing_summary *out);

int32_t cos_index_enable_metadata(cos_index *ix, uint32_t mdim , uint32_t max_replicas_per_node);
int32_t cos_index_upload_meta_nodes(cos_index *ix, uint32_t n_nodes, const uint32_t *node_ids, const int32_t *mbits);
int32_t cos_index_upload_meta_graph_level(cos_index *ix, uint32_t level, uint32_t n_nodes, const uint32_t *node_ids,
                                          const uint32_t *nbr_ids);
int32_t cos_index_build_meta(cos_index *ix, uint32_t n_nodes, const uint32_t *node_ids, const int32_t *mbits, const uint8_t *max_levels,
                             uint32_t batch_size );
int32_t cos_index_meta_level_count(cos_index *ix, uint32_t level, uint32_t *out);
int32_t cos_index_download_meta_graph_level(cos_index *ix, uint32_t level, uint32_t *node_ids, uint32_t *nbr_ids);
int32_t cos_search_filtered_batch(cos_index *ix, const float *queries, uint32_t B, const uint32_t *filter_offsets,
                                  const int8_t *filter_dims, uint32_t top_k, uint32_t *out_ids, float *out_scores,
                                  uint32_t *out_counts, int32_t *out_status);
int32_t cos_ann_search_filtered_batch(cos_index *ix, const float *queries, uint32_t B, const uint32_t *filter_offsets,
                                      const int8_t *filter_dims, uint32_t *out_ids, float *out_sims, uint32_t *out_counts,
                                      int32_t *out_status);

int32_t cos_quantize_batch(uint32_t storage, uint32_t resolution, uint32_t dim, float range_lo, float range_hi,
                           const float *x, uint32_t n, void *codes, float *mags);
size_t cos_code_bytes(uint32_t storage, uint32_t resolution, uint32_t dim);
int32_t cos_sample_values_range(const float *x, uint32_t n, uint32_t dim, float clamp_margin_percent, float *range_lo,
                                float *range_hi);
int32_t cos_distance_batch(uint32_t metric, uint32_t storage, uint32_t resolution, uint32_t dim, const void *x_codes,
                           const float *x_mags, uint32_t nx, const void *y_codes, const float *y_mags, uint32_t ny,
                           const uint32_t *pair_x, const uint32_t *pair_y, uint32_t n_pairs, float *out,
                           int32_t *status);
int32_t cos_bruteforce_topk(cos_index *ix, const float *queries, uint32_t B, uint32_t k, uint32_t *out_ids,
                            float *out_scores);

typedef struct {
    float gemm_ms;
    uint32_t gemm_launches;
    double int8_ops;
    double code_bytes;
} cos_flat_stats;
int32_t cos_flat_search_batch(cos_index *ix, const float *queries, uint32_t B, uint32_t top_k, uint32_t *out_ids,
                              float *out_scores, uint32_t *out_counts, cos_flat_stats *stats );

#define COS_SCAN_SKIP_DELETED 1u
typedef struct cos_scan_mask {
    uint32_t struct_size;
    uint32_t flags;
    uint32_t n_masks;
    const uint32_t *bits;
    const uint32_t *query_mask;
} cos_scan_mask;
int32_t cos_flat_search_masked_batch(cos_index *ix, const float *queries, uint32_t B, uint32_t top_k, const cos_scan_mask *mask,
                                     uint32_t *out_ids, float *out_scores, uint32_t *out_counts, cos_flat_stats *stats );
int32_t cos_bruteforce_topk_masked(cos_index *ix, const float *queries, uint32_t B, uint32_t k, const cos_scan_mask *mask,
                                   uint32_t *out_ids, float *out_scores, uint32_t *out_counts);
int32_t cos_index_deleted_count(cos_index *ix, uint32_t *out);
int32_t cos_index_download_deleted(cos_index *ix, uint32_t *bits);

typedef struct cos_bm25 cos_bm25;
int32_t cos_bm25_create(int32_t device, const uint32_t *term_hashes, const uint64_t *offsets, uint32_t n_terms,
                        const uint32_t *doc_ids, const float *tfs, uint32_t documents_count, cos_bm25 **out);
int32_t cos_bm25_destroy(cos_bm25 *b);
int32_t cos_bm25_insert(cos_bm25 *b, const uint32_t *doc_ids, const uint64_t *doc_offsets, uint32_t m, const uint32_t *term_hashes,
                        const float *tfs);
int32_t cos_bm25_delete(cos_bm25 *b, const uint32_t *doc_ids, const uint64_t *doc_offsets, uint32_t m, const uint32_t *term_hashes);
typedef struct {
    uint32_t struct_size;
    uint32_t documents_count;
    uint32_t n_terms;
    uint32_t largest_doc_id;
    uint32_t dir_rows;
    uint32_t dir_tiles;
    uint32_t reserved;
    uint64_t postings;
    uint64_t tombstones;
    uint64_t device_bytes;
} cos_bm25_index_stats;
int32_t cos_bm25_stats(cos_bm25 *b, cos_bm25_index_stats *out);
int32_t cos_bm25_download(cos_bm25 *b, uint32_t *n_terms, uint64_t *n_postings, uint32_t *term_hashes, uint64_t *offsets,
                          uint32_t *doc_ids, float *tfs, uint8_t *tombstones);
int32_t cos_bm25_search_batch(cos_bm25 *b, const uint32_t *q_terms, const uint32_t *q_offsets, uint32_t B,
                              uint32_t top_k, uint32_t *out_ids, float *out_scores, uint32_t *out_counts);
int32_t cos_bm25_search_batch_device(cos_bm25 *b, const uint32_t *q_terms, const uint32_t *q_offsets, uint32_t B, uint32_t top_k,
                                     uint32_t *d_out_ids, float *d_out_scores, uint32_t *d_out_counts, void *stream);
int32_t cos_rrf_fuse_batch(const uint32_t *dense_ids, const uint32_t *dense_counts, uint32_t dense_stride,
                           const uint32_t *sparse_ids, const uint32_t *sparse_counts, uint32_t sparse_stride, uint32_t B,
                           float fusion_constant_k, uint32_t top_k, uint32_t *out_ids, float *out_scores,
                           uint32_t *out_counts);

int32_t cos_hybrid_search_batch(cos_index *ix, cos_bm25 *b, const float *queries, const uint32_t *q_terms, const uint32_t *q_offsets,
                                uint32_t B, uint32_t top_k, float fusion_constant_k, uint32_t *out_ids, float *out_scores,
                                uint32_t *out_counts);

typedef size_t (*cos_stem_fn)(void *ctx, const char *token, size_t token_len, char *out, size_t out_cap);
int32_t cos_text_process(const char *utf8, size_t len, uint32_t max_token_len, float average_document_length, float k1, float b,
                         cos_stem_fn stem, void *stem_ctx, uint32_t *out_hashes, float *out_tfs, uint32_t cap, uint32_t *out_n);
uint32_t cos_text_count_tokens(const char *utf8, size_t len, uint32_t max_token_len);
float cos_bm25_term_frequency(uint32_t count, uint32_t document_length, float average_document_length, float k1, float b);
uint32_t cos_xxhash32(const void *data, size_t len, uint32_t seed);
size_t cos_stem_english(void *ctx, const char *token, size_t token_len, char *out, size_t out_cap);

typedef struct cos_sparse cos_sparse;
int32_t cos_sparse_create(int32_t device, uint32_t quantization_bits, float values_upper_bound, const uint32_t *dims, uint32_t n_dims,
                          const uint64_t *key_offsets, const uint32_t *vec_ids, uint32_t n_vectors, const uint64_t *row_offsets,
                          const uint32_t *raw_dims, const float *raw_vals, cos_sparse **out);
int32_t cos_sparse_build_csr(uint32_t quantization_bits, float values_upper_bound, uint32_t n_vectors, const uint64_t *row_offsets,
                             const uint32_t *raw_dims, const float *raw_vals, uint32_t *out_dims, uint64_t *out_key_offsets,
                             uint32_t *out_vec_ids, uint32_t *n_dims);
int32_t cos_sparse_create_from_vectors(int32_t device, uint32_t quantization_bits, float values_upper_bound, uint32_t n_vectors,
                                       const uint64_t *row_offsets, const uint32_t *raw_dims, const float *raw_vals, int32_t keep_raw,
                                       cos_sparse **out);
int32_t cos_sparse_destroy(cos_sparse *s);
int32_t cos_sparse_search_batch(cos_sparse *s, const uint32_t *q_dims, const float *q_vals, const uint32_t *q_offsets, uint32_t B,
                                uint32_t top_k, float early_terminate_threshold, uint32_t reranking_factor, uint32_t *out_ids,
                                float *out_scores, uint32_t *out_counts);

int32_t cos_sparse_set_max_candidates(cos_sparse *s, uint32_t max_candidates);
int32_t cos_sparse_max_candidates(cos_sparse *s, uint32_t *out);

typedef struct cos_sparse_stats {
    float kernel_ms;
    uint32_t blocks;
    uint64_t postings_visited;
    uint64_t posting_bytes;
} cos_sparse_search_stats;
int32_t cos_sparse_last_stats(cos_sparse *s, cos_sparse_search_stats *out);
int32_t cos_sparse_layout(cos_sparse *s, uint32_t *packed);
int32_t cos_sparse_insert(cos_sparse *s, uint32_t m, const uint64_t *row_offsets, const uint32_t *raw_dims, const float *raw_vals,
                          uint32_t *out_first_id);
int32_t cos_sparse_delete(cos_sparse *s, const uint32_t *ids, const uint64_t *row_offsets, uint32_t m, const uint32_t *raw_dims,
                          const float *raw_vals, uint64_t *out_removed);
typedef struct {
    uint32_t struct_size;
    uint32_t n_vectors;
    uint32_t n_dims;
    uint32_t dir_rows;
    uint32_t dir_tiles;
    uint32_t packed;
    uint32_t have_raw;
    uint32_t reserved;
    uint64_t postings;
    uint64_t removed;
    uint64_t raw_pairs;
    uint64_t device_bytes;
} cos_sparse_index_stats;
int32_t cos_sparse_stats(cos_sparse *s, cos_sparse_index_stats *out);
int32_t cos_sparse_download(cos_sparse *s, uint32_t *n_dims, uint64_t *n_postings, uint32_t *dims, uint64_t *key_offsets,
                            uint32_t *vec_ids);

typedef struct cos_hybrid cos_hybrid;
int32_t cos_hybrid_create(int32_t device, cos_hybrid **out);
// ... 56 lines not shown
```

Before: 1.135 million.

## Memoize upper-level similarities in LDS hash table to skip re-evaluation on lower levels

While writing each level's result list, the walk kernel now fills a small hash table in shared memory (reusing visited/worklist storage) that maps row ids to their computed similarity keys. When the search descends to the next level, neighbours that hit this memo reuse the stored score instead of recomputing the u8 dot product, and the entry point's score comes from the memo as well. The aim is to cut redundant distance evaluations in the HNSW descent. In exchange it adds hash probes, wave barriers and LDS traffic, and it aliases shared buffers, which carries a correctness risk. Optional per-level hit statistics are exposed through a new API.

```diff
diff --git a/cosdata_amd/_lib.py b/cosdata_amd/_lib.py
--- a/cosdata_amd/_lib.py
+++ b/cosdata_amd/_lib.py
@@ -120,7 +120,7 @@
     "cos_index_download_graph_level", "cos_index_download_codes", "cos_index_download_root", "cos_index_build", "cos_index_append", "cos_index_delete", "cos_index_restore_link_state", "cos_index_release_link_state", "cos_index_enable_metadata", "cos_index_upload_meta_nodes", "cos_index_upload_meta_graph_level", "cos_index_build_meta", "cos_index_meta_level_count", "cos_index_download_meta_graph_level", "cos_search_filtered_batch",
     "cos_ann_search_filtered_batch", "cos_index_load_reference_dir", "cos_reference_dir_level_counts", "cos_reference_dir_read_level",
     "cos_search_batch", "cos_search_batch_device", "cos_ann_search_batch", "cos_index_set_coalescing", "cos_index_coalescing_stats", "cos_index_set_ef_search",
-    "cos_index_set_visited_mode", "cos_index_set_latency_mode", "cos_index_set_latency_waves", "cos_index_set_walk_order", "cos_index_walk_order_cuts", "cos_index_set_walk_table", "cos_index_walk_table_info", "cos_index_last_walk_split", "cos_index_enable_timing", "cos_index_last_stats", "cos_index_timing_summary", "cos_quantize_batch",
+    "cos_index_set_visited_mode", "cos_index_set_latency_mode", "cos_index_set_latency_waves", "cos_index_set_walk_order", "cos_index_walk_order_cuts", "cos_index_set_walk_table", "cos_index_walk_table_info", "cos_index_last_walk_split", "cos_index_last_walk_memo", "cos_index_enable_timing", "cos_index_last_stats", "cos_index_timing_summary", "cos_quantize_batch",
     "cos_code_bytes", "cos_sample_values_range", "cos_distance_batch", "cos_bruteforce_topk", "cos_flat_search_batch",
     "cos_flat_search_masked_batch", "cos_bruteforce_topk_masked", "cos_index_deleted_count", "cos_index_download_deleted", "cos_bm25_create", "cos_bm25_destroy",
     "cos_bm25_insert", "cos_bm25_delete", "cos_bm25_stats", "cos_bm25_download",
@@ -189,6 +189,7 @@
         "cos_index_set_walk_table": [vp, u32, u32],
         "cos_index_walk_table_info": [vp, C.POINTER(u32), C.POINTER(u32)],
         "cos_index_last_walk_split": [vp, vp, C.POINTER(CosWalkSplit)],
+        "cos_index_last_walk_memo": [vp, vp, C.POINTER(C.c_uint32), C.POINTER(C.c_uint64)],
         "cos_index_timing_summary": [vp, vp, C.POINTER(CosTimingSummary)],
         "cos_quantize_batch": [u32, u32, u32, f32, f32, vp, u32, vp, vp],
         "cos_sample_values_range": [vp, u32, u32, f32, C.POINTER(f32), C.POINTER(f32)],
diff --git a/cosdata_amd/csrc/engine.hip b/cosdata_amd/csrc/engine.hip
--- a/cosdata_amd/csrc/engine.hip
+++ b/cosdata_amd/csrc/engine.hip
@@ -682,6 +682,7 @@
 }
 static constexpr long long WALK_TABLE_EARLY_WGS_DEFAULT = 0;
 static constexpr long long WALK_UP_TABLE_DEFAULT = 1;
+static constexpr long long WALK_MEMO_DEFAULT = 1;
 cosdev::WalkPlanIn cos_walk_plan_in(const cos_index *ix, u32 B, u32 ef) {
     cosdev::WalkPlanIn in{};
     in.eng = ix->eng;
@@ -709,6 +710,7 @@
     in.table_supported = cosdev::level_table_eng_supported(ix->eng, ix->row_stride);
     in.adj_mag_valid = ix->adj_mag_valid;
     in.up_table_mode = (u32)std::min<long long>(std::max<long long>(cosdev::tune_or(cosdev::TUNE_WALK_UP_TABLE, WALK_UP_TABLE_DEFAULT), 0), 2);
+    in.memo_mode = (u32)std::min<long long>(std::max<long long>(cosdev::tune_or(cosdev::TUNE_WALK_MEMO, WALK_MEMO_DEFAULT), 0), 2);
     in.table_early_wgs = (u32)std::min<long long>(std::max<long long>(cosdev::tune_or(cosdev::TUNE_WALK_TABLE_EARLY_WGS, WALK_TABLE_EARLY_WGS_DEFAULT), 0), 0xFFFFFFFFll);
     in.table_queue = cosdev::level_table_gemm_queue(ix->eng, ix->row_stride);
     in.n_cus = ix->n_cus;
@@ -905,6 +907,7 @@
     cosdev::WalkPlan plan;
     u32 ef = 0, visited_mode = 0;
     bool timed = false;
+    bool memo_stats = false;
     u64 tab_stride = 0;
     u32 tab_col0[cosdev::MAX_LEVELS] = {};
     const uint8_t *tcodes = nullptr;
@@ -965,6 +968,7 @@
         have.order_buffers = w->order.cap >= B;
         have.n_order_keys = (u32)ix->order_levels.size();
         have.order_level0 = have.n_order_keys ? ix->order_levels[0] : 0u;
+        for (u32 l : ix->order_levels) have.order_key_mask |= 1u << l;
     }
     if (want.prepare_table) {
         if (int32_t rc = ensure_level_table(ix)) return rc;
@@ -990,6 +994,11 @@
         have.table_buffer = w->tab && (size_t)B * ix->table_stride <= w->tab.cap;
     }
     L->plan = cosdev::walk_plan(in, &have);
+    L->memo_stats = L->plan.memo_levels != 0u && (L->timed || in.memo_mode == 2);
+    if (L->memo_stats && w->memo_stats.cap < (size_t)w->capB * cosdev::MAX_LEVELS) {
+        HIP_TRY(hipStreamSynchronize(st));
+        HIP_TRY(w->memo_stats.alloc((size_t)w->capB * cosdev::MAX_LEVELS));
+    }
     if (L->plan.use_table) {
         L->tab_stride = ix->table_stride;
         memcpy(L->tab_col0, ix->table_col0, sizeof(L->tab_col0));
@@ -1044,6 +1053,7 @@
     HIP_TRY(launch_quantize_rows(ix->eng, d_queries, ix->p.dim, B, ix->p.dim, ix->p.range_lo, ix->p.range_hi, w->q_codes, ix->row_stride,
                                  w->q_mags, w->q_raw_mags, st, plan.use_table && ix->eng == ENG_U8 ? w->qsums.p : nullptr));
     HIP_TRY(hipMemsetAsync(w->stats2, 0, (size_t)B * 32, st));
+    if (L.memo_stats) HIP_TRY(hipMemsetAsync(w->memo_stats, 0, (size_t)B * cosdev::MAX_LEVELS * 4, st));
     if (plan.use_table) {
         auto table_part = [&](hipEvent_t cos_index::*handle_ev, hipEvent_t own_ev, hipEvent_t *marks, u32 wgs, bool first) -> int32_t {
             if (plan.table_waits_for_sort) {
@@ -1075,6 +1085,8 @@
     wa.out_status = w->walk_status;
     wa.out_stats = w->stats;
     wa.out_stats2 = w->stats2;
+    wa.memo_levels = plan.kernel == cosdev::WalkKernel::Throughput ? plan.memo_levels : 0u;
+    wa.out_memo = L.memo_stats ? w->memo_stats.p : nullptr;
     if (plan.use_table) {
         wa.tab = w->tab;
         wa.tab_mags = L.tmags;
@@ -1152,6 +1164,7 @@
     w->lastB = B;
     w->timed = timed;
     w->last_plan = plan;
+    w->last_memo_stats = L.memo_stats;
     { std::lock_guard<std::mutex> g(ix->mu); ix->last_ws = w; }
     return COS_OK;
 }
@@ -1631,6 +1644,31 @@
     out->upper_evals = st[0] - s2[0];
     out->upper_expansions = st[1] - s2[1];
     out->upper_adj_bytes = st[2] - s2[2];
+    return COS_OK;
+}
+
+extern "C" int32_t cos_index_last_walk_memo(cos_index *ix, void *stream, uint32_t *memo_levels, uint64_t *hits) {
+    if (!ix || !memo_levels || !hits) return cos_fail(COS_ERR_INVALID, "null argument");
+    *memo_levels = 0;
+    for (int l = 0; l < cosdev::MAX_LEVELS; l++) hits[l] = 0;
+    int32_t rc = cos_set_device(ix);
+    if (rc) return rc;
+    Workspace *w = find_workspace(ix, stream, true);
+    if (!w || w->lastB == 0) return cos_fail(COS_ERR_NOT_READY, "no batch has run on this stream");
+    const u32 mask = w->last_plan.kernel == cosdev::WalkKernel::Throughput ? w->last_plan.memo_levels : 0u;
+    *memo_levels = mask;
+    if (!w->last_memo_stats) return COS_OK;
+    HIP_TRY(hipDeviceSynchronize());
+    std::vector<u32> ms((size_t)w->lastB * cosdev::MAX_LEVELS);
+    HIP_TRY(hipMemcpy(ms.data(), w->memo_stats, ms.size() * 4, hipMemcpyDeviceToHost));
+    for (u32 b = 0; b < w->lastB; b++) {
+        const u32 *q = &ms[(size_t)b * cosdev::MAX_LEVELS];
+        for (int l = 0; l < cosdev::MAX_LEVELS; l++) {
+            if (!((mask >> l) & 1u) || q[l] == 0u) continue;
+            const bool above = l + 1 < cosdev::MAX_LEVELS && ((mask >> (l + 1)) & 1u);
+            hits[l] += q[l] - (above ? q[l + 1] : 0u);
+        }
+    }
     return COS_OK;
 }
 
diff --git a/cosdata_amd/csrc/engine_internal.h b/cosdata_amd/csrc/engine_internal.h
--- a/cosdata_amd/csrc/engine_internal.h
+++ b/cosdata_amd/csrc/engine_internal.h
@@ -130,6 +130,8 @@
     DevArr<int32_t> walk_status;
     DevArr<u64> stats;
     DevArr<u64> stats2;
+    DevArr<u32> memo_stats;
+    bool last_memo_stats = false;
     DevArr<float> tab;
     DevArr<u32> qsums;
     DevArr<u32> tab_queue;
diff --git a/cosdata_amd/csrc/engine_types.h b/cosdata_amd/csrc/engine_types.h
--- a/cosdata_amd/csrc/engine_types.h
+++ b/cosdata_amd/csrc/engine_types.h
@@ -82,6 +82,8 @@
     u32 *entry0;
     u32 *order_key;
     u32 *order_iota;
+    u32 memo_levels;
+    u32 *out_memo;
 };
 
 constexpr u32 WALK_FAST_MAX_EF = 1024u;
diff --git a/cosdata_amd/csrc/tuning.h b/cosdata_amd/csrc/tuning.h
--- a/cosdata_amd/csrc/tuning.h
+++ b/cosdata_amd/csrc/tuning.h
@@ -40,6 +40,7 @@
     TUNE_FLAT_FP4_W8,
     TUNE_WALK_TABLE_EARLY_WGS,
     TUNE_WALK_UP_TABLE,
+    TUNE_WALK_MEMO,
     TUNE_COUNT
 };
 
diff --git a/cosdata_amd/csrc/tuning.hip b/cosdata_amd/csrc/tuning.hip
--- a/cosdata_amd/csrc/tuning.hip
+++ b/cosdata_amd/csrc/tuning.hip
@@ -15,7 +15,7 @@
     "bm25_blocks", "sparse_layout", "walk_pb", "walk_pb_upper", "walk_lat", "walk_lat4", "walk_small_table_tk", "walk_lat_warm",
     "walk_lat_la", "walk_lat4_e", "finalize_fast", "shardset_force_rccl", "build_profile",
     "walk_merge_min", "walk_adj_mag", "walk_table_rule_c", "walk_table_after_sort", "walk_upper_lds_pad", "walk_r2", "finalize_wide_max_b", "flat_fp4_w8",
-    "walk_table_early_wgs", "walk_up_table",
+    "walk_table_early_wgs", "walk_up_table", "walk_memo",
 };
 std::atomic<long long> g_values[TUNE_COUNT];
 std::once_flag g_once;
diff --git a/cosdata_amd/csrc/walk_kernel.inc b/cosdata_amd/csrc/walk_kernel.inc
--- a/cosdata_amd/csrc/walk_kernel.inc
+++ b/cosdata_amd/csrc/walk_kernel.inc
@@ -89,10 +89,13 @@
     const int level_first = wa.phase ? (int)wa.level_first : (int)L, level_last = wa.phase ? (int)wa.level_last : 0;
     u32 order_key = wa.key_n;
 
+    constexpr bool MEMO_OK = ENG == ENG_U8 && G64 && !EXACT;
     auto single_distance = [&](u32 row, float &sim_out) -> bool {
         float dotf;
         if constexpr (!FLOAT_ENG) {
-            dotf = (float)int_row_dot_group0<ENG, CH>(qreg, ix.codes + (u64)row * ix.row_stride, ix.nchunks, lig, grp, G);
+            int lig_here = lig;
+            if constexpr (MEMO_OK) asm volatile("" : "+v"(lig_here));
+            dotf = (float)int_row_dot_group0<ENG, CH>(qreg, ix.codes + (u64)row * ix.row_stride, ix.nchunks, lig_here, grp, G);
         } else if constexpr (ENG == ENG_F16) {
             float d = f16_lane_dot(ix.codes + (u64)row * ix.row_stride, sm.qf, ix.dim);
             dotf = __uint_as_float(readlane_u32(__float_as_uint(d), 0));
@@ -104,6 +107,9 @@
         sim_out = cosine_or_dot(metric, dotf, qmag, uniform_f32(ix.mags[row]), bad);
         return !bad;
     };
+
+    auto memo_slot = [&](u32 s, u32 Mp) -> uint2 * { return (uint2 *)((s < 64u ? sm.wl_vec : sm.vis + 2u * Mp - 128u) + 2u * s); };
+    auto memo_shift_of = [&](u32 Mp) -> u32 { return (u32)__clz((int)(64u + Mmax - Mp)) + 1u; };
 
     for (int level = level_first; level >= level_last; level--) {
         const LevelDev lv = ix.lv[level];
@@ -115,6 +121,9 @@
         const bool tab_level = TABLE_OK && wa.tab != nullptr && (u32)level >= wa.tab_level_min;
         const float *tabq = wa.tab + (u64)qi * wa.tab_stride + wa.tab_col0[level];
         const float *tabm = wa.tab_mags + wa.tab_col0[level];
+        bool memo_probe = false;
+        if constexpr (MEMO_OK) memo_probe = ((wa.memo_levels >> level) & 1u) != 0u && level < level_first && !tab_level;
+        const u32 memo_shift = MEMO_OK ? memo_shift_of(lv.M) : 0u;
 
         if (!exact) {
             vis_clear<64>(sm.vis, M, lane);
@@ -129,10 +138,15 @@
         {
             const u32 erow = uniform_u32(lv.node_vec ? lv.node_vec[entry] : entry);
             float s0;
+            u32 memo_key0 = 0;
             if (tab_level) {
                 bool bad;
                 s0 = cosine_or_dot(metric, uniform_f32(tabq[entry]), qmag, uniform_f32(tabm[entry]), bad);
                 if (bad) { status = COS_ERR_CALCULATION; break; }
+            } else if (memo_probe) {
+                memo_key0 = uniform_u32(memo_slot((erow * 0x9E3779B1u) >> memo_shift, M)->y);
+                n_tab += 1ull << 32;
+                s0 = 0.0f;
             } else if (!single_distance(erow, s0)) { status = COS_ERR_CALCULATION; break; }
             if (lane == 0) {
                 if (!exact) vis_set_bit(sm.vis, vis_bit_of(erow, N, ix.id_stride, bitmask));
@@ -141,7 +155,8 @@
                     vlog[0] = entry >> 5;
                 }
             }
-            pool.insert_at(pack_key(metric_key(metric, s0), entry), 0, lane);
+            if constexpr (MEMO_OK) pool.insert_at(pack_key(memo_probe ? memo_key0 : metric_key(metric, s0), entry), 0, lane);
+            else pool.insert_at(pack_key(metric_key(metric, s0), entry), 0, lane);
             npool = 1;
             if (exact) nlog = 1;
         }
@@ -155,6 +170,7 @@
         constexpr bool COSINE = decltype(cosc)::value;
         constexpr bool AMAG = decltype(amagc)::value && G64 && !FLOAT_ENG;
         constexpr bool UPT = decltype(upc)::value && AMAG && !TAB && ENG == ENG_U8;
+        constexpr bool MEMO = AMAG && !TAB && !UPT && MEMO_OK;
         const u32 metric_t = COSINE ? 0u : metric;
         constexpr int LAW = UPT ? LA - 1 : LA;
         u32 *const w_vec = sm.win_vec, *const w_node = UPT ? sm.win_vec + LAW * 64 : sm.win_node, *const w_up = sm.win_vec + 3 * LAW * 64;
@@ -336,6 +352,17 @@
                             m = wmask & ~tmask;
                         }
                     }
+                    if constexpr (MEMO) {
+                    if (memo_probe) {
+                        const uint2 me = *memo_slot((nb_vec * 0x9E3779B1u) >> memo_shift, M);
+                        const u64 hmask = wmask & ballot64(me.x == nb_vec);
+                        if (hmask) {
+                            commit(hmask, me.y, nb_node);
+                            n_tab += (u64)__popcll(hmask) << 32;
+                            m = wmask & ~hmask;
+                        }
+                    }
+                    }
                     while (m && !failed) {
                         u32 lsel = 0;
                         u32 tot = 0;
@@ -487,6 +514,9 @@
             }
             if (!done) level_rounds(std::false_type{}, std::false_type{}, std::false_type{}, std::false_type{});
         }
+        if constexpr (MEMO_OK) {
+            if (memo_probe && wa.out_memo != nullptr && lane == 0) wa.out_memo[(u64)qi * MAX_LEVELS + (u32)level] = (u32)(n_tab >> 32);
+        }
         n_exp += npop;
         adj_bytes += (u64)npop * slots * 4;
         n_evals += lev_evals;
@@ -520,6 +550,18 @@
             cnt = 1;
         }
         const u64 obase = level_list_base(ix, wa, qi, out_slot);
+        bool memo_build = false;
+        u32 build_M = 0, build_shift = 0, vrow_head = 0;
+        if constexpr (MEMO_OK) {
+            memo_build = level > level_last && ((wa.memo_levels >> (level - 1)) & 1u) != 0u;
+            if (memo_build) {
+                build_M = ix.lv[level - 1].M;
+                build_shift = memo_shift_of(build_M);
+                for (u32 s = (u32)lane; s < (1u << (32u - build_shift)); s += 64u) *memo_slot(s, build_M) = make_uint2(ROW_EMPTY, 0u);
+                __builtin_amdgcn_fence(__ATOMIC_RELEASE, "wavefront");
+                __builtin_amdgcn_wave_barrier();
+            }
+        }
 #pragma unroll
         for (int r = 0; r < R; r++) {
             const u32 e = (u32)lane * R + r;
@@ -529,6 +571,20 @@
                 wa.out_ids[obase + e] = vrow == N ? COS_ROOT_ID : vrow * ix.id_stride;
                 wa.out_sims[obase + e] = metric_key_inv(metric, (u32)(rk[r] >> 32));
                 if (wa.out_nodes) wa.out_nodes[obase + e] = nd;
+                if constexpr (MEMO_OK) {
+                    if (memo_build && e != 0u) *memo_slot((vrow * 0x9E3779B1u) >> build_shift, build_M) = make_uint2(vrow, (u32)(rk[r] >> 32));
+                    if (r == 0) vrow_head = vrow;
+                }
+            }
+        }
+        if constexpr (MEMO_OK) {
+            if (memo_build) {
+                __builtin_amdgcn_fence(__ATOMIC_RELEASE, "wavefront");
+                __builtin_amdgcn_wave_barrier();
+                if (lane == 0) *memo_slot((vrow_head * 0x9E3779B1u) >> build_shift, build_M) = make_uint2(vrow_head, (u32)(rk[0] >> 32));
+                __builtin_amdgcn_fence(__ATOMIC_RELEASE, "wavefront");
+                __builtin_amdgcn_wave_barrier();
+                __builtin_amdgcn_fence(__ATOMIC_ACQUIRE, "wavefront");
             }
         }
         if (lane == 0) wa.out_counts[(u64)qi * (L + 1) + out_slot] = cnt;
@@ -559,6 +615,7 @@
                 wa.out_stats2[(u64)qi * 4 + 1] = n_exp;
                 wa.out_stats2[(u64)qi * 4 + 2] = adj_bytes;
             }
+            if constexpr (MEMO_OK) n_tab &= 0xFFFFFFFFull;
             wa.out_stats2[(u64)qi * 4 + 3] = n_tab + (resume ? wa.out_stats2[(u64)qi * 4 + 3] : 0ull);
         }
     }
diff --git a/cosdata_amd/csrc/walk_plan.h b/cosdata_amd/csrc/walk_plan.h
--- a/cosdata_amd/csrc/walk_plan.h
+++ b/cosdata_amd/csrc/walk_plan.h
@@ -37,6 +37,7 @@
     bool table_queue;
     uint32_t n_cus;
     uint32_t up_table_mode;
+    uint32_t memo_mode;
 };
 
 struct WalkHave {
@@ -45,6 +46,7 @@
     uint32_t n_order_keys, order_level0;
     bool order_buffers;
     uint32_t adj_up_level;
+    uint32_t order_key_mask;
 };
 
 struct WalkPlan {
@@ -60,6 +62,7 @@
     bool prepare_order, prepare_table;
     uint32_t table_level_min, table_cols, cut_after_level;
     uint32_t up_table_level;
+    uint32_t memo_levels;
 };
 
 inline uint32_t table_gemm_stripe_tiles(uint32_t B, uint32_t cols, uint32_t n_cus, bool shared) {
@@ -142,6 +145,15 @@
         if (in.up_table_mode == 2 && in.adj_mag_valid && in.adj_mag_mode != 0) p.use_adj_mag |= 1u << l;
         if ((p.use_adj_mag >> l) & 1u) p.up_table_level = l;
     }
+    if (have && p.kernel == WalkKernel::Throughput && in.memo_mode != 0 && in.eng == WALK_PLAN_ENG_U8 && in.G == 64u && in.mdim == 0u &&
+        in.visited_mode == 0u) {
+        const uint32_t row_top = p.use_table ? p.table_level_min - 1u : in.num_layers;
+        for (uint32_t l = 0; l < row_top; l++) {
+            if (p.ordered && ((have->order_key_mask >> (l + 1u)) & 1u)) continue;
+            if (in.memo_mode == 2 && in.adj_mag_valid && in.adj_mag_mode != 0) p.use_adj_mag |= 1u << l;
+            if ((p.use_adj_mag >> l) & 1u) p.memo_levels |= 1u << l;
+        }
+    }
     p.side_stream = in.side_min_B && in.B >= in.side_min_B;
     p.prepare_order = p.ordered;
     p.prepare_table = p.use_table;
diff --git a/cosdata_amd/index.py b/cosdata_amd/index.py
--- a/cosdata_amd/index.py
+++ b/cosdata_amd/index.py
@@ -280,6 +280,12 @@
         st.struct_size = C.sizeof(CosWalkSplit)
         check(_lib.lib().cos_index_last_walk_split(self._h, C.c_void_p(stream), C.byref(st)))
         return st
+
+    def last_walk_memo(self, stream: int = 0):
+        mask = C.c_uint32()
+        hits = (C.c_uint64 * 16)()
+        check(_lib.lib().cos_index_last_walk_memo(self._h, C.c_void_p(stream), C.byref(mask), hits))
+        return int(mask.value), [int(h) for h in hits]
 
     def batch_search(self, queries, top_k: int, return_status: bool = False):
         q = self._queries(queries)
diff --git a/include/cosdata_hip.h b/include/cosdata_hip.h
--- a/include/cosdata_hip.h
+++ b/include/cosdata_hip.h
@@ -144,6 +144,7 @@
     uint64_t lower_evals, lower_expansions, lower_adj_bytes;
 } cos_walk_split;
 int32_t cos_index_last_walk_split(cos_index *ix, void *stream, cos_walk_split *out);
+int32_t cos_index_last_walk_memo(cos_index *ix, void *stream, uint32_t *out_memo_levels, uint64_t *hits);
 int32_t cos_index_enable_timing(cos_index *ix, int32_t on);
 int32_t cos_index_last_stats(cos_index *ix, void *stream, cos_search_stats *out);
 typedef struct {
```

Result: faster. 1.151 million, median of 6 (+1.4%).
